# rogerbarton/optix-renderer

Hardware: AMD Instinct MI355X
Metric: Msamples/sec (whole node) + traversal HBM GB/s, cbox 1024x1024 256spp (higher is better)
Workload: dtype f32; 1 GPU; Cornell box (diffuse-only) 1024x1024, 16400 spp, path_mis; config=c2, width=1024, height=1024, spp=16400, mode=wavefront, traversal=ordered, pools=2, gpu_max_hw_queues=8, parallelism=single GPU

## Files before the change

### include/nori_hip.h

```cpp
#ifndef NORI_HIP_H
#define NORI_HIP_H

#include <stddef.h>
#include <stdint.h>

#ifdef __cplusplus
extern "C" {
#endif

#define NH_OK 0
#define NH_ERR_INVALID 1
#define NH_ERR_IO 2
#define NH_ERR_DEVICE 3
#define NH_ERR_UNSUPPORTED 4
#define NH_ERR_STATE 5


enum { NH_SHAPE_MESH = 0, NH_SHAPE_SPHERE = 1 };
enum { NH_BSDF_DIFFUSE = 0, NH_BSDF_MIRROR = 1, NH_BSDF_DIELECTRIC = 2, NH_BSDF_MICROFACET = 3, NH_BSDF_DISNEY = 4 };
enum { NH_EMITTER_AREA = 0, NH_EMITTER_POINT = 1, NH_EMITTER_ENVMAP = 2, NH_EMITTER_SPOT = 3,
       NH_EMITTER_DIRECTIONAL = 4 };
enum { NH_INTEGRATOR_PATH_MIS = 0, NH_INTEGRATOR_PATH_MATS = 1, NH_INTEGRATOR_DIRECT_EMS = 2,
       NH_INTEGRATOR_DIRECT_MATS = 3, NH_INTEGRATOR_DIRECT_MIS = 4, NH_INTEGRATOR_DIRECT = 5,
       NH_INTEGRATOR_NORMALS = 6,
// ... 102 lines not shown

typedef struct nh_envmap {
    int32_t width, height;
    const float *rgba;
    float radiance[3];
    float scale_u, scale_v;
    float offset_u, offset_v;
    int32_t spherical;
    int32_t constant;
    const float *cdf;
    float normalization;
    float rotation[9];
} nh_envmap;

enum { NH_DENOISER_NONE = 0, NH_DENOISER_SIMPLE = 1 };
typedef struct nh_denoiser {
    int32_t type;
    float sigma_d;
    float sigma_vr;
    int32_t range;
    int32_t amount;
} nh_denoiser;

enum { NH_SAMPLER_INDEPENDENT = 0, NH_SAMPLER_ADAPTIVE = 1 };

typedef struct nh_scene_desc {
    nh_camera camera;
    nh_filter filter;
    int32_t integrator;
    int32_t sample_count;
    uint32_t n_shapes;
    const nh_shape *shapes;
    uint32_t n_bsdfs;
    const nh_bsdf *bsdfs;
    uint32_t n_emitters;
    const nh_emitter *emitters;
    const float *emitter_cdf;
    int32_t envmap;
    uint32_t n_vertices;
    const float *V;
    const float *N;
    const float *UV;
    const float *T;
    const float *BT;
    uint32_t n_faces;
    const uint32_t *F;
    uint32_t n_area_cdf;
    const float *area_cdf;
    nh_envmap env;
    nh_denoiser denoiser;
    uint32_t n_textures;
    const nh_texture *textures;
    uint64_t n_texels;
    const float *texels;
    float normals_direction[3];
    const nh_emitter_ext *emitter_ext;
    uint32_t n_media;
    const nh_medium *media;
    const uint32_t *shape_medium;
    uint32_t ambient_medium;
    int32_t sampler;
    int32_t adaptive_initial_uniform;
} nh_scene_desc;


typedef struct nh_bvh_node {
    uint32_t word0;
    uint32_t word1;
    float bbox_min[3];
    float bbox_max[3];
} nh_bvh_node;

typedef struct nh_bvh_desc {
    uint32_t n_nodes;
    const nh_bvh_node *nodes;
    uint32_t n_indices;
    const uint32_t *indices;
    uint32_t n_shapes;
    const uint32_t *shape_offset;
    float bbox_min[3], bbox_max[3];
    uint32_t max_depth;
} nh_bvh_desc;


typedef struct nh_ray_soa {
    const float *ox, *oy, *oz;
    const float *dx, *dy, *dz;
    const float *mint, *maxt;
} nh_ray_soa;

typedef struct nh_hit_soa {
    uint8_t *hit;
    float *t, *u, *v;
    uint32_t *prim;
    uint32_t *shape;
} nh_hit_soa;


enum { NH_MODE_MEGAKERNEL = 0, NH_MODE_WAVEFRONT = 1 };
enum { NH_TRAVERSAL_REFERENCE = 0, NH_TRAVERSAL_ORDERED = 1, NH_TRAVERSAL_WIDE = 2 };

typedef struct nh_render_req {
    int32_t sample_begin;
    int32_t sample_end;
    uint64_t seed;
    int32_t n_blocks;
    const int32_t *blocks;
    int32_t mode;
    int32_t traversal;
    int32_t clear;
    int32_t collect_stats;
} nh_render_req;

#define NH_SMALL_TABLES_BYTES 4096

typedef struct nh_render_stats {
    double kernel_ms_path;
    double kernel_ms_splat;
    double kernel_ms_extend;
    double kernel_ms_shadow;
    double kernel_ms_shade;
    uint64_t launches_path, launches_splat, launches_extend, launches_shadow, launches_shade;
    uint64_t samples;
    uint64_t ray_queries;
    uint64_t nodes_visited;
    uint64_t boxes_tested;
    uint64_t prims_tested;
    uint64_t invalid_samples;
    uint64_t shadow_queries, shadow_nodes_visited, shadow_boxes_tested, shadow_prims_tested;
    uint64_t shade_state_bytes, extend_queue_bytes, shadow_queue_bytes, paths_shaded;
    double kernel_ms_tail;
    uint64_t launches_tail;
    uint64_t node_bytes;
    uint64_t tail_queries, tail_nodes_visited, tail_boxes_tested, tail_prims_tested;
    uint64_t tail_shadow_queries, tail_shadow_nodes_visited, tail_shadow_boxes_tested, tail_shadow_prims_tested;
    uint64_t lds_scene;
    uint64_t fused_bounce;
    uint64_t comm_inits;
    double kernel_ms_denoise;
    uint64_t launches_denoise;
    uint64_t tails_async;
    uint64_t pools_active;
    uint64_t trace_fused;
    uint64_t tail_cycles_body, tail_cycles_shadow, tail_cycles_closest, tail_cycles_head;
    uint64_t tail_bounces, tail_max_bounces;
    uint64_t tail_coop_cycles_body, tail_coop_cycles_shadow, tail_coop_cycles_closest, tail_coop_cycles_head;
    uint64_t tail_coop_bounces;
    uint64_t bounce_cycles_load, bounce_cycles_body, bounce_cycles_shadow, bounce_cycles_closest, bounce_cycles_head;
    uint64_t bounce_cycles_store, bounce_bounces;
    uint64_t bounce_traits;
    uint64_t primary_masks;
    uint64_t pair_kinds;
    uint64_t flat_trace;
} nh_render_stats;

typedef struct nh_scene nh_scene;
typedef struct nh_bvh nh_bvh;
typedef struct nh_ctx nh_ctx;

int nh_scene_load_xml(const char *path, nh_scene **out);
int nh_scene_load_xml_index(const char *path, int32_t index, nh_scene **out);
int nh_scene_get_desc(const nh_scene *scene, nh_scene_desc *out);
int nh_scene_set_resolution(nh_scene *scene, int32_t width, int32_t height);
int nh_scene_set_sample_count(nh_scene *scene, int32_t spp);
int nh_scene_set_sampler(nh_scene *scene, int32_t type, int32_t initial_uniform);
int nh_scene_set_bsdf(nh_scene *scene, uint32_t shape, const nh_bsdf *bsdf);
uint32_t nh_scene_add_texture(nh_scene *scene, const nh_texture *tex, const float *texels);
int nh_scene_set_normal_map(nh_scene *scene, uint32_t shape, uint32_t texture);
int nh_scene_set_lens_draw_order(nh_scene *scene, int32_t order);
int nh_texture_decode(const uint8_t *rgba8, uint64_t n, int32_t srgb, float *out);
int nh_scene_set_integrator(nh_scene *scene, int32_t integrator);
typedef struct nh_photon_params {
    int32_t photon_count;
    float photon_radius;
} nh_photon_params;
int nh_scene_get_photon_params(const nh_scene *scene, nh_photon_params *out);
int nh_scene_set_photon_params(nh_scene *scene, const nh_photon_params *params);
typedef struct nh_av_params {
    float length;
} nh_av_params;
int nh_scene_get_av_params(const nh_scene *scene, nh_av_params *out);
int nh_scene_set_av_params(nh_scene *scene, const nh_av_params *params);
int nh_photon_tables(float *cos_theta, float *sin_theta, float *cos_phi, float *sin_phi, float *exp_table);
void nh_scene_free(nh_scene *scene);
const char *nh_host_last_error(void);
int nh_debug_transform(const char *request, float *out, int32_t cap);

int nh_bvh_build(const nh_scene_desc *scene, int32_t n_threads, nh_bvh **out);
int nh_bvh_get_desc(const nh_bvh *bvh, nh_bvh_desc *out);
void nh_bvh_free(nh_bvh *bvh);

int nh_primary_masks(const nh_camera *camera, const float *records, int32_t n_records, const int32_t *blocks,
                     int32_t n_blocks, uint64_t *masks, int32_t *built);
int32_t nh_primary_mask_pad(int32_t width, int32_t height);

int nh_pair_layout(const float *records, int32_t n_records, const int32_t *leaves, int32_t n_leaves, int32_t by_kind,
                   int32_t *slots, int32_t *leaf_pairs);

int nh_flat_image(const float *records, int32_t n_records, const int32_t *leaves, int32_t n_leaves, const float *boxes,
                  int32_t allowed, float *image, int32_t image_cap_f4, int32_t *n_f4, int32_t *box_equal);

int nh_framebuffer_to_rgb(const float *rgbw, int32_t width, int32_t height, int32_t border, float *rgb);
int nh_write_pfm(const char *path, const float *rgb, int32_t width, int32_t height);
int nh_image_load_png(const char *path, uint8_t *rgba, size_t cap, int32_t *width, int32_t *height);
int nh_write_exr(const char *path, const float *rgb, int32_t width, int32_t height);
int nh_rgb_to_ldr(const float *rgb, int32_t width, int32_t height, uint8_t *rgb8);
int nh_write_png(const char *path, const float *rgb, int32_t width, int32_t height);

int nh_get_device_count(int *n);
int nh_create(int device, nh_ctx **out);
void nh_destroy(nh_ctx *ctx);
int nh_upload_scene(nh_ctx *ctx, const nh_scene_desc *scene);
int nh_upload_bvh(nh_ctx *ctx, const nh_bvh_desc *bvh);
int nh_trace_rays(nh_ctx *ctx, const nh_ray_soa *rays, int32_t n, int32_t any_hit, int32_t traversal, nh_hit_soa *out);
#define NH_ADAPTIVE_MAX_SAMPLES 133948
#define NH_ADAPTIVE_STAGING_BYTES ((size_t)4 << 30)
int nh_render(nh_ctx *ctx, const nh_render_req *req);
typedef struct nh_adaptive_stats {
    uint64_t total_samples;
    uint64_t passes;
    uint64_t max_passes;
    uint64_t n_blocks;
} nh_adaptive_stats;
int nh_get_adaptive_stats(nh_ctx *ctx, nh_adaptive_stats *out);
int nh_get_adaptive_variance(nh_ctx *ctx, float *out, size_t n_floats);
int nh_synchronize(nh_ctx *ctx);
int nh_get_framebuffer(nh_ctx *ctx, float *rgbw, size_t n_floats);
int nh_framebuffer_device_ptr(nh_ctx *ctx, void **dptr, size_t *n_floats);
int nh_get_stats(nh_ctx *ctx, nh_render_stats *out);
int nh_reset_stats(nh_ctx *ctx);
int nh_reduce_framebuffers(nh_ctx **ctxs, int32_t n, int32_t root);
int nh_denoise(nh_ctx *ctx, const nh_denoiser *params);
int nh_denoise_image(nh_ctx *ctx, float *rgbw, int32_t width, int32_t height, int32_t border,
                     const nh_denoiser *params);
enum { NH_BSDF_QUERY_EVAL = 0, NH_BSDF_QUERY_SAMPLE = 1 };
int nh_bsdf_query(nh_ctx *ctx, const nh_bsdf *bsdf, const float *albedo, int32_t mode, int32_t n, const float *wi,
                  const float *wo, const float *sample, float *wo_out, float *value, float *pdf, int32_t *measure);
enum { NH_EMITTER_QUERY_SAMPLE = 0, NH_EMITTER_QUERY_EVAL = 1, NH_EMITTER_QUERY_PDF = 2,
       NH_EMITTER_QUERY_SAMPLE_PHOTON = 3 };
#define NH_EMITTER_QUERY_SAMPLE_STRIDE 16
#define NH_EMITTER_QUERY_PHOTON_STRIDE 12
#define NH_EMITTER_QUERY_IN_STRIDE 9
int nh_emitter_query(nh_ctx *ctx, uint32_t emitter, int32_t mode, int32_t n, const float *ref, const float *sample,
                     float *out);
enum { NH_MEDIUM_QUERY_FREE_PATH = 0, NH_MEDIUM_QUERY_TRANSMITTANCE = 1, NH_MEDIUM_QUERY_PHASE_SAMPLE = 2,
       NH_MEDIUM_QUERY_PHASE_PDF = 3 };
int nh_medium_query(nh_ctx *ctx, uint32_t medium, int32_t mode, int32_t n, const float *in, float *out);


enum { NH_TEST_TTEST = 0, NH_TEST_CHI2TEST = 1 };
typedef struct nh_test_desc {
    int32_t type;
    float significance_level;
    int32_t sample_count;
    uint32_t n_angles;
    const float *angles;
    uint32_t n_references;
    const float *references;
    uint32_t n_scenes;
    uint32_t n_bsdfs;
    const nh_bsdf *bsdfs;
} nh_test_desc;
typedef struct nh_test nh_test;
int nh_test_load_xml(const char *path, nh_test **out);
int nh_test_get_desc(const nh_test *test, nh_test_desc *out);
void nh_test_free(nh_test *test);

int nh_students_t_test(double mean, double variance, double reference, int32_t n, double alpha, int32_t num_tests,
                       int32_t *accepted, double *p_value);

#define NH_RADIANCE_QUERY_MAX (1 << 24)
int nh_radiance_query(nh_ctx *ctx, uint64_t seed, int32_t n, const int32_t *pixel, const int32_t *sample,
                      const float *pixel_sample, float *rgb, float *jitter);
int nh_ttest_scene(nh_ctx *ctx, uint64_t seed, int64_t first, int32_t n, double *mean, double *variance,
                   float *luminance);
int nh_ttest_bsdf(nh_ctx *ctx, const nh_bsdf *bsdf, const float *albedo, float angle_deg, uint64_t first_draw,
                  int32_t n, double *mean, double *variance, float *luminance);
typedef struct nh_test_result {
    double mean, variance, reference, p_value;
    int32_t accepted;
    int32_t sample_count;
    float angle;
    int32_t pad;
} nh_test_result;
int nh_test_run(int device, const char *path, uint64_t seed, nh_test_result *results, int32_t cap,
                int32_t *n_results);


#define NH_PHOTON_STREAM ((uint64_t)1 << 32)
#define NH_PHOTON_DEFAULT_BATCH (1 << 18)
int nh_photon_map_build(nh_ctx *ctx, const nh_photon_params *params, uint64_t seed, int32_t batch_paths);
typedef struct nh_photon_stats {
    int32_t stored;
    int32_t emitted;
    float radius;
    float cell_size;
    uint64_t occupied_cells;
} nh_photon_stats;
int nh_get_photon_stats(nh_ctx *ctx, nh_photon_stats *out);
int nh_get_photons(nh_ctx *ctx, int32_t first, int32_t n, float *position, float *direction, float *power,
                   uint8_t *bytes, int32_t *path, int32_t *bounce);
enum { NH_PHOTON_QUERY_CODEC = 0, NH_PHOTON_QUERY_GATHER = 1 };
int nh_photon_query(nh_ctx *ctx, int32_t mode, int32_t n, const float *in, uint8_t *bytes, int32_t *count, float *out);


int nh_set_av_params(nh_ctx *ctx, const nh_av_params *params);

const char *nh_last_error(const nh_ctx *ctx);

#ifdef __cplusplus
}
#endif
#endif
```

### optix-renderer_amd/csrc/nh_api.hip

```cpp
#include <atomic>
#include <cmath>
#include <cstring>

#include "nh_ctx.h"

using nhd::DBsdf;

int query_bsdf_record(nh_ctx *c, std::vector<void *> &owner, const nh_bsdf *b, const float *albedo, DBsdf &o,
                      float alb[3]) {
    std::memset(&o, 0, sizeof(o));
    o.type = b->type;
    o.ar = b->albedo[0]; o.ag = b->albedo[1]; o.ab = b->albedo[2];
    o.alpha = b->alpha; o.int_ior = b->int_ior; o.ext_ior = b->ext_ior; o.ks = b->ks;
    o.kr = b->kd[0]; o.kg = b->kd[1]; o.kb = b->kd[2];
    o.tex = b->type == NH_BSDF_DISNEY && b->albedo_texture ? 1 : 0;
    for (int k = 0; k < 3; ++k) alb[k] = albedo ? albedo[k] : b->albedo[k];
    if (b->type == NH_BSDF_DISNEY) {
        nhd::DDisney *rec = nullptr;
        const std::vector<nhd::DDisney> recs{disney_record(*b)};
        const std::vector<float> a(alb, alb + 3);
        if (int rc = disney_upload(c, owner, recs, a, &rec)) return rc;
        disney_set_record(o, rec);
    }
    return NH_OK;
}

extern "C" {

const char *nh_last_error(const nh_ctx *ctx) { return ctx ? ctx->err.c_str() : "null context"; }

int nh_get_device_count(int *n) {
    if (!n) return NH_ERR_INVALID;
    int c = 0;
    if (hipGetDeviceCount(&c) != hipSuccess) c = 0;
    *n = c;
    return NH_OK;
}

int nh_create(int device, nh_ctx **out) {
    if (!out) return NH_ERR_INVALID;
    *out = nullptr;
    int n = 0;
    if (hipGetDeviceCount(&n) != hipSuccess || device < 0 || device >= n) return NH_ERR_DEVICE;
    auto *c = new nh_ctx();
    static std::atomic<uint64_t> next_id{1};
    c->id = next_id++;
    c->device = device;
    if (hipSetDevice(device) != hipSuccess || hipStreamCreateWithFlags(&c->stream, hipStreamNonBlocking) != hipSuccess ||
        hipMalloc(&c->counters, kStatShards * kStatStride * sizeof(unsigned long long)) != hipSuccess ||
        hipEventCreateWithFlags(&c->fb_ev, hipEventDisableTiming) != hipSuccess) {
        delete c;
        return NH_ERR_DEVICE;
    }
    (void)hipMemset(c->counters, 0, kStatShards * kStatStride * sizeof(unsigned long long));
    *out = c;
    return NH_OK;
}

void nh_destroy(nh_ctx *c) {
    if (!c) return;
    DeviceGuard guard;
    (void)hipSetDevice(c->device);
    (void)pipeline_drain(c);
    if (c->stream) (void)hipStreamSynchronize(c->stream);
    free_all(c->scene_bufs);
    free_all(c->bvh_bufs);
    (void)hipFree(c->fb);
    (void)hipFree(c->rec);
    c->px.release();
    (void)hipFree(c->pmask);
    (void)hipFree(c->block_rank);
    (void)hipFree(c->staging);
    free_all(c->av_bufs);
    (void)hipFree(c->counters);
    photon_release(c, true);
    (void)hipFree(c->d_scene);
    c->d_scene = nullptr;
    for (WfPool &p : c->pools) pool_free(p);
    adaptive_release(c);
    c->comms.reset();
    if (c->fb_ev) (void)hipEventDestroy(c->fb_ev);
    if (c->stream) (void)hipStreamDestroy(c->stream);
    delete c;
}

int nh_trace_rays(nh_ctx *c, const nh_ray_soa *r, int32_t n, int32_t any_hit, int32_t traversal, nh_hit_soa *out) {
    if (!c || !r || !out || n < 0) return NH_ERR_INVALID;
    if (!c->has_bvh) return fail(c, "nh_trace_rays: no BVH uploaded"), NH_ERR_STATE;
    if (n == 0) return NH_OK;
    HIP_TRY(c, hipSetDevice(c->device));
    if (int rc_ = pipeline_drain(c)) return rc_;
    std::vector<void *> tmp;
    const float *in[8];
    const float *src[8] = {r->ox, r->oy, r->oz, r->dx, r->dy, r->dz, r->mint, r->maxt};
    int rc;
    for (int i = 0; i < 8; ++i)
        if ((rc = upload(c, tmp, src[i], (size_t)n, &in[i]))) { free_all(tmp); return rc; }
    RayBatch rb{in[0], in[1], in[2], in[3], in[4], in[5], in[6], in[7]};
    HitBatch hb{};
    void *p;
    size_t nn = (size_t)n;
    HIP_TRY(c, hipMalloc(&p, nn)); tmp.push_back(p); hb.hit = (uint8_t *)p;
    HIP_TRY(c, hipMalloc(&p, nn * 4)); tmp.push_back(p); hb.t = (float *)p;
    HIP_TRY(c, hipMalloc(&p, nn * 4)); tmp.push_back(p); hb.u = (float *)p;
    HIP_TRY(c, hipMalloc(&p, nn * 4)); tmp.push_back(p); hb.v = (float *)p;
    HIP_TRY(c, hipMalloc(&p, nn * 4)); tmp.push_back(p); hb.k = (int *)p;
    if (traversal == NH_TRAVERSAL_WIDE && c->tv.wnodes) {
        HIP_TRY(c, hipMalloc(&p, nn * (size_t)c->depth_wide * sizeof(int2)));
        tmp.push_back(p);
        nh::launch_trace_wide(c->d_scene, c->tv, rb, hb, n, any_hit != 0, true, false, (int2 *)p, c->depth_wide,
                              c->counters, c->stream, c->wide_w);
    } else {
        nh::launch_trace(c->d_scene, c->tv, rb, hb, n, any_hit != 0, traversal != NH_TRAVERSAL_REFERENCE, false,
                         c->depth, c->counters, c->stream);
    }
    HIP_TRY(c, hipGetLastError());
    std::vector<int> k(nn);
    HIP_TRY(c, hipMemcpyAsync(out->hit, hb.hit, nn, hipMemcpyDeviceToHost, c->stream));
    if (!any_hit) {
        if (out->t) HIP_TRY(c, hipMemcpyAsync(out->t, hb.t, nn * 4, hipMemcpyDeviceToHost, c->stream));
        if (out->u) HIP_TRY(c, hipMemcpyAsync(out->u, hb.u, nn * 4, hipMemcpyDeviceToHost, c->stream));
        if (out->v) HIP_TRY(c, hipMemcpyAsync(out->v, hb.v, nn * 4, hipMemcpyDeviceToHost, c->stream));
        HIP_TRY(c, hipMemcpyAsync(k.data(), hb.k, nn * 4, hipMemcpyDeviceToHost, c->stream));
    }
    HIP_TRY(c, hipStreamSynchronize(c->stream));
    free_all(tmp);
    if (!any_hit)
        for (size_t i = 0; i < nn; ++i) {
            uint32_t prim = 0xffffffffu, shape = 0xffffffffu;
            if (k[i] >= 0) {
                prim = c->bvh_indices[(size_t)k[i]];
                shape = (uint32_t)(std::upper_bound(c->shape_offset.begin(), c->shape_offset.end(), prim) -
                                   c->shape_offset.begin()) - 1;
            }
            if (out->prim) out->prim[i] = prim;
            if (out->shape) out->shape[i] = shape;
        }
    return NH_OK;
}

int nh_bsdf_query(nh_ctx *c, const nh_bsdf *b, const float *albedo, int32_t mode, int32_t n, const float *wi,
                  const float *wo, const float *sample, float *wo_out, float *value, float *pdf, int32_t *measure) {
    if (!c) return NH_ERR_INVALID;
    if (!b || n < 0 || !wi || !value || !pdf) return fail(c, "nh_bsdf_query: null argument"), NH_ERR_INVALID;
    if (b->type < NH_BSDF_DIFFUSE || b->type > NH_BSDF_DISNEY) return fail(c, "unknown BSDF type"), NH_ERR_INVALID;
    if (mode != NH_BSDF_QUERY_EVAL && mode != NH_BSDF_QUERY_SAMPLE)
        return fail(c, "nh_bsdf_query: unknown mode"), NH_ERR_INVALID;
    if (mode == NH_BSDF_QUERY_EVAL ? !wo : (!sample || !wo_out || !measure))
        return fail(c, "nh_bsdf_query: the mode's arrays are missing"), NH_ERR_INVALID;
    if (n == 0) return NH_OK;
    HIP_TRY(c, hipSetDevice(c->device));
    std::vector<void *> bufs;
    struct Free {
        std::vector<void *> &v;
        ~Free() { free_all(v); }
    } guard{bufs};
    nh_disney::nh::BsdfQuery q;
    std::memset(&q, 0, sizeof(q));
    if (int rc = query_bsdf_record(c, bufs, b, albedo, q.bsdf, q.albedo)) return rc;
    q.mode = mode;
    q.n = n;
    const size_t sn = (size_t)n;
    if (int rc = upload(c, bufs, wi, 3 * sn, &q.wi)) return rc;
    if (mode == NH_BSDF_QUERY_EVAL) {
        if (int rc = upload(c, bufs, wo, 3 * sn, &q.wo)) return rc;
    } else {
        if (int rc = upload(c, bufs, sample, 2 * sn, &q.sample)) return rc;
    }
    void *out = nullptr;
    HIP_TRY(c, hipMalloc(&out, 8 * sn * sizeof(float)));
    bufs.push_back(out);
    float *f = static_cast<float *>(out);
    q.wo_out = f;
    q.value = f + 3 * sn;
    q.pdf = f + 6 * sn;
    q.measure = reinterpret_cast<int *>(f + 7 * sn);
    nh_disney::nh::launch_bsdf_query(q, c->stream);
    HIP_TRY(c, hipGetLastError());
    std::vector<float> host(8 * sn);
    HIP_TRY(c, hipMemcpyAsync(host.data(), out, host.size() * sizeof(float), hipMemcpyDeviceToHost, c->stream));
    HIP_TRY(c, hipStreamSynchronize(c->stream));
    if (wo_out) std::memcpy(wo_out, host.data(), 3 * sn * sizeof(float));
    std::memcpy(value, host.data() + 3 * sn, 3 * sn * sizeof(float));
    std::memcpy(pdf, host.data() + 6 * sn, sn * sizeof(float));
    if (measure) std::memcpy(measure, host.data() + 7 * sn, sn * sizeof(float));
    return NH_OK;
}

int nh_emitter_query(nh_ctx *c, uint32_t emitter, int32_t mode, int32_t n, const float *ref, const float *sample,
                     float *out) {
    if (!c) return NH_ERR_INVALID;
    const bool photon = mode == NH_EMITTER_QUERY_SAMPLE_PHOTON;
    if (n < 0 || (!ref && !photon) || !sample || !out) return fail(c, "nh_emitter_query: null argument"), NH_ERR_INVALID;
    if (mode < NH_EMITTER_QUERY_SAMPLE || mode > NH_EMITTER_QUERY_SAMPLE_PHOTON)
        return fail(c, "nh_emitter_query: unknown mode"), NH_ERR_INVALID;
    if (!c->has_scene) return fail(c, "nh_emitter_query: no scene uploaded"), NH_ERR_STATE;
    if (emitter >= c->h_emitters.size()) return fail(c, "nh_emitter_query: emitter index out of range"), NH_ERR_INVALID;
    const nhd::DEmitter &e = c->h_emitters[emitter];
    if (e.type == NH_EMITTER_AREA && (e.shape < 0 || (size_t)e.shape >= c->h_shapes.size()))
        return fail(c, "nh_emitter_query: area light without a valid shape"), NH_ERR_INVALID;
    if (photon && e.type != NH_EMITTER_AREA)
        return fail(c, "nh_emitter_query: samplePhoton of an emitter that is not an area light is not supported"),
               NH_ERR_UNSUPPORTED;
    const size_t sn = (size_t)n;
    if (mode == NH_EMITTER_QUERY_SAMPLE || photon)
        for (size_t i = 0; i < (photon ? 4 : 2) * sn; ++i)
            if (!(sample[i] >= 0.f && sample[i] < 1.f))
                return fail(c, "nh_emitter_query: sample outside [0, 1)"), NH_ERR_INVALID;
    if (n == 0) return NH_OK;
    HIP_TRY(c, hipSetDevice(c->device));
    if (int rc_ = pipeline_drain(c)) return rc_;
    std::vector<void *> bufs;
    struct Free {
        std::vector<void *> &v;
        ~Free() { free_all(v); }
    } guard{bufs};
    const nhd::DScene *d_s = nullptr;
    if (int rc = upload(c, bufs, &c->S, 1, &d_s)) return rc;
    nh_disney::nh::EmitterQuery q;
    q.emitter = (int)emitter;
    q.mode = mode;
    q.n = n;
    const size_t in_stride = photon ? 4 : (mode == NH_EMITTER_QUERY_SAMPLE ? 2 : NH_EMITTER_QUERY_IN_STRIDE);
// ... 272 lines not shown
```

### optix-renderer_amd/csrc/nh_ctx.h

```cpp
#pragma once
#include <hip/hip_runtime.h>
#include <rccl/rccl.h>

#include <algorithm>
#include <cstdint>
#include <deque>
#include <memory>
#include <string>
#include <vector>

#include "nh_internal.h"
#include "nori_hip.h"

constexpr int kRing = 4;
constexpr int kPools = 4;
constexpr int kTails = 3;
constexpr int kTailCap = 65536;
#ifndef NH_DEFAULT_POOLS
#define NH_DEFAULT_POOLS 2
#endif

struct WfJob {
    uint64_t seq;
    int s0, rounds;
// ... 1 lines not shown
    bool ordered, stats;
    bool staged;
    bool jit;
};

struct WfPool {
    hipStream_t stream = nullptr;
    WfState wf{};
    std::vector<void *> bufs;
    size_t cap = 0;
    float *rec = nullptr;
    size_t rec_cap = 0;
    float2 *jit = nullptr;
    size_t jit_cap = 0;
    float4 *staging = nullptr;
    size_t staging_cap = 0;
    uint32_t *spill = nullptr;
    int spill_words = 0;
    unsigned *h_counts = nullptr;
    hipEvent_t copy_ev[kRing] = {};
    std::vector<hipEvent_t> events;
    hipEvent_t ev_begin = nullptr, ev_path = nullptr, ev_splat0 = nullptr, ev_splat = nullptr;
    hipEvent_t ev_handoff = nullptr;
    enum State { IDLE, ENQUEUE, COUNTS, SPLAT, FINISH } state = IDLE;
    WfJob job{};
    WfLaunch L{};
    bool persistent = false, wide = false, trace2 = false, tail = false, draining = false;
    bool fused = false, sorted = false;
    bool rr = false;
    bool trait = false;
    bool shade_sorted = false;
    int64_t tail_at = 0, drain_at = 0;
    int it = 0;
    std::vector<uint64_t> in_e, in_s;
};

struct CommSet {
    std::vector<uint64_t> ids;
    std::vector<int> devices;
    std::vector<ncclComm_t> comms;
    ~CommSet() {
        int cur = 0;
        const bool have = hipGetDevice(&cur) == hipSuccess;
        for (size_t i = 0; i < comms.size(); ++i) {
            (void)hipSetDevice(devices[i]);
            (void)ncclCommDestroy(comms[i]);
        }
        if (have) (void)hipSetDevice(cur);
    }
};

struct DeviceGuard {
    int dev = 0;
    bool ok = false;
    DeviceGuard() { ok = hipGetDevice(&dev) == hipSuccess; }
    ~DeviceGuard() {
        if (ok) (void)hipSetDevice(dev);
    }
};

struct PixelList {
    int *pixel_list = nullptr, *pixel_map = nullptr;
    int *block_ids = nullptr, *block_slot = nullptr;
    int *color_slots = nullptr;
    int n_blocks = 0, n_color0 = 0, n_list = 0;
    std::vector<int32_t> list_key;
    bool have_list = false;
    void release() {
        for (int *p : {pixel_list, pixel_map, block_ids, block_slot, color_slots}) (void)hipFree(p);
        *this = PixelList{};
    }
};

struct AdaptiveState {
    int n_blocks = 0, nbx = 0, nby = 0;
    int next_sample = -1;
    int4 *blocks = nullptr;
    int *block_rank = nullptr, *active_list = nullptr, *next = nullptr;
    AdBlock *state = nullptr;
    unsigned *counts = nullptr, *h_count = nullptr;
    int2 *pos = nullptr;
    float4 *rad = nullptr, *staging = nullptr;
    float2 *jit = nullptr;
    size_t slot_cap = 0;
    unsigned long long *stats = nullptr;
    std::vector<int4> h_blocks;
};

struct PhotonState {
    bool built = false;
    std::vector<void *> bufs;
    const float *tables = nullptr;
    std::vector<float> h_tables;
    float *pos = nullptr;
    uint2 *bytes = nullptr;
    uint32_t *path = nullptr;
    int *bounce = nullptr;
    nh_photon_stats stats{};
};

struct nh_ctx {
    uint64_t id = 0;
    std::shared_ptr<CommSet> comms;
    int device = 0;
    hipStream_t stream = nullptr;
    std::string err;
    std::vector<nh_shape> shapes;
    std::vector<float> V;
    std::vector<uint32_t> F;
    int width = 0, height = 0, border = 0, n_emitters = 0, integrator = 0;
    nh_filter filter{};
    nhd::DScene S{};
    nhd::DScene *d_scene = nullptr;
    nhd::Traversal tv{};
    std::vector<void *> scene_bufs, bvh_bufs;
    bool has_scene = false, has_bvh = false;
    int depth = 0;
    int depth_wide = 0;
    int wide_w = 4;
    int n_node_f4 = 0, n_leaves = 0, n_prim_f4 = 0;
    std::vector<uint32_t> bvh_indices, shape_offset;
    std::vector<int> shape_bsdf_type;
    std::vector<int> shape_bsdf_real;
    int n_bsdf_types = 0;
    bool disney = false;
    bool specular = false;
    bool textured = false;
    bool normal_mapped = false;
    bool diffuse_area = false;
    bool bsdfless = false, has_media = false;
    int sampler = 0, adaptive_initial_uniform = 0;
    AdaptiveState ad;
    PhotonState photon;
    bool av_set = false;
    AvLaunch av{};
    std::vector<void *> av_bufs;
    size_t av_cap = 0;
    int2 *av_spill = nullptr;
    int av_spill_depth = 0;
    std::vector<nhd::DShape> h_shapes;
    std::vector<nhd::DBsdf> h_bsdfs;
    std::vector<nhd::DEmitter> h_emitters;
    std::vector<float> h_area_cdf;
    int n_emit_faces = 0;
    float4 *small_image = nullptr;
    int small_tab[5] = {0, 0, 0, 0, 0};
    bool pair_kinds = false;
    float4 *small_image_ref = nullptr;
    const float4 *flat_image = nullptr;
    nh_camera camera{};
    std::vector<float> h_prims;
    unsigned long long *pmask = nullptr;
    bool pmask_known = false;
    float *fb = nullptr;
    size_t fb_floats = 0;
    float *rec = nullptr;
    size_t rec_cap = 0;
    int *block_rank = nullptr;
    int nbx = 0, nby = 0;
    PixelList px;
    float4 *staging = nullptr;
    size_t staging_cap = 0;
    unsigned long long *counters = nullptr;
    nh_render_stats stats{};
    WfPool pools[kPools + kTails];
    std::deque<WfJob> jobs;
    uint64_t job_seq = 0, splat_seq = 0;
    hipEvent_t fb_ev = nullptr;
    bool fb_ev_set = false;
    uint64_t stats_comm_inits = 0;
};

inline void drop_primary_masks(nh_ctx *c) {
    (void)hipFree(c->pmask);
    c->pmask = nullptr;
    c->pmask_known = false;
}

#define NH_LAUNCH(c, fn) ((c)->disney ? nh_disney::nh::fn : nh::fn)

void pool_free(WfPool &p);
int pipeline_drain(nh_ctx *c);
int check_device(nh_ctx *c, const char *where);
int render_adaptive(nh_ctx *c, const nh_render_req *q);
void adaptive_release(nh_ctx *c);
void photon_release(nh_ctx *c, bool tables = false);
nhd::DDisney disney_record(const nh_bsdf &b);
void disney_set_record(nhd::DBsdf &o, const nhd::DDisney *rec);
int disney_upload(nh_ctx *c, std::vector<void *> &owner, const std::vector<nhd::DDisney> &recs,
                  const std::vector<float> &albedo, nhd::DDisney **out);

int query_bsdf_record(nh_ctx *c, std::vector<void *> &owner, const nh_bsdf *b, const float *albedo, nhd::DBsdf &o,
                      float alb[3]);

inline bool fail(nh_ctx *c, const std::string &m) {
    if (c) c->err = m;
    return false;
}

#define HIP_TRY(ctx, expr)                                                                               \
    do {                                                                                                 \
        hipError_t e_ = (expr);                                                                          \
        if (e_ != hipSuccess) {                                                                          \
            (ctx)->err = std::string(#expr) + ": " + hipGetErrorString(e_);                              \
            return NH_ERR_DEVICE;                                                                        \
        }                                                                                                \
    } while (0)

template <typename T>
int upload(nh_ctx *c, std::vector<void *> &owner, const T *src, size_t n, const T **dst) {
    void *p = nullptr;
    size_t bytes = (std::max<size_t>(n * sizeof(T), 16) + 15) / 16 * 16;
    HIP_TRY(c, hipMalloc(&p, bytes));
    owner.push_back(p);
    if (n) HIP_TRY(c, hipMemcpyAsync(p, src, n * sizeof(T), hipMemcpyHostToDevice, c->stream));
    *dst = reinterpret_cast<const T *>(p);
    return NH_OK;
}

inline void free_all(std::vector<void *> &v) {
    for (void *p : v) (void)hipFree(p);
    v.clear();
}
```

### optix-renderer_amd/csrc/nh_internal.h

```cpp
#pragma once
#include <hip/hip_runtime.h>
#include <stdint.h>

#include "nh_device.h"
#include "nh_traverse.h"
#include "nori_hip.h"

struct RayBatch {
    const float *ox, *oy, *oz, *dx, *dy, *dz, *mint, *maxt;
};
struct HitBatch {
    uint8_t *hit;
    float *t, *u, *v;
    int *k;
};
#ifndef NH_REC_STRIDE
#define NH_REC_STRIDE 3
#endif
constexpr int kRecFloats = NH_REC_STRIDE;

struct PathLaunch {
    int n_paths;
    int n_list;
    int s0;
    uint64_t seed;
    const int *pixel_list;
    float *rec;
    unsigned long long *counters;
};
struct AvLaunch {
    int n_paths, n_list, s0;
    uint64_t seed;
    const int *pixel_list;
    float *rec;
    float *ray[8];
    HitBatch hit;
    uint64_t *rng;
    float *q_ray[8];
    int *q_path;
    uint8_t *q_hit;
    unsigned *q_count;
};
__host__ __device__ __forceinline__ int stage_pitch(int cols) { return (cols + 7) & ~7; }
__host__ __device__ __forceinline__ int stage_off(int cols, int band, int xt, int yt) {
    if (!band) return yt * stage_pitch(cols) + xt;
    if (xt >= 32) return 1024 + yt * 4 + (xt - 32);
    if (yt >= 32) return 1024 + 144 + (yt - 32) * 32 + xt;
    return yt * 32 + xt;
}

struct SplatLaunch {
    float *fb;
    int width, height, border, reach, nbx, n_rounds, n_list;
    const int *pixel_map;
    const int *block_rank;
    const float *rec;
    const float2 *jit;
    uint64_t seed;
    int s0;
    float radius, lookup;
    float table[33];
    const int *blocks;
    const int *block_slot;
    int n_blocks;
    float4 *staging;
    int staged;
    int direct;
    int persist;
    int band;
    const int *color_slots;
    int n_color0;
    int debug;
};

struct DenoiseLaunch {
    const float4 *src;
    int src_stride;
    float4 *dst;
    int dst_stride;
    int width, height, range;
    float sigma_vr;
    const float *g;
    float *var;
    unsigned *minmax;
    int band_first;
    int lag;
    int chunk;
};

constexpr int kStatShards = 8, kStatStride = 48, kStatAny = 8, kStatTail = 16, kStatTailAny = 20;
constexpr int kStatTailClk = 24;
constexpr int kStatTailCoopClk = 32;
constexpr int kStatBounceClk = 40;
__device__ __forceinline__ unsigned long long *stat_shard(unsigned long long *c) {
    return c + (blockIdx.x & (kStatShards - 1)) * kStatStride;
}
__device__ __forceinline__ void flush_stats(const nhd::TravStats &st, uint32_t queries, unsigned long long *counters) {
    unsigned long long v[4] = {queries, st.nodes, st.boxes, st.prims};
#pragma unroll
    for (int i = 0; i < 4; ++i) {
        unsigned long long x = v[i];
#pragma unroll
        for (int off = 32; off > 0; off >>= 1) x += __shfl_xor(x, off, 64);
        if ((threadIdx.x & 63) == 0) atomicAdd(&counters[i], x);
    }
}

namespace nh {
void launch_trace(const nhd::DScene *S, const nhd::Traversal &tv, const RayBatch &rb, const HitBatch &hb, int n,
                  bool any, bool ordered, bool stats, int depth, unsigned long long *ctr, hipStream_t st);
void launch_trace_wide(const nhd::DScene *S, const nhd::Traversal &tv, const RayBatch &rb, const HitBatch &hb, int n,
                       bool any, bool ordered, bool stats, int2 *spill, int spill_depth, unsigned long long *ctr,
                       hipStream_t st, int wide = 4);
void launch_path(const nhd::DScene *S, const nhd::Traversal &tv, const PathLaunch &L, bool ordered, bool stats,
                 int depth, bool pm, hipStream_t st);
void launch_splat(const SplatLaunch &P, hipStream_t st);
void launch_av_primary(const nhd::DScene *S, const AvLaunch &L, hipStream_t st);
void launch_av_shade(const nhd::DScene *S, const nhd::Traversal &tv, const AvLaunch &L, hipStream_t st);
void launch_av_resolve(const AvLaunch &L, int bound, hipStream_t st);
bool splat_uses_staging(int border, int reach);
void launch_count_invalid(const float *rec, size_t n, unsigned long long *out, hipStream_t st);
void launch_denoise_variance(const DenoiseLaunch &P, hipStream_t st);
int denoise_band_rows();
int denoise_max_chunk();
int tree_top_nodes();
size_t denoise_tile_static_lds();
void launch_denoise_band(const DenoiseLaunch &P, int L, int n_bands, size_t tile_bytes, hipStream_t st);
void launch_denoise_copy(const float4 *src, int src_stride, float4 *dst, int dst_stride, int width, int height,
                         hipStream_t st);
}

constexpr int kQueueShards = 8, kCountStride = 32;

struct WfBuf {
    float4 *ray_o;
    float4 *ray_d;
    float4 *hit;
    uint64_t *rng;
    float4 *li;
    float4 *thr;
    float4 *pend;
    uint8_t *occl;
};
struct WfState {
    WfBuf buf[2];
    float4 *sh_o, *sh_d;
    int *sh_slot;
    unsigned *counts;
};
constexpr int kCountGroup = kQueueShards * kCountStride;
constexpr int kCountSlot = 4 * kCountGroup;

struct WfLaunch {
    WfState st;
    int n_paths, n_list, s0;
    uint64_t seed;
    const int *pixel_list;
    float *rec;
    float2 *jit;
    int in_q;
    int first;
    int cam_rays;
    unsigned *cnt_in;
    unsigned *cnt_out;
    int seg_cap;
    int small_nodes, small_leaves, small_prims;
    int small_frames;
    const float4 *small_image;
    int small_tab[5];
    uint32_t *trav_spill;
    int spill_depth;
    unsigned long long *counters;
    const unsigned long long *pmask;
    int pmask_nbx;
    const float4 *flat;
};
constexpr int kPersistentBlocks = 256 * 16;
constexpr size_t kSmallSceneBytes = 16384;
constexpr int kSmallFramesMaxPrims = 256;
constexpr size_t kSmallTablesBytes = NH_SMALL_TABLES_BYTES;
namespace nh {
void launch_wf_trace(const nhd::DScene *S, const nhd::Traversal &tv, const WfLaunch &L, bool ordered, bool stats,
                     bool shadow, bool persistent, int wide, int bound, int depth, hipStream_t st);
void launch_wf_trace2(const nhd::DScene *S, const nhd::Traversal &tv, const WfLaunch &L, bool ordered, bool stats,
                      int wide, int bound, hipStream_t st);
void launch_wf_camera_rays(const nhd::DScene *S, const WfLaunch &L, int bound, hipStream_t st);
void launch_wf_shade(const nhd::DScene *S, const nhd::Traversal &tv, const WfLaunch &L, bool sort, bool nmap, int bound,
                     hipStream_t st);
void launch_wf_bounce(const nhd::DScene *S, const nhd::Traversal &tv, const WfLaunch &L, bool ordered, bool stats,
                      bool sort, int bound, hipStream_t st);
void launch_wf_bounce_rr(const nhd::DScene *S, const nhd::Traversal &tv, const WfLaunch &L, bool ordered, bool stats, bool sort,
                         bool lean, bool nmap, bool trait, int bound, hipStream_t st);
void launch_wf_tail_rr(const nhd::DScene *S, const nhd::Traversal &tv, const WfLaunch &L, bool ordered, bool stats, int bound,
                       bool specular, bool lean, bool nmap, bool trait, hipStream_t st);
void launch_wf_bounce_trait(const nhd::DScene *S, const nhd::Traversal &tv, const WfLaunch &L, bool stats, int bound,
                            hipStream_t st);
void launch_wf_tail_trait(const nhd::DScene *S, const nhd::Traversal &tv, const WfLaunch &L, bool stats, int bound,
                          int coop, hipStream_t st);
void launch_wf_tail(const nhd::DScene *S, const nhd::Traversal &tv, const WfLaunch &L, bool ordered, bool stats,
                    int wide, int bound, int depth, hipStream_t st);
void launch_wf_pack_rr(const WfLaunch &L, const WfBuf &dst, unsigned *dst_counts, int bound, hipStream_t st);
void launch_small_image(const nhd::Traversal &tv, int n_prim_f4, const int2 *slots, int pairs_off, int frames_off,
                        float4 *image, hipStream_t st);
void launch_wf_counts(const unsigned *src, unsigned *host_dst, int n_copy, unsigned *zero, int n_zero, hipStream_t st);
}

namespace nh_disney {
namespace nh {
void launch_path(const nhd::DScene *S, const nhd::Traversal &tv, const PathLaunch &L, bool ordered, bool stats,
                 int depth, bool pm, hipStream_t st);
void launch_wf_shade(const nhd::DScene *S, const nhd::Traversal &tv, const WfLaunch &L, bool sort, bool nmap, int bound,
                     hipStream_t st);
void launch_wf_bounce(const nhd::DScene *S, const nhd::Traversal &tv, const WfLaunch &L, bool ordered, bool stats,
                      bool sort, int bound, hipStream_t st);
void launch_wf_bounce_rr(const nhd::DScene *S, const nhd::Traversal &tv, const WfLaunch &L, bool ordered, bool stats, bool sort,
                         bool lean, bool nmap, bool trait, int bound, hipStream_t st);
void launch_wf_tail_rr(const nhd::DScene *S, const nhd::Traversal &tv, const WfLaunch &L, bool ordered, bool stats, int bound,
                       bool specular, bool lean, bool nmap, bool trait, hipStream_t st);
void launch_wf_tail(const nhd::DScene *S, const nhd::Traversal &tv, const WfLaunch &L, bool ordered, bool stats,
                    int wide, int bound, int depth, hipStream_t st);
void launch_disney_fold(nhd::DDisney *recs, const float *albedo, int n, hipStream_t st);
struct BsdfQuery {
    nhd::DBsdf bsdf;
    float albedo[3];
    int mode, n;
    const float *wi, *wo, *sample;
    float *wo_out, *value, *pdf;
    int *measure;
};
void launch_bsdf_query(const BsdfQuery &q, hipStream_t st);
struct EmitterQuery {
    int emitter, mode, n;
    const float *ref, *in;
    float *out;
};
void launch_emitter_query(const nhd::DScene *S, const EmitterQuery &q, hipStream_t st);
void launch_vol_path(const nhd::DScene *S, const nhd::Traversal &tv, const PathLaunch &L, bool mis, bool stats, int depth,
                     hipStream_t st);
struct MediumQuery {
    int medium, mode, n;
    const float *in;
    float *out;
};
void launch_medium_query(const nhd::DScene *S, const MediumQuery &q, hipStream_t st);
}
}

struct PhotonTrace {
    uint64_t seed, k0;
    int n_paths;
    long long *counts;
    const long long *offsets;
    long long base;
    int cap;
    float *pos;
    uint2 *bytes;
    uint32_t *path;
    int *bounce;
    int *emitted;
};
struct PhotonFinalize {
    int n;
    const float *pos;
    const uint2 *bytes;
    const float *tab;
    nhd::DPhotonMap pm;
    uint64_t *keys;
    uint32_t *index;
    const uint32_t *sorted_index;
    unsigned long long *cells;
};
struct PhotonQuery {
    int mode, n;
    const float *in;
    const float *tab;
    uint8_t *bytes;
    int *count;
    float *out;
};
namespace nh_disney {
namespace nh {
void launch_photon_trace(const nhd::DScene *S, const nhd::Traversal &tv, const PhotonTrace &P, int depth, hipStream_t st);
size_t photon_scan_temp_bytes(int n);
hipError_t photon_scan(const long long *counts, long long *offsets, int n, void *tmp, size_t tmp_bytes, hipStream_t st);
void launch_photon_keys(const PhotonFinalize &F, hipStream_t st);
hipError_t photon_sort(const uint64_t *keys_in, uint64_t *keys_out, const uint32_t *index_in, uint32_t *index_out,
                       int n, hipStream_t st);
void launch_photon_scatter(const PhotonFinalize &F, hipStream_t st);
void launch_photon_path(const nhd::DScene *S, const nhd::Traversal &tv, const PathLaunch &L, bool stats, int depth,
                        hipStream_t st);
void launch_photon_query(const nhd::DScene *S, const PhotonQuery &q, hipStream_t st);
}
}

constexpr int kAdBlock = 4;
constexpr int kAdPaths = 16;
constexpr int kAdPassStride = 1002;
constexpr int kAdMaxRound = 1000;
constexpr int kAdMaxBorder = 2;
constexpr int kAdImagePx = 64;
struct AdBlock {
    uint64_t rng_state, rng_inc;
    float old_var[16];
    float old_norm;
    int active;
    int npass;
    int head, last;
    int pad;
};
struct AdaptiveLaunch {
    int n_blocks, nbx, nby;
    int width, height, border, initial_uniform;
    int s, k;
    uint64_t seed;
    const int4 *blocks;
    const int *block_rank;
    AdBlock *state;
    int *active_list;
    unsigned *counts;
    int n_active;
    int2 *pos;
    float4 *rad;
    float2 *jit;
    float4 *staging;
    int *next;
    int slot_base;
    unsigned long long *stats;
// ... 41 lines not shown
```

### optix-renderer_amd/csrc/nh_pipeline.hip

```cpp
#include <cmath>
#include <cstdlib>
#include <cstring>
#include <thread>
#include <type_traits>

#include "../host/gpu_layout.h"
#include "nh_ctx.h"


constexpr size_t kWfBytesPerPath = 2 * (16 * 6 + 8 + 1) + 36;

static int pool_alloc(nh_ctx *c, WfPool &p, size_t n, size_t rec_n, size_t staging_f4, bool jit = false) {
    if (!p.stream) {
        if (!p.h_counts && hipHostMalloc(reinterpret_cast<void **>(&p.h_counts),
                                         (kRing * 2 * kCountGroup + kCountSlot) * sizeof(unsigned)) != hipSuccess) {
            p.h_counts = nullptr;
            return fail(c, "hipHostMalloc failed"), NH_ERR_DEVICE;
        }
        for (hipEvent_t &e : p.copy_ev)
            if (!e) HIP_TRY(c, hipEventCreateWithFlags(&e, hipEventDisableTiming));
        for (hipEvent_t *e : {&p.ev_begin, &p.ev_path, &p.ev_splat0, &p.ev_splat})
            if (!*e) HIP_TRY(c, hipEventCreate(e));
        if (!p.ev_handoff) HIP_TRY(c, hipEventCreateWithFlags(&p.ev_handoff, hipEventDisableTiming));
        HIP_TRY(c, hipStreamCreateWithFlags(&p.stream, hipStreamNonBlocking));
// ... 41 lines not shown
        (void)hipFree(p.staging);
        p.staging = nullptr;
        p.staging_cap = 0;
        HIP_TRY(c, hipMalloc(&p.staging, staging_f4 * sizeof(float4)));
        p.staging_cap = staging_f4;
    }
    return NH_OK;
}

void pool_free(WfPool &p) {
    free_all(p.bufs);
    (void)hipFree(p.rec);
    (void)hipFree(p.jit);
    (void)hipFree(p.staging);
    (void)hipFree(p.spill);
    if (p.h_counts) (void)hipHostFree(p.h_counts);
    for (hipEvent_t e : p.events) (void)hipEventDestroy(e);
    for (hipEvent_t e : p.copy_ev)
        if (e) (void)hipEventDestroy(e);
    for (hipEvent_t e : {p.ev_begin, p.ev_path, p.ev_splat0, p.ev_splat, p.ev_handoff})
        if (e) (void)hipEventDestroy(e);
    if (p.stream) (void)hipStreamDestroy(p.stream);
    p = WfPool{};
}

static SplatLaunch make_splat(const nh_ctx *c, const float *rec, uint64_t seed, int s0, float4 *staging, int rounds,
                              bool staged) {
    SplatLaunch P{};
    P.staged = staged ? 1 : 0;
    P.fb = c->fb;
    P.width = c->width;
    P.height = c->height;
    P.border = c->border;
    P.reach = (int)std::floor(c->filter.radius + 0.5f);
    P.nbx = c->nbx;
    P.n_rounds = rounds;
    P.n_list = c->px.n_list;
    P.pixel_map = c->px.pixel_map;
    P.block_rank = c->block_rank;
    P.rec = rec;
    P.seed = seed;
    P.s0 = s0;
    P.radius = c->filter.radius;
    P.lookup = c->filter.lookup_factor;
    std::memcpy(P.table, c->filter.table, sizeof(P.table));
    P.blocks = c->px.block_ids;
    P.block_slot = c->px.block_slot;
    P.n_blocks = c->px.n_blocks;
    P.color_slots = c->px.color_slots;
    P.n_color0 = c->px.n_color0;
    P.staging = staging;
    return P;
}

static bool splat_staged(const nh_ctx *c) {
    return nh::splat_uses_staging(c->border, (int)std::floor(c->filter.radius + 0.5f));
}
static size_t block_px(const nh_ctx *c, bool staged) {
    if (!staged) return 0;
    return (size_t)(32 + 2 * c->border) * (size_t)stage_pitch(32 + 2 * c->border);
}

static int active_pools(const nh_ctx *c) {
    const char *np = std::getenv("NH_POOLS");
    const int def = c->specular ? NH_DEFAULT_POOLS + 1 : NH_DEFAULT_POOLS;
    return std::max(1, std::min(kPools, np ? std::atoi(np) : def));
}

static bool tail_async_enabled() {
    const char *e = std::getenv("NH_TAIL_ASYNC");
    return e && e[0] == '1';
}

static int pool_start(nh_ctx *c, WfPool &p, const WfJob &job) {
    WfJob j = job;
    j.staged = splat_staged(c);
    const char *jv = std::getenv("NH_SPLAT_JITTER");
    j.jit = jv && std::strcmp(jv, "stored") == 0;
    const int n_paths = j.rounds * c->px.n_list;
    const size_t staging_f4 = (size_t)j.rounds * c->px.n_blocks * block_px(c, j.staged);
    int rc = pool_alloc(c, p, (size_t)n_paths, (size_t)n_paths, staging_f4, j.jit);
    if (rc) return rc;
    for (int i = 0; i < active_pools(c); ++i) {
        WfPool &o = c->pools[i];
        if (&o == &p || o.state != WfPool::IDLE) continue;
        if ((rc = pool_alloc(c, o, (size_t)n_paths, (size_t)n_paths, staging_f4, j.jit))) return rc;
    }
    if (active_pools(c) > 1 && tail_async_enabled())
        for (int i = kPools; i < kPools + kTails; ++i) {
            WfPool &o = c->pools[i];
            if (o.state != WfPool::IDLE) continue;
            if ((rc = pool_alloc(c, o, (size_t)kTailCap, (size_t)n_paths, staging_f4, j.jit))) return rc;
        }
    p.job = j;
    WfLaunch &L = p.L;
    L = WfLaunch{};
    L.st = p.wf;
    L.n_paths = n_paths;
    L.n_list = c->px.n_list;
    L.s0 = j.s0;
    L.seed = j.seed;
    L.pixel_list = c->px.pixel_list;
    L.rec = p.rec;
    L.jit = j.jit ? p.jit : nullptr;
    L.counters = c->counters;
    const size_t scene_bytes = 16 * (size_t)(c->n_node_f4 + c->n_prim_f4) + 8 * (size_t)c->n_leaves;
    bool small = scene_bytes <= kSmallSceneBytes;
    if (const char *e = std::getenv("NH_LDS_SCENE")) small = small && e[0] != '0';
    if (small) {
        L.small_nodes = c->n_node_f4;
        L.small_leaves = c->n_leaves;
        L.small_prims = c->n_prim_f4;
        L.small_frames = c->n_prim_f4 / 3 <= kSmallFramesMaxPrims;
        if (const char *e = std::getenv("NH_LDS_FRAMES")) L.small_frames = L.small_frames && e[0] != '0';
        L.small_image = j.stats && c->small_image_ref ? c->small_image_ref : c->small_image;
        for (int i = 0; i < 5; ++i) L.small_tab[i] = c->small_tab[i];
    }
    const int per_chunk = 256;
    const int max_chunks = (n_paths + per_chunk - 1) / per_chunk;
    L.seg_cap = (max_chunks + kQueueShards - 1) / kQueueShards * per_chunk;
    p.persistent = c->depth > 20;
    if (const char *e = std::getenv("NH_PERSISTENT")) p.persistent = e[0] == '1';
    p.wide = p.persistent && j.ordered && c->tv.wnodes != nullptr;
    if (const char *e = std::getenv("NH_WIDE")) p.wide = p.wide && e[0] != '0';
    if (p.wide && !j.ordered) return fail(c, "wavefront pool: the wide traversal needs an ordered job"), NH_ERR_STATE;
    p.trace2 = p.wide && scene_bytes <= (size_t)256 << 20;
    if (const char *e = std::getenv("NH_TRACE2")) p.trace2 = p.wide && e[0] != '0';
    c->stats.trace_fused = p.trace2 ? 1 : 0;
    const int spill_words = p.wide ? 2 * c->depth_wide : (c->depth + 1) / 2 * 2;
    if (p.persistent && p.spill_words < spill_words) {
        HIP_TRY(c, hipStreamSynchronize(p.stream));
        (void)hipFree(p.spill);
        p.spill = nullptr;
        p.spill_words = 0;
        HIP_TRY(c, hipMalloc(&p.spill, (size_t)kPersistentBlocks * 128 * spill_words * sizeof(uint32_t)));
        p.spill_words = spill_words;
    }
    p.fused = small && !p.persistent && c->depth <= 16;
    if (const char *e = std::getenv("NH_FUSED")) p.fused = p.fused && e[0] != '0';
    p.sorted = p.fused && c->n_bsdf_types > 1;
    p.rr = p.fused;
    if (const char *e = std::getenv("NH_RR_AHEAD")) p.rr = p.fused && e[0] != '0';
    p.shade_sorted = false;
    if (const char *e = std::getenv("NH_SORT_SHADE")) p.shade_sorted = !p.fused && e[0] == '1';
    if (const char *e = std::getenv("NH_SORT")) p.sorted = p.fused && e[0] == '1';
    p.trait = p.rr && c->diffuse_area && c->small_tab[0] > 0 && j.ordered && !p.sorted;
    if (const char *e = std::getenv("NH_BOUNCE_TRAITS")) p.trait = p.trait && e[0] != '0';
    c->stats.bounce_traits = p.rr ? (p.trait ? 2 : 1) : 0;
    const char *pm = std::getenv("NH_PRIMARY_MASKS");
    const bool masks = p.rr && c->pmask && !j.stats && !(pm && pm[0] == '0');
    L.pmask = masks ? c->pmask : nullptr;
    L.pmask_nbx = c->nbx;
    c->stats.primary_masks = masks ? 1 : 0;
    c->stats.pair_kinds = p.fused && c->pair_kinds && !j.stats ? 1 : 0;
    const bool flat = p.rr && c->flat_image && c->pair_kinds && !j.stats && !c->disney;
    L.flat = flat ? c->flat_image : nullptr;
    c->stats.flat_trace = flat ? 1 : 0;
    c->stats.fused_bounce = p.fused ? 1 : 0;
    c->stats.node_bytes = p.wide ? 16 * nhd::kWideF4 * (c->wide_w / 4) : 64;
    c->stats.lds_scene = small && !p.persistent && c->depth <= 16 ? 1 : 0;
    L.trav_spill = p.spill;
    L.spill_depth = p.spill_words;
    p.tail_at = p.fused ? std::min<int64_t>(std::max<int64_t>(n_paths / 1024, 8192), 16384)
                        : std::min<int64_t>(std::max<int64_t>(n_paths / 64, 8192), 262144);
    if (const char *e = std::getenv("NH_TAIL")) p.tail_at = std::atoll(e);
    p.drain_at = std::max<int64_t>(n_paths / 8, p.tail_at);
    HIP_TRY(c, hipEventRecord(p.ev_begin, p.stream));
    unsigned *h_init = p.h_counts + kRing * 2 * kCountGroup;
    std::memset(h_init, 0, kCountSlot * sizeof(unsigned));
    h_init[0] = (unsigned)n_paths;
    HIP_TRY(c, hipMemcpyAsync(p.wf.counts, h_init, kCountSlot * sizeof(unsigned), hipMemcpyHostToDevice, p.stream));
    p.in_e.assign(1, (uint64_t)n_paths);
    p.in_s.assign(1, 0);
    p.it = 0;
    p.tail = false;
    p.draining = false;
    p.state = WfPool::ENQUEUE;
    return NH_OK;
}

static void chunk_swap(WfPool &a, WfPool &b) {
    std::swap(a.h_counts, b.h_counts);
    std::swap(a.copy_ev, b.copy_ev);
    std::swap(a.events, b.events);
    std::swap(a.ev_begin, b.ev_begin);
    std::swap(a.ev_path, b.ev_path);
    std::swap(a.ev_splat0, b.ev_splat0);
    std::swap(a.ev_splat, b.ev_splat);
    std::swap(a.job, b.job);
    std::swap(a.L, b.L);
    std::swap(a.persistent, b.persistent);
    std::swap(a.wide, b.wide);
    std::swap(a.trace2, b.trace2);
    std::swap(a.tail, b.tail);
    std::swap(a.draining, b.draining);
    std::swap(a.fused, b.fused);
    std::swap(a.sorted, b.sorted);
    std::swap(a.rr, b.rr);
    std::swap(a.trait, b.trait);
    std::swap(a.shade_sorted, b.shade_sorted);
    std::swap(a.tail_at, b.tail_at);
    std::swap(a.drain_at, b.drain_at);
    std::swap(a.it, b.it);
    std::swap(a.in_e, b.in_e);
    std::swap(a.in_s, b.in_s);
    std::swap(a.rec, b.rec);
    std::swap(a.rec_cap, b.rec_cap);
    std::swap(a.jit, b.jit);
    std::swap(a.jit_cap, b.jit_cap);
    std::swap(a.staging, b.staging);
    std::swap(a.staging_cap, b.staging_cap);
}

static WfPool *free_tail_slot(nh_ctx *c, const WfPool &p, int bound) {
    if (!p.rr || bound > kTailCap || active_pools(c) < 2) return nullptr;
    if (!tail_async_enabled()) return nullptr;
    for (int i = kPools; i < kPools + kTails; ++i)
        if (c->pools[i].state == WfPool::IDLE) return &c->pools[i];
    return nullptr;
}

static int pool_handoff(nh_ctx *c, WfPool &p, WfPool &T, int bound, hipEvent_t *ev) {
    int rc = pool_alloc(c, T, (size_t)kTailCap, 0, 0);
    if (rc) return rc;
    HIP_TRY(c, hipMemsetAsync(T.wf.counts, 0, kCountSlot * sizeof(unsigned), p.stream));
    nh::launch_wf_pack_rr(p.L, T.wf.buf[0], T.wf.counts, bound, p.stream);
    HIP_TRY(c, hipGetLastError());
    HIP_TRY(c, hipEventRecord(p.ev_handoff, p.stream));
    chunk_swap(p, T);
    WfLaunch &L = T.L;
    L.st = T.wf;
    L.in_q = 0;
    L.cnt_in = T.wf.counts;
    HIP_TRY(c, hipStreamWaitEvent(T.stream, p.ev_handoff, 0));
    HIP_TRY(c, hipEventRecord(ev[1], T.stream));
    HIP_TRY(c, hipEventRecord(ev[2], T.stream));
    NH_LAUNCH(c, launch_wf_tail_rr)(c->d_scene, c->tv, L, T.job.ordered, T.job.stats, bound, c->specular,
                          !c->specular && !c->textured, c->normal_mapped, T.trait, T.stream);
    HIP_TRY(c, hipGetLastError());
    HIP_TRY(c, hipEventRecord(ev[3], T.stream));
    T.tail = true;
    T.draining = true;
    T.state = WfPool::SPLAT;
    p.state = WfPool::IDLE;
    c->stats.tails_async++;
    return NH_OK;
}

static bool count_kernel() {
    static const bool on = [] {
        const char *e = std::getenv("NH_COUNT_KERNEL");
        return !(e && e[0] == '0');
    }();
    return on;
}

static int count_service(nh_ctx *c, WfPool &p, unsigned *out, unsigned *in_slot, int it) {
    unsigned *h = p.h_counts + (size_t)(it % kRing) * 2 * kCountGroup;
    if (count_kernel()) {
        nh::launch_wf_counts(out, h, 2 * kCountGroup, in_slot, kCountSlot, p.stream);
        HIP_TRY(c, hipGetLastError());
    } else {
        HIP_TRY(c, hipMemcpyAsync(h, out, 2 * kCountGroup * sizeof(unsigned), hipMemcpyDeviceToHost, p.stream));
    }
    HIP_TRY(c, hipEventRecord(p.copy_ev[it % kRing], p.stream));
    return NH_OK;
}

static int pool_enqueue(nh_ctx *c, WfPool &p) {
    WfLaunch &L = p.L;
    const int it = p.it, in = it & 1;
    unsigned *slot[2] = {p.wf.counts, p.wf.counts + kCountSlot};
    L.in_q = in;
    L.first = it == 0;
    L.cam_rays = it == 0 && p.persistent && c->S.dof ? 1 : 0;
    L.cnt_in = slot[in];
    L.cnt_out = slot[in ^ 1];
    while ((size_t)(it + 1) * 4 > p.events.size()) {
        hipEvent_t e;
        HIP_TRY(c, hipEventCreate(&e));
        p.events.push_back(e);
    }
    hipEvent_t *ev = &p.events[(size_t)it * 4];
    const int bound = (int)p.in_e[it == 0 ? 0 : it - 1];
    const bool ordered = p.job.ordered, stats = p.job.stats;
    if (it == 0 || !count_kernel()) HIP_TRY(c, hipMemsetAsync(slot[in ^ 1], 0, kCountSlot * sizeof(unsigned), p.stream));
    HIP_TRY(c, hipEventRecord(ev[0], p.stream));
    if (p.fused) {
        if (it > 0 && (int64_t)bound <= p.tail_at)
            if (WfPool *T = free_tail_slot(c, p, bound)) return pool_handoff(c, p, *T, bound, ev);
        HIP_TRY(c, hipEventRecord(ev[1], p.stream));
        HIP_TRY(c, hipEventRecord(ev[2], p.stream));
        if (it > 0 && (int64_t)bound <= p.tail_at) {
            if (p.rr)
                NH_LAUNCH(c, launch_wf_tail_rr)(c->d_scene, c->tv, L, ordered, stats, bound, c->specular,
                                                !c->specular && !c->textured, c->normal_mapped, p.trait, p.stream);
            else NH_LAUNCH(c, launch_wf_tail)(c->d_scene, c->tv, L, ordered, stats, false, bound, c->depth, p.stream);
            HIP_TRY(c, hipGetLastError());
            HIP_TRY(c, hipEventRecord(ev[3], p.stream));
            p.tail = true;
            p.draining = true;
            p.state = WfPool::SPLAT;
            return NH_OK;
        }
        if (p.rr) NH_LAUNCH(c, launch_wf_bounce_rr)(c->d_scene, c->tv, L, ordered, stats, p.sorted,
                                                    !c->specular && !c->textured, c->normal_mapped, p.trait, bound,
// ... 176 lines not shown
        if (q != hipSuccess && q != hipErrorNotReady) e = q;
    }
    if (e != hipSuccess) {
        c->err = std::string(where) + ": device error in the rendering kernels: " + hipGetErrorString(e);
        return NH_ERR_DEVICE;
    }
    return NH_OK;
}

static void pipeline_reset(nh_ctx *c) {
    for (WfPool &p : c->pools)
        if (p.stream) (void)hipStreamSynchronize(p.stream);
    for (WfPool &p : c->pools) p.state = WfPool::IDLE;
    c->jobs.clear();
    c->splat_seq = c->job_seq;
}

static int pipeline_run(nh_ctx *c, bool all) {
    const int n_pools = active_pools(c);
    c->stats.pools_active = (uint64_t)n_pools;
    for (;;) {
        bool progress = false;
        hipError_t ev_err = hipSuccess;
        for (WfPool &p : c->pools) {
            int rc = NH_OK;
            bool others_draining = true;
            for (const WfPool &o : c->pools) others_draining = others_draining && (o.state == WfPool::IDLE || o.draining);
            if (p.state == WfPool::IDLE && !c->jobs.empty() && &p - c->pools < n_pools && others_draining) {
                rc = pool_start(c, p, c->jobs.front());
                c->jobs.pop_front();
                progress = true;
            }
            if (!rc && p.state == WfPool::ENQUEUE) {
                rc = pool_enqueue(c, p);
                progress = true;
            }
            if (!rc && p.state == WfPool::COUNTS && event_done(p.copy_ev[(p.it - 1) % kRing], ev_err)) {
                rc = pool_read(c, p);
                progress = true;
            }
            if (!rc && p.state == WfPool::SPLAT && p.job.seq == c->splat_seq) {
                rc = pool_splat(c, p);
                progress = true;
            }
            if (!rc && p.state == WfPool::FINISH && event_done(p.ev_splat, ev_err)) {
                rc = pool_finish(c, p);
                progress = true;
            }
            if (!rc && ev_err != hipSuccess) {
                c->err = std::string("wavefront pipeline: ") + hipGetErrorString(ev_err);
                rc = NH_ERR_DEVICE;
            }
            if (rc) {
                pipeline_reset(c);
                return rc;
            }
        }
        if (c->jobs.empty()) {
            bool idle = true, draining = true;
            for (const WfPool &p : c->pools) {
                idle = idle && p.state == WfPool::IDLE;
                draining = draining && (p.state == WfPool::IDLE || p.draining);
            }
            if (idle || (!all && draining)) return NH_OK;
        }
        if (!progress) std::this_thread::yield();
    }
}

int pipeline_drain(nh_ctx *c) {
    int rc = pipeline_run(c, true);
    if (rc) return rc;
    for (WfPool &p : c->pools)
        if (p.stream) HIP_TRY(c, hipStreamSynchronize(p.stream));
    return NH_OK;
}

static int ensure_pixel_list(nh_ctx *c, const nh_render_req *q) {
    std::vector<int32_t> key;
    if (q->n_blocks > 0 && q->blocks) key.assign(q->blocks, q->blocks + q->n_blocks);
    if (c->px.have_list && key == c->px.list_key) return NH_OK;
    if (int rc = pipeline_drain(c)) return rc;
    std::vector<int32_t> blocks = key;
    if (blocks.empty())
        for (int i = 0; i < c->nbx * c->nby; ++i) blocks.push_back(i);
    std::vector<int> list, map((size_t)c->width * c->height, -1);
    for (int32_t bid : blocks) {
        if (bid < 0 || bid >= c->nbx * c->nby) return fail(c, "block id out of range"), NH_ERR_INVALID;
        int bx = bid % c->nbx, by = bid / c->nbx;
        for (int y = by * 32; y < std::min(c->height, by * 32 + 32); ++y)
            for (int x = bx * 32; x < std::min(c->width, bx * 32 + 32); ++x) {
                int pix = y * c->width + x;
                if (map[pix] >= 0) return fail(c, "duplicate block id"), NH_ERR_INVALID;
                map[pix] = (int)list.size();
                list.push_back(pix);
            }
    }
    std::vector<int> slot_map((size_t)c->nbx * c->nby, -1);
    for (size_t i = 0; i < blocks.size(); ++i) slot_map[blocks[i]] = (int)i;
    std::vector<int> color_slots;
    for (int col = 0; col < 2; ++col)
        for (size_t i = 0; i < blocks.size(); ++i)
            if (((blocks[i] % c->nbx + blocks[i] / c->nbx) & 1) == col) color_slots.push_back((int)i);
    PixelList n;
    struct Guard {
        PixelList &l;
        ~Guard() { l.release(); }
    } guard{n};
    for (int32_t bid : blocks) n.n_color0 += ((bid % c->nbx + bid / c->nbx) & 1) == 0;
    n.n_blocks = (int)blocks.size();
    n.n_list = (int)list.size();
    n.list_key = key;
    n.have_list = true;
    const auto table = [&](int *&dst, const std::vector<int> &src) -> int {
        HIP_TRY(c, hipMalloc(&dst, std::max<size_t>(src.size(), 1) * sizeof(int)));
        if (!src.empty())
            HIP_TRY(c, hipMemcpyAsync(dst, src.data(), src.size() * sizeof(int), hipMemcpyHostToDevice, c->stream));
        return NH_OK;
    };
    int rc;
    if ((rc = table(n.color_slots, color_slots)) || (rc = table(n.block_ids, blocks)) ||
        (rc = table(n.block_slot, slot_map)) || (rc = table(n.pixel_list, list)) || (rc = table(n.pixel_map, map)))
        return rc;
    HIP_TRY(c, hipStreamSynchronize(c->stream));
    std::swap(c->px, n);
    drop_primary_masks(c);
    return NH_OK;
}

static int ensure_primary_masks(nh_ctx *c) {
    if (c->pmask_known) return NH_OK;
    if (int rc = pipeline_drain(c)) return rc;
    drop_primary_masks(c);
    c->pmask_known = true;
    const size_t scene_bytes = 16 * (size_t)(c->n_node_f4 + c->n_prim_f4) + 8 * (size_t)c->n_leaves;
    if (c->h_prims.empty() || scene_bytes > kSmallSceneBytes) return NH_OK;
    std::vector<int32_t> blocks = c->px.list_key;
    if (blocks.empty())
        for (int i = 0; i < c->nbx * c->nby; ++i) blocks.push_back(i);
    std::vector<uint64_t> m;
    if (!nh::primary_masks(c->camera, reinterpret_cast<const nh::f4 *>(c->h_prims.data()), (int)(c->h_prims.size() / 12),
                           blocks.data(), (int)blocks.size(), m))
        return NH_OK;
    std::vector<unsigned long long> grid((size_t)c->nbx * c->nby, 0ull);
    for (size_t i = 0; i < blocks.size(); ++i) grid[(size_t)blocks[i]] = m[i];
    unsigned long long *d = nullptr;
    HIP_TRY(c, hipMalloc(&d, std::max<size_t>(grid.size(), 1) * sizeof(unsigned long long)));
    const hipError_t e = hipMemcpy(d, grid.data(), grid.size() * sizeof(unsigned long long), hipMemcpyHostToDevice);
    if (e != hipSuccess) {
        (void)hipFree(d);
        HIP_TRY(c, e);
    }
    c->pmask = d;
    return NH_OK;
}

constexpr size_t kAvBytesPerPath = 94;

static bool av_wide(const nh_ctx *c, const nh_render_req *q) {
    return q->traversal != NH_TRAVERSAL_REFERENCE && c->depth > 20 && c->tv.wnodes != nullptr;
}
static size_t av_bytes_per_path(const nh_ctx *c, const nh_render_req *q) {
    return kAvBytesPerPath + (av_wide(c, q) ? (size_t)c->depth_wide * sizeof(int2) : 0);
}

static int av_reserve(nh_ctx *c, size_t paths, bool wide) {
    const int spill_depth = wide ? c->depth_wide : 0;
    if (c->av_cap >= paths && c->av_spill_depth >= spill_depth) return NH_OK;
    free_all(c->av_bufs);
    c->av_cap = 0;
    c->av_spill_depth = 0;
    c->av_spill = nullptr;
    AvLaunch &L = c->av;
    L = AvLaunch{};
    const auto get = [&](auto **p, size_t n) -> int {
        void *d = nullptr;
        HIP_TRY(c, hipMalloc(&d, std::max<size_t>(n, 1) * sizeof(**p)));
        c->av_bufs.push_back(d);
        *p = static_cast<std::remove_reference_t<decltype(*p)>>(d);
        return NH_OK;
    };
    int rc = NH_OK;
    for (int i = 0; i < 8 && !rc; ++i)
        if (!(rc = get(&L.ray[i], paths))) rc = get(&L.q_ray[i], paths);
    if (rc || (rc = get(&L.hit.hit, paths)) || (rc = get(&L.hit.t, paths)) || (rc = get(&L.hit.u, paths)) ||
        (rc = get(&L.hit.v, paths)) || (rc = get(&L.hit.k, paths)) || (rc = get(&L.rng, paths)) ||
        (rc = get(&L.q_path, paths)) || (rc = get(&L.q_hit, paths)) || (rc = get(&L.q_count, 1)) ||
        (spill_depth && (rc = get(&c->av_spill, paths * (size_t)spill_depth)))) {
        free_all(c->av_bufs);
        return rc;
    }
    c->av_cap = paths;
    c->av_spill_depth = spill_depth;
    return NH_OK;
}

static int av_chunk(nh_ctx *c, const nh_render_req *q, const PathLaunch &P) {
    AvLaunch L = c->av;
    L.n_paths = P.n_paths;
    L.n_list = P.n_list;
    L.s0 = P.s0;
    L.seed = P.seed;
    L.pixel_list = P.pixel_list;
    L.rec = P.rec;
    const bool wide = av_wide(c, q), ordered = q->traversal != NH_TRAVERSAL_REFERENCE, stats = q->collect_stats != 0;
    const auto batch = [&](float *const r[8], const HitBatch &hb, int n, bool any) {
        const RayBatch rb{r[0], r[1], r[2], r[3], r[4], r[5], r[6], r[7]};
        unsigned long long *ctr = c->counters + (any ? kStatAny : 0);
        if (wide) nh::launch_trace_wide(c->d_scene, c->tv, rb, hb, n, any, true, stats, c->av_spill, c->av_spill_depth, ctr,
                                        c->stream, c->wide_w);
        else nh::launch_trace(c->d_scene, c->tv, rb, hb, n, any, ordered, stats, c->depth, ctr, c->stream);
    };
    HIP_TRY(c, hipMemsetAsync(L.q_count, 0, sizeof(unsigned), c->stream));
    nh::launch_av_primary(c->d_scene, L, c->stream);
    batch(L.ray, L.hit, L.n_paths, false);
    nh::launch_av_shade(c->d_scene, c->tv, L, c->stream);
    HIP_TRY(c, hipGetLastError());
    int n_queue = L.n_paths;
    if (stats) {
        unsigned n = 0;
        HIP_TRY(c, hipMemcpyAsync(&n, L.q_count, sizeof(n), hipMemcpyDeviceToHost, c->stream));
        HIP_TRY(c, hipStreamSynchronize(c->stream));
        n_queue = (int)n;
    }
    HitBatch occl{};
    occl.hit = L.q_hit;
    batch(L.q_ray, occl, n_queue, true);
    nh::launch_av_resolve(L, n_queue, c->stream);
    return NH_OK;
}

extern "C" {

int nh_render(nh_ctx *c, const nh_render_req *q) {
    if (!c || !q) return NH_ERR_INVALID;
    if (!c->has_scene || !c->has_bvh) return fail(c, "nh_render: scene and BVH must be uploaded"), NH_ERR_STATE;
    if (q->sample_end < q->sample_begin || q->sample_begin < 0) return fail(c, "invalid sample range"), NH_ERR_INVALID;
    if (c->S.dof && q->sample_end > nhd::kLensLo * nhd::kLensHi)
        return fail(c, "depth of field: sample rounds beyond 2^24"), NH_ERR_UNSUPPORTED;
    if ((c->integrator == NH_INTEGRATOR_PATH_MIS || c->integrator == NH_INTEGRATOR_DIRECT_MIS) && c->n_emitters == 0)
        return fail(c, "No Emitter in scene!"), NH_ERR_INVALID;
    if (q->mode != NH_MODE_MEGAKERNEL && q->mode != NH_MODE_WAVEFRONT) return fail(c, "unknown render mode"), NH_ERR_INVALID;
    const bool volumetric = c->integrator == NH_INTEGRATOR_PATH_VOL_MATS || c->integrator == NH_INTEGRATOR_PATH_VOL_MIS;
    if (!volumetric && (c->bsdfless || c->has_media))
        return fail(c, "the scene has a participating medium or a shape without a BSDF: only the path_vol_mats and "
                       "path_vol_mis integrators render it"), NH_ERR_UNSUPPORTED;
    if (c->integrator == NH_INTEGRATOR_PATH_VOL_MIS && c->n_emitters == 0)
        return fail(c, "No Emitter in scene!"), NH_ERR_INVALID;
    const bool photon = c->integrator == NH_INTEGRATOR_PHOTONMAPPER;
    if (photon && !c->photon.built)
        return fail(c, "nh_render: the photon mapper needs a photon map (nh_photon_map_build)"), NH_ERR_STATE;
    if (photon && c->sampler == NH_SAMPLER_ADAPTIVE)
        return fail(c, "photonmapper: the adaptive sampler is not supported"), NH_ERR_UNSUPPORTED;
    if (c->integrator == NH_INTEGRATOR_AV && !c->av_set)
        return fail(c, "nh_render: the av integrator needs its length (nh_set_av_params)"), NH_ERR_STATE;
    if (c->integrator == NH_INTEGRATOR_ENVMAPTESTER && c->S.envmap < 0)
        return fail(c, "This integrator requires an env map."), NH_ERR_INVALID;
    const bool av_split = q->mode == NH_MODE_WAVEFRONT && c->integrator == NH_INTEGRATOR_AV;
    const bool wavefront = q->mode == NH_MODE_WAVEFRONT && c->integrator <= NH_INTEGRATOR_PATH_MATS;
    if (q->traversal < NH_TRAVERSAL_REFERENCE || q->traversal > NH_TRAVERSAL_WIDE)
        return fail(c, "unknown traversal"), NH_ERR_INVALID;
    if (c->border > 4) return fail(c, "reconstruction filters wider than border 4 are not supported"), NH_ERR_UNSUPPORTED;
    HIP_TRY(c, hipSetDevice(c->device));
    int rc = NH_OK;
    if (!wavefront || q->collect_stats || q->clear || c->sampler == NH_SAMPLER_ADAPTIVE) rc = pipeline_drain(c);
    if (rc) return rc;
    if (c->sampler == NH_SAMPLER_ADAPTIVE) return render_adaptive(c, q);
    rc = ensure_pixel_list(c, q);
    if (rc) return rc;
    if (wavefront && (rc = ensure_primary_masks(c))) return rc;
    c->stats.node_bytes = 64;
    if (av_split && av_wide(c, q)) c->stats.node_bytes = 16 * nhd::kWideF4 * (c->wide_w / 4);
    c->stats.primary_masks = 0;
    c->stats.pair_kinds = 0;
    c->stats.flat_trace = 0;
    c->stats.trace_fused = 0;
    c->stats.lds_scene = 0;
    c->stats.fused_bounce = 0;
    if (q->clear) {
        HIP_TRY(c, hipMemsetAsync(c->fb, 0, c->fb_floats * sizeof(float), c->stream));
        HIP_TRY(c, hipEventRecord(c->fb_ev, c->stream));
        c->fb_ev_set = true;
    }
    const int rounds = q->sample_end - q->sample_begin;
    if (rounds == 0 || c->px.n_list == 0) return NH_OK;
    if (q->collect_stats)
        HIP_TRY(c, hipMemsetAsync(c->counters, 0, kStatShards * kStatStride * sizeof(unsigned long long), c->stream));
    const size_t per_round = (size_t)c->px.n_list;
    const char *jv = std::getenv("NH_SPLAT_JITTER");
    const size_t rec_bytes = kRecFloats * 4 + (wavefront && jv && std::strcmp(jv, "stored") == 0 ? 8 : 0);
    const size_t per_round_bytes = per_round * rec_bytes + (size_t)c->px.n_blocks * block_px(c, splat_staged(c)) * 16 +
                                   (wavefront ? per_round * kWfBytesPerPath : 0) +
                                   (av_split ? per_round * av_bytes_per_path(c, q) : 0);
    size_t budget = wavefront ? (size_t)24 << 30 : (size_t)1 << 30;
    if (const char *e = std::getenv(wavefront ? "NH_WF_BUDGET_MB" : "NH_RECORD_BUDGET_MB"))
        budget = (size_t)std::max(1L, std::atol(e)) << 20;
    if (wavefront) {
        size_t free_b = 0, total_b = 0;
        if (hipMemGetInfo(&free_b, &total_b) == hipSuccess) {
            size_t held = 0;
            for (const WfPool &p : c->pools)
                held += p.cap * kWfBytesPerPath + p.rec_cap * kRecFloats * 4 + p.jit_cap * 8 + p.staging_cap * sizeof(float4);
            const int shares = active_pools(c) + (active_pools(c) > 1 && tail_async_enabled() ? kTails : 0);
            const size_t avail = (size_t)((double)(free_b + held) * 0.85) / (size_t)shares;
            budget = std::min(budget, std::max(avail, per_round_bytes));
        }
    }
    int chunk = (int)std::max<size_t>(1, std::min<size_t>((size_t)rounds, budget / per_round_bytes));
    while ((size_t)chunk * per_round > (size_t)0x7fffffff) chunk = std::max(1, chunk / 2);
    if (wavefront) {
        if (per_round > ((size_t)1 << 26))
            return fail(c, "wavefront mode renders at most 2^26 pixels per context"), NH_ERR_UNSUPPORTED;
        chunk = std::min(chunk, (int)(((size_t)1 << 26) / per_round));
    }

    if (wavefront) {
        HIP_TRY(c, hipStreamSynchronize(c->stream));
        for (int s = q->sample_begin; s < q->sample_end; s += chunk)
            c->jobs.push_back(WfJob{c->job_seq++, s, std::min(chunk, q->sample_end - s), q->seed,
                                    q->traversal != NH_TRAVERSAL_REFERENCE, q->collect_stats != 0});
        rc = q->collect_stats ? pipeline_drain(c) : pipeline_run(c, false);
        if (rc) return rc;
        if (int e = check_device(c, "nh_render")) return e;
    } else {
        if (c->rec_cap < (size_t)chunk * per_round) {
            (void)hipFree(c->rec);
            c->rec = nullptr;
            c->rec_cap = 0;
            const size_t cap = (size_t)chunk * per_round;
            HIP_TRY(c, hipMalloc(&c->rec, cap * kRecFloats * sizeof(float)));
            c->rec_cap = cap;
        }
        if (av_split && (rc = av_reserve(c, (size_t)chunk * per_round, av_wide(c, q)))) return rc;
        const bool staged = splat_staged(c);
        if (c->staging_cap < (size_t)chunk * c->px.n_blocks * block_px(c, staged)) {
            (void)hipFree(c->staging);
            c->staging = nullptr;
            c->staging_cap = 0;
            const size_t cap = (size_t)chunk * c->px.n_blocks * block_px(c, staged);
            HIP_TRY(c, hipMalloc(&c->staging, cap * sizeof(float4)));
            c->staging_cap = cap;
        }
        struct Ev {
            hipEvent_t a, b, d;
        };
        std::vector<Ev> evs;
        for (int s = q->sample_begin; s < q->sample_end; s += chunk) {
            const int k = std::min(chunk, q->sample_end - s);
            PathLaunch L{};
            L.n_paths = k * c->px.n_list;
            L.n_list = c->px.n_list;
            L.s0 = s;
            L.seed = q->seed;
            L.pixel_list = c->px.pixel_list;
            L.rec = c->rec;
            L.counters = c->counters;
            Ev ev;
            HIP_TRY(c, hipEventCreate(&ev.a));
            HIP_TRY(c, hipEventCreate(&ev.b));
            HIP_TRY(c, hipEventCreate(&ev.d));
            HIP_TRY(c, hipEventRecord(ev.a, c->stream));
            if (av_split) {
                if ((rc = av_chunk(c, q, L))) return rc;
            } else if (photon)
                nh_disney::nh::launch_photon_path(c->d_scene, c->tv, L, q->collect_stats != 0, c->depth, c->stream);
            else if (volumetric)
                nh_disney::nh::launch_vol_path(c->d_scene, c->tv, L, c->integrator == NH_INTEGRATOR_PATH_VOL_MIS,
                                               q->collect_stats != 0, c->depth, c->stream);
            else
                NH_LAUNCH(c, launch_path)(c->d_scene, c->tv, L, q->traversal != NH_TRAVERSAL_REFERENCE, q->collect_stats != 0,
                            c->depth, c->integrator == NH_INTEGRATOR_PATH_MIS && !c->normal_mapped, c->stream);
            HIP_TRY(c, hipGetLastError());
            HIP_TRY(c, hipEventRecord(ev.b, c->stream));
            if (q->collect_stats) nh::launch_count_invalid(c->rec, (size_t)L.n_paths, c->counters, c->stream);
            nh::launch_splat(make_splat(c, c->rec, q->seed, s, c->staging, k, staged), c->stream);
            HIP_TRY(c, hipGetLastError());
            HIP_TRY(c, hipEventRecord(ev.d, c->stream));
            evs.push_back(ev);
        }
        HIP_TRY(c, hipStreamSynchronize(c->stream));
        for (auto &ev : evs) {
            float a = 0, b = 0;
            (void)hipEventElapsedTime(&a, ev.a, ev.b);
            (void)hipEventElapsedTime(&b, ev.b, ev.d);
            c->stats.kernel_ms_path += a;
            c->stats.kernel_ms_splat += b;
            c->stats.launches_path++;
            c->stats.launches_splat++;
            (void)hipEventDestroy(ev.a);
            (void)hipEventDestroy(ev.b);
            (void)hipEventDestroy(ev.d);
        }
        c->stats.samples += (uint64_t)rounds * (uint64_t)c->px.n_list;
    }
    if (q->collect_stats) {
        unsigned long long hs[kStatShards * kStatStride], h[kStatStride] = {};
        HIP_TRY(c, hipMemcpy(hs, c->counters, sizeof(hs), hipMemcpyDeviceToHost));
        for (int sh = 0; sh < kStatShards; ++sh)
            for (int j = 0; j < kStatStride; ++j) h[j] += hs[sh * kStatStride + j];
        h[kStatTailClk + 5] = 0;
        for (int sh = 0; sh < kStatShards; ++sh)
            h[kStatTailClk + 5] = std::max(h[kStatTailClk + 5], hs[sh * kStatStride + kStatTailClk + 5]);
        c->stats.tail_cycles_body += h[kStatTailClk];
        c->stats.tail_cycles_shadow += h[kStatTailClk + 1];
        c->stats.tail_cycles_closest += h[kStatTailClk + 2];
        c->stats.tail_cycles_head += h[kStatTailClk + 3];
        c->stats.tail_bounces += h[kStatTailClk + 4];
        c->stats.tail_max_bounces = std::max<uint64_t>(c->stats.tail_max_bounces, h[kStatTailClk + 5]);
        c->stats.tail_coop_cycles_body += h[kStatTailCoopClk];
        c->stats.tail_coop_cycles_shadow += h[kStatTailCoopClk + 1];
        c->stats.tail_coop_cycles_closest += h[kStatTailCoopClk + 2];
        c->stats.tail_coop_cycles_head += h[kStatTailCoopClk + 3];
        c->stats.tail_coop_bounces += h[kStatTailCoopClk + 4];
        c->stats.bounce_cycles_load += h[kStatBounceClk];
        c->stats.bounce_cycles_body += h[kStatBounceClk + 1];
        c->stats.bounce_cycles_shadow += h[kStatBounceClk + 2];
        c->stats.bounce_cycles_closest += h[kStatBounceClk + 3];
        c->stats.bounce_cycles_head += h[kStatBounceClk + 4];
        c->stats.bounce_cycles_store += h[kStatBounceClk + 5];
        c->stats.bounce_bounces += h[kStatBounceClk + 6];
        const unsigned long long *cl = h, *an = h + kStatAny, *tc = h + kStatTail, *ta = h + kStatTailAny;
        c->stats.ray_queries += cl[0] + an[0] + tc[0] + ta[0];
        c->stats.nodes_visited += cl[1] + an[1] + tc[1] + ta[1];
        c->stats.boxes_tested += cl[2] + an[2] + tc[2] + ta[2];
        c->stats.prims_tested += cl[3] + an[3] + tc[3] + ta[3];
        c->stats.invalid_samples += h[4];
// ... 18 lines not shown
```

### optix-renderer_amd/csrc/nh_upload.hip

```cpp
#include <cmath>
#include <cstdlib>
#include <cstring>

#include "../host/gpu_layout.h"
#include "nh_ctx.h"

using nhd::DBsdf;
using nhd::DEmitter;
using nhd::DShape;

static_assert(sizeof(nh::f4) == sizeof(float4) && alignof(float4) % alignof(nh::f4) == 0, "nh::f4 is float4's layout");
static_assert(sizeof(nh::i2) == sizeof(int2) && alignof(int2) % alignof(nh::i2) == 0, "nh::i2 is int2's layout");
static_assert(sizeof(nh::u64x2) == sizeof(ulonglong2) && alignof(ulonglong2) % alignof(nh::u64x2) == 0,
              "nh::u64x2 is ulonglong2's layout");
static_assert((int)nhd::BSDF_DIELECTRIC == (int)NH_BSDF_DIELECTRIC, "the isolated-sphere marking reads NH_BSDF_*");

nhd::DDisney disney_record(const nh_bsdf &b) {
    nhd::DDisney o;
    std::memset(&o, 0, sizeof(o));
    o.metallic = b.metallic; o.subsurface = b.subsurface; o.specular = b.specular; o.roughness = b.roughness;
    o.specular_tint = b.specular_tint; o.anisotropic = b.anisotropic; o.sheen = b.sheen; o.sheen_tint = b.sheen_tint;
    o.clearcoat = b.clearcoat; o.clearcoat_gloss = b.clearcoat_gloss;
    return o;
}
// ... 209 lines not shown
    if ((rc = upload(c, c->scene_bufs, d->BT, 3 * nv, &S.BT))) return rc;
    if ((rc = upload(c, c->scene_bufs, d->F, 3 * (size_t)d->n_faces, &S.F))) return rc;
    S.emit_faces = nullptr;
    if (!ef_tri.empty()) {
        const uint4 *tri = nullptr;
        if ((rc = upload(c, c->scene_bufs, ef_tri.data(), ef_tri.size(), &tri))) return rc;
        float4 *faces = nullptr;
        HIP_TRY(c, hipMalloc(&faces, 3 * ef_tri.size() * sizeof(float4)));
        c->scene_bufs.push_back(faces);
        const int n = (int)ef_tri.size();
        hipLaunchKernelGGL(emit_face_kernel, dim3((n + 255) / 256), dim3(256), 0, c->stream, S.V, tri, n, faces);
        HIP_TRY(c, hipGetLastError());
        S.emit_faces = faces;
    }
    if ((rc = upload(c, c->scene_bufs, d->area_cdf, (size_t)d->n_area_cdf, &S.area_cdf))) return rc;
    if (!dt.empty() && (rc = upload(c, c->scene_bufs, dt.data(), dt.size(), &S.texs))) return rc;
    if (d->n_texels) {
        const float *tx = nullptr;
        if ((rc = upload(c, c->scene_bufs, d->texels, 4 * (size_t)d->n_texels, &tx))) return rc;
        S.texels = reinterpret_cast<const float4 *>(tx);
    }
    S.envmap = d->envmap;
    if (d->envmap >= 0) {
        const nh_envmap &e = d->env;
        const size_t texels = (size_t)e.width * (size_t)e.height;
        const float *rgba = nullptr;
        if ((rc = upload(c, c->scene_bufs, e.rgba, 4 * texels, &rgba))) return rc;
        S.env_rgba = reinterpret_cast<const float4 *>(rgba);
        if ((rc = upload(c, c->scene_bufs, e.cdf, texels + 1, &S.env_cdf))) return rc;
        S.env_guide = nullptr;
        S.env_guide_bits = 0;
        bool monotone = true;
        for (size_t i = 0; i <= texels && monotone; ++i)
            monotone = !std::isnan(e.cdf[i]) && (i == 0 || !(e.cdf[i] < e.cdf[i - 1]));
        if (monotone && texels >= 64 && !(std::getenv("NH_ENV_GUIDE") && std::getenv("NH_ENV_GUIDE")[0] == '0')) {
            int bits = 0;
            while (bits < 20 && ((size_t)1 << (bits + 2)) < texels) ++bits;
            const size_t M = (size_t)1 << bits;
            std::vector<int> guide(M + 1);
            size_t i = 0;
            for (size_t j = 0; j <= M; ++j) {
                const float t = (float)((double)j / (double)M);
                while (i <= texels && e.cdf[i] < t) ++i;
                guide[j] = (int)i;
            }
            const int *g = nullptr;
            if ((rc = upload(c, c->scene_bufs, guide.data(), guide.size(), &g))) return rc;
            HIP_TRY(c, hipStreamSynchronize(c->stream));
            S.env_guide = g;
            S.env_guide_bits = bits;
        }
        S.env_w = e.width;
        S.env_h = e.height;
        S.env_spherical = e.spherical;
        std::memcpy(S.env_rot, e.rotation, sizeof(S.env_rot));
        S.env_constant = e.constant;
        S.env_norm = e.normalization;
        S.env_su = e.scale_u;
        S.env_sv = e.scale_v;
        S.env_ou = e.offset_u;
        S.env_ov = e.offset_v;
        S.env_r = e.radiance[0];
        S.env_g = e.radiance[1];
        S.env_b = e.radiance[2];
    }
    S.n_emitters = (int)d->n_emitters;
    S.nee_finite = nh::nee_finite(d) ? 1 : 0;
    if (d->integrator < NH_INTEGRATOR_PATH_MIS || d->integrator > NH_INTEGRATOR_ENVMAPTESTER)
        return fail(c, "unknown integrator"), NH_ERR_INVALID;
    S.integrator = d->integrator;
    S.av_length = 0.f;
    for (int i = 0; i < 3; ++i) S.ndir[i] = d->normals_direction[i];
    std::memcpy(S.s2c, d->camera.sample_to_camera, sizeof(S.s2c));
    std::memcpy(S.c2w, d->camera.camera_to_world, sizeof(S.c2w));
    {
        float ow[4];
        const float z = 0.0f;
        for (int i = 0; i < 4; ++i) {
            float acc = S.c2w[4 * i] * z;
            acc = acc + S.c2w[4 * i + 1] * z;
            acc = acc + S.c2w[4 * i + 2] * z;
            acc = acc + S.c2w[4 * i + 3] * 1.0f;
            ow[i] = acc;
        }
        for (int i = 0; i < 3; ++i) S.cam_o[i] = ow[i] / ow[3];
    }
    S.inv_w = d->camera.inv_output_size[0];
    S.inv_h = d->camera.inv_output_size[1];
    S.near_clip = d->camera.near_clip;
    S.far_clip = d->camera.far_clip;
    S.width = d->camera.width;
    S.height = d->camera.height;
    S.dof = d->camera.lens_radius > 1e-4f ? 1 : 0;
    S.lens_radius = d->camera.lens_radius;
    S.focal_distance = d->camera.focal_distance;
    S.lens_rtl = d->camera.lens_draw_order == NH_LENS_DRAWS_RTL ? 1 : 0;
    S.lens_pix = S.lens_lo = nullptr;
    S.lens_hi = nullptr;
    if (S.dof) {
        const nh::LensTables lt = nh::lens_tables(S.width, S.height);
        const nh::u64x2 *pix = nullptr, *lo = nullptr;
        if ((rc = upload(c, c->scene_bufs, lt.pix.data(), lt.pix.size(), &pix))) return rc;
        if ((rc = upload(c, c->scene_bufs, lt.lo.data(), lt.lo.size(), &lo))) return rc;
        if ((rc = upload(c, c->scene_bufs, lt.hi.data(), lt.hi.size(), &S.lens_hi))) return rc;
        S.lens_pix = reinterpret_cast<const ulonglong2 *>(pix);
        S.lens_lo = reinterpret_cast<const ulonglong2 *>(lo);
        HIP_TRY(c, hipStreamSynchronize(c->stream));
    }
    S.filter_radius = d->filter.radius;
    S.lookup = d->filter.lookup_factor;
    S.border = d->filter.border;
    std::memcpy(S.table, d->filter.table, sizeof(S.table));

    c->shapes.assign(d->shapes, d->shapes + d->n_shapes);
    c->shape_bsdf_type.clear();
    c->shape_bsdf_real.clear();
    unsigned types = 0;
    for (uint32_t i = 0; i < d->n_shapes; ++i) {
        const int t = d->shapes[i].bsdf < 0 ? NH_BSDF_DIFFUSE : d->bsdfs[d->shapes[i].bsdf].type;
        c->shape_bsdf_real.push_back(t);
        types |= 1u << t;
    }
    int disney_key = 0;
    for (int k : {NH_BSDF_MICROFACET, NH_BSDF_MIRROR, NH_BSDF_DIELECTRIC, NH_BSDF_DIFFUSE})
        if (!(types & (1u << k))) {
            disney_key = k;
            break;
        }
    for (int t : c->shape_bsdf_real) c->shape_bsdf_type.push_back(t == NH_BSDF_DISNEY ? disney_key : t);
    c->disney = (types & (1u << NH_BSDF_DISNEY)) != 0;
    c->disney = c->disney || !dx.empty();
    c->n_bsdf_types = __builtin_popcount(types);
    c->specular = (types & ((1u << NH_BSDF_MIRROR) | (1u << NH_BSDF_DIELECTRIC))) != 0;
    c->textured = false;
    for (uint32_t i = 0; i < d->n_bsdfs; ++i) c->textured = c->textured || d->bsdfs[i].albedo_texture != 0;
    c->normal_mapped = false;
    for (uint32_t i = 0; i < d->n_shapes; ++i) c->normal_mapped = c->normal_mapped || d->shapes[i].normal_map != 0;
    c->textured = c->textured || c->normal_mapped;
    c->diffuse_area = S.integrator == NH_INTEGRATOR_PATH_MIS && !c->textured && !S.dof && d->envmap < 0 &&
                      d->n_emitters > 0;
    for (uint32_t i = 0; i < d->n_bsdfs; ++i) c->diffuse_area = c->diffuse_area && d->bsdfs[i].type == NH_BSDF_DIFFUSE;
    for (uint32_t i = 0; i < d->n_emitters; ++i) {
        const nh_emitter &e = d->emitters[i];
        c->diffuse_area = c->diffuse_area && e.type == NH_EMITTER_AREA && e.shape >= 0 &&
                          (uint32_t)e.shape < d->n_shapes && ds[e.shape].ef_off >= 0;
    }
    for (uint32_t i = 0; i < d->n_shapes; ++i)
        c->diffuse_area = c->diffuse_area && d->shapes[i].emitter < (int32_t)d->n_emitters;
    c->h_shapes = ds;
    c->h_bsdfs = db;
    c->h_emitters = de;
    c->h_area_cdf.assign(d->area_cdf, d->area_cdf + d->n_area_cdf);
    c->n_emit_faces = (int)ef_tri.size();
    c->small_image = c->small_image_ref = nullptr;
    c->flat_image = nullptr;
    c->pair_kinds = false;
    c->V.assign(d->V, d->V + 3 * nv);
    c->F.assign(d->F, d->F + 3 * (size_t)d->n_faces);
    c->width = d->camera.width;
    c->height = d->camera.height;
    c->border = d->filter.border;
    c->filter = d->filter;
    c->n_emitters = (int)d->n_emitters;
    c->integrator = S.integrator;
    if (d->sampler != NH_SAMPLER_INDEPENDENT && d->sampler != NH_SAMPLER_ADAPTIVE)
        return fail(c, "unknown sampler"), NH_ERR_INVALID;
    c->sampler = d->sampler;
    c->adaptive_initial_uniform = std::max(1, (int)d->adaptive_initial_uniform);
    adaptive_release(c);
    photon_release(c);
    c->av_set = false;

    (void)hipFree(c->fb);
    c->fb = nullptr;
    c->fb_floats = 4 * (size_t)(c->width + 2 * c->border) * (size_t)(c->height + 2 * c->border);
    HIP_TRY(c, hipMalloc(&c->fb, c->fb_floats * sizeof(float)));
    HIP_TRY(c, hipMemsetAsync(c->fb, 0, c->fb_floats * sizeof(float), c->stream));
    auto rank = nh::spiral_rank(c->width, c->height, 32, c->nbx, c->nby);
    (void)hipFree(c->block_rank);
    HIP_TRY(c, hipMalloc(&c->block_rank, rank.size() * sizeof(int)));
    HIP_TRY(c, hipMemcpyAsync(c->block_rank, rank.data(), rank.size() * sizeof(int), hipMemcpyHostToDevice, c->stream));
    HIP_TRY(c, hipStreamSynchronize(c->stream));
    c->has_scene = true;
    return NH_OK;
}

static int build_small_image(nh_ctx *c, const nh::GpuBvh &g) {
    c->small_image = c->small_image_ref = nullptr;
    c->flat_image = nullptr;
    c->pair_kinds = false;
    for (int &v : c->small_tab) v = 0;
    const size_t scene_bytes = 16 * (size_t)(c->n_node_f4 + c->n_prim_f4) + 8 * (size_t)c->n_leaves;
    if (scene_bytes > kSmallSceneBytes) return NH_OK;
    const int n = c->n_prim_f4 / 3;
    const int leaves_f4 = (c->n_leaves + 1) / 2;
    const int pairs_off = c->n_node_f4 + c->n_prim_f4 + leaves_f4;
    const bool frames = n <= kSmallFramesMaxPrims;
    std::vector<float4> tab;
    if (c->diffuse_area) {
        std::vector<nhd::DShape> sh = c->h_shapes;
        std::vector<float> cdf;
        for (const nhd::DEmitter &e : c->h_emitters) {
            nhd::DShape &s = sh[e.shape];
            if ((size_t)s.pdf_off + s.n_faces + 1 > c->h_area_cdf.size()) return fail(c, "area CDF out of range"), NH_ERR_INVALID;
            const int off = (int)cdf.size();
            cdf.insert(cdf.end(), c->h_area_cdf.begin() + s.pdf_off, c->h_area_cdf.begin() + s.pdf_off + s.n_faces + 1);
            s.pdf_off = off;
        }
        cdf.resize((cdf.size() + 3) / 4 * 4, 0.f);
        const size_t bytes = sh.size() * sizeof(nhd::DShape) + c->h_bsdfs.size() * sizeof(nhd::DBsdf) +
                             c->h_emitters.size() * sizeof(nhd::DEmitter) + cdf.size() * sizeof(float) +
                             3 * (size_t)c->n_emit_faces * sizeof(float4);
        if (bytes <= kSmallTablesBytes) {
            static_assert(sizeof(nhd::DShape) % 16 == 0 && sizeof(nhd::DBsdf) % 16 == 0 && sizeof(nhd::DEmitter) % 16 == 0,
                          "table records are whole float4s");
            c->small_tab[0] = (int)(sh.size() * sizeof(nhd::DShape) / 16);
            c->small_tab[1] = (int)(c->h_bsdfs.size() * sizeof(nhd::DBsdf) / 16);
            c->small_tab[2] = (int)(c->h_emitters.size() * sizeof(nhd::DEmitter) / 16);
            c->small_tab[3] = (int)(cdf.size() / 4);
            c->small_tab[4] = 3 * c->n_emit_faces;
            tab.resize((size_t)c->small_tab[0] + c->small_tab[1] + c->small_tab[2] + c->small_tab[3]);
            char *w = reinterpret_cast<char *>(tab.data());
            std::memcpy(w, sh.data(), sh.size() * sizeof(nhd::DShape));
            w += sh.size() * sizeof(nhd::DShape);
            std::memcpy(w, c->h_bsdfs.data(), c->h_bsdfs.size() * sizeof(nhd::DBsdf));
            w += c->h_bsdfs.size() * sizeof(nhd::DBsdf);
            std::memcpy(w, c->h_emitters.data(), c->h_emitters.size() * sizeof(nhd::DEmitter));
            w += c->h_emitters.size() * sizeof(nhd::DEmitter);
            std::memcpy(w, cdf.data(), cdf.size() * sizeof(float));
        }
    }
    const int tab_f4 = (int)tab.size() + c->small_tab[4];
    const int pleaves_off = pairs_off + nhd::kPairF4 * n, tab_off = pleaves_off + leaves_f4;
    const int frames_off = tab_off + tab_f4;
    const size_t total = (size_t)frames_off + (frames ? 3 * (size_t)n : 0);
    const auto d2d = [&](float4 *dst, const void *src, size_t bytes) {
        return bytes ? hipMemcpyAsync(dst, src, bytes, hipMemcpyDeviceToDevice, c->stream) : hipSuccess;
    };
    const char *pk = std::getenv("NH_PAIR_KINDS");
    c->pair_kinds = n > 0 && !(pk && pk[0] == '0');
    for (int pass = 0; pass < (c->pair_kinds ? 2 : 1); ++pass) {
        const bool by_kind = c->pair_kinds && pass == 0;
        const nh::PairLayout pl = nh::pair_layout(g.leaves.data(), c->n_leaves, g.prims.data(), n, by_kind);
        float4 *img = nullptr;
        HIP_TRY(c, hipMalloc(&img, std::max<size_t>(total, 1) * sizeof(float4)));
        c->bvh_bufs.push_back(img);
        HIP_TRY(c, hipMemsetAsync(img, 0, std::max<size_t>(total, 1) * sizeof(float4), c->stream));
        HIP_TRY(c, d2d(img, c->tv.nodes, 16 * (size_t)c->n_node_f4));
        HIP_TRY(c, d2d(img + c->n_node_f4, c->tv.prims, 16 * (size_t)c->n_prim_f4));
        HIP_TRY(c, d2d(img + c->n_node_f4 + c->n_prim_f4, c->tv.leaves, 8 * (size_t)c->n_leaves));
        if (n > 0) {
            const nh::i2 *slots = nullptr;
            if (int rc = upload(c, c->bvh_bufs, pl.slots.data(), pl.slots.size(), &slots)) return rc;
            nh::launch_small_image(c->tv, c->n_prim_f4, reinterpret_cast<const int2 *>(slots), pairs_off,
                                   frames ? frames_off : -1, img, c->stream);
            HIP_TRY(c, hipGetLastError());
        }
        if (c->n_leaves > 0)
            HIP_TRY(c, hipMemcpyAsync(img + pleaves_off, pl.leaves.data(), 8 * (size_t)c->n_leaves, hipMemcpyHostToDevice,
                                      c->stream));
        if (!tab.empty()) {
            float4 *t = img + tab_off;
            HIP_TRY(c, hipMemcpyAsync(t, tab.data(), tab.size() * sizeof(float4), hipMemcpyHostToDevice, c->stream));
            HIP_TRY(c, d2d(t + tab.size(), c->S.emit_faces, 16 * (size_t)c->small_tab[4]));
        }
        HIP_TRY(c, hipStreamSynchronize(c->stream));
        (pass == 0 ? c->small_image : c->small_image_ref) = img;
    }
    const bool one_leaf = g.root_kind == 2 && c->n_leaves == 1;
    bool two_leaves = g.root_kind == 1 && c->n_node_f4 == 4 && c->n_leaves == 2;
    if (two_leaves) {
        int refs[2];
        std::memcpy(refs, &g.nodes[3].x, sizeof(refs));
        two_leaves = refs[0] == ~0 && refs[1] == ~1;
    }
    if (c->pair_kinds && (one_leaf || two_leaves)) {
        float boxes[18];
        for (int i = 0; i < 3; ++i) {
            boxes[i] = g.root_min[i];
            boxes[3 + i] = g.root_max[i];
        }
        if (two_leaves) {
            const nh::f4 n0 = g.nodes[0], n1 = g.nodes[1], n2 = g.nodes[2];
            const float lr[12] = {n0.x, n0.y, n0.z, n0.w, n1.x, n1.y, n1.z, n1.w, n2.x, n2.y, n2.z, n2.w};
            std::memcpy(boxes + 6, lr, sizeof(lr));
        } else {
            std::memcpy(boxes + 6, boxes, 6 * sizeof(float));
            std::memcpy(boxes + 12, boxes, 6 * sizeof(float));
        }
        const nh::PairLayout pl = nh::pair_layout(g.leaves.data(), c->n_leaves, g.prims.data(), n, true);
        const nh::FlatImage fi = nh::flat_image(boxes, g.leaves.data(), c->n_leaves, g.prims.data(), n, pl, nh::flat_trace_knob());
        if (fi.flat) {
            const nh::f4 *dev = nullptr;
            if (int rc = upload(c, c->bvh_bufs, fi.data.data(), fi.data.size(), &dev)) return rc;
            HIP_TRY(c, hipStreamSynchronize(c->stream));
            c->flat_image = reinterpret_cast<const float4 *>(dev);
        }
    }
    return NH_OK;
}

int nh_set_av_params(nh_ctx *c, const nh_av_params *params) {
    if (!c) return NH_ERR_INVALID;
    if (!params || std::isnan(params->length)) return fail(c, "nh_set_av_params: invalid av parameters"), NH_ERR_INVALID;
    if (!c->has_scene) return fail(c, "nh_set_av_params: no scene uploaded"), NH_ERR_STATE;
    HIP_TRY(c, hipSetDevice(c->device));
// ... 65 lines not shown
```

### optix-renderer_amd/csrc/nh_wavefront.hip

```cpp
#include "nh_dispatch.h"
#include "nh_internal.h"
#include "nh_shade.h"

#include <algorithm>
#include <cstdlib>

using namespace nhd;

#ifdef NH_DISNEY
namespace nh_disney {
#endif

namespace {

enum : int { F_DISCRETE = 1, F_NEE = 2, F_ZERO_COL = 4, F_ZNAN = 8, F_FIRST = 64 };
constexpr int kPidBits = 26;

__device__ __forceinline__ int wave_append(unsigned *counter, bool pred) {
    const unsigned long long mask = __ballot(pred);
    const int lane = threadIdx.x & 63;
    const int leader = __ffsll((long long)mask) - 1;
    unsigned base = 0;
    if (mask != 0ull && lane == leader) base = atomicAdd(counter, (unsigned)__popcll(mask));
    base = __shfl(base, leader < 0 ? 0 : leader, 64);
// ... 855 lines not shown
    const QView qv = queue_view(L.cnt_in);
    const int base = blockIdx.x * 256;
    if (base >= qv.n) return;
    if (threadIdx.x < kMatClasses) s_n[threadIdx.x] = 0u;
    const Traversal tv = stage_small_scene<true>(tv_g, L, lds_scene);
    const int shard = blockIdx.x & (kQueueShards - 1);
    const int q = base + (int)threadIdx.x;
    const WfBuf &B = L.st.buf[L.in_q];
    uint32_t *my_stk = stk + threadIdx.x;
    TravStats st_e{0, 0, 0}, st_s{0, 0, 0};
    unsigned long long q_e = 0, q_s = 0;
    bool cont = false;
    PState o;
    float4 hit_out = make_float4(0.f, 0.f, 0.f, 0.f);
    int cls = kMatClasses - 1;
    if (q < qv.n) {
        const int s = queue_slot(qv.pre, L.seg_cap, q);
        float4 hv;
        if (L.first) {
            float4 ro, rd;
            load_ray(S, L, B, q, s, ro, rd);
            Hit h;
            const bool live = rd.w >= ro.w;
            q_e += live ? 1 : 0;
            const bool found = live && trace<16, ORDERED, false, STATS, true>(tv, S, xyz(ro), xyz(rd), ro.w, rd.w, h,
                                                                        my_stk, 256, st_e);
            hv = make_float4(h.t, h.u, h.v, __int_as_float(found ? h.k : -1));
        } else {
            hv = B.hit[s];
        }
        bool nee = false;
        float4 so, sd;
        cont = shade_path(S, tv, L, MemState{B, s}, s, hv, o, nee, so, sd);
        if (cont) {
            if (nee) {
                Hit hs;
                ++q_s;
                if (!trace<16, ORDERED, true, STATS, true>(tv, S, xyz(so), xyz(sd), so.w, sd.w, hs, my_stk, 256, st_s)) {
                    o.li.x = o.li.x + o.pe.x;
                    o.li.y = o.li.y + o.pe.y;
                    o.li.z = o.li.z + o.pe.z;
                    o.thr.w = o.pe.w;
                } else if (o.flags & F_ZNAN) {
                    o.li.x = o.li.x + NAN;
                    o.li.y = o.li.y + NAN;
                    o.li.z = o.li.z + NAN;
                }
                o.flags &= ~(F_NEE | F_ZNAN);
            }
            Hit h;
            const bool live = o.rd.w >= o.ro.w;
            q_e += live ? 1 : 0;
#ifdef NH_EXPERIMENT_TRACE_TWICE
            {
                Hit h2;
                if (live && trace<16, ORDERED, false, STATS, true>(tv, S, xyz(o.ro), xyz(o.rd), o.ro.w, o.rd.w, h2, my_stk, 256, st_e))
                    o.rng ^= (uint64_t)(h2.k == -7);
            }
#endif
            const bool found = live && trace_next<16, ORDERED, STATS, true>(tv, S, __float_as_int(hv.w), xyz(o.ro),
                                                                      xyz(o.rd), o.ro.w, o.rd.w, h, my_stk, 256, st_e);
            hit_out = make_float4(h.t, h.u, h.v, __int_as_float(found ? h.k : -1));
            if (found) cls = prim_material(tv.prims[3 * h.k + 2]);
        }
    }
    int rank = 0;
    if (SORT) {
#pragma unroll
        for (int c = 0; c < kMatClasses; ++c) {
            const int r = wave_append(&s_n[c], cont && cls == c);
            if (cls == c) rank = r;
        }
    } else {
        cls = 0;
        rank = wave_append(&s_n[0], cont);
    }
    __syncthreads();
    if (threadIdx.x == 0) {
        unsigned tot = 0;
        for (int c = 0; c < kMatClasses; ++c) {
            s_off[c] = tot;
            tot += s_n[c];
        }
        s_base = tot ? atomicAdd(&L.cnt_out[shard * kCountStride], tot) : 0u;
    }
    __syncthreads();
    if (cont) {
        const WfBuf &Bo = L.st.buf[1 - L.in_q];
        const int slot = shard * L.seg_cap + (int)(s_base + s_off[cls]) + rank;
        store_state(Bo, slot, o);
        Bo.hit[slot] = hit_out;
    }
    if (STATS) {
        flush_trav_stats(stat_shard(L.counters), q_e, st_e);
        flush_trav_stats(stat_shard(L.counters) + kStatAny, q_s, st_s);
    }
}

__device__ __forceinline__ void store_post_head(const WfBuf &B, int s, const PathV &v, const Hit &h) {
    B.ray_o[s] = make_float4(v.org.x, v.org.y, v.org.z, 0.f);
    B.ray_d[s] = make_float4(v.d.x, v.d.y, v.d.z, __int_as_float((int)(((unsigned)(v.flags & 0x30) << kPidBits) | (unsigned)v.pid)));
    B.li[s] = make_float4(v.li.x, v.li.y, v.li.z, v.w_mats);
    B.thr[s] = make_float4(v.t.x, v.t.y, v.t.z, v.w_ems);
    B.rng[s] = v.rng.state;
    B.hit[s] = make_float4(h.t, h.u, h.v, __int_as_float(h.k));
}

struct RawState {
    float4 ro, rd, li4, th4, hv;
    uint64_t rng;
};
__device__ __forceinline__ RawState load_raw_state(const WfBuf &B, int s) {
    RawState r;
    r.ro = B.ray_o[s];
    r.rd = B.ray_d[s];
    r.li4 = B.li[s];
    r.th4 = B.thr[s];
    r.hv = B.hit[s];
    r.rng = B.rng[s];
    return r;
}

template <bool NMAP = true, class ST = DScene>
__device__ __forceinline__ void unpack_post_head(const DScene &S, const ST &T, const Traversal &tv, const WfLaunch &L,
                                                 const RawState &r, PathV &v, Hit &h, Its &its) {
    const float4 ro = r.ro, rd = r.rd, li4 = r.li4, th4 = r.th4, hv = r.hv;
    v.rng.state = r.rng;
    const int bits = __float_as_int(rd.w);
    v.flags = (int)((unsigned)bits >> kPidBits);
    v.pid = bits & ((1 << kPidBits) - 1);
    v.rng.inc = ((uint64_t)(L.s0 + v.pid / L.n_list) << 1u) | 1u;
    v.org = xyz(ro);
    v.d = xyz(rd);
    v.li = xyz(li4);
    v.w_mats = li4.w;
    v.t = xyz(th4);
    v.w_ems = th4.w;
    h.t = hv.x;
    h.u = hv.y;
    h.v = hv.z;
    h.k = __float_as_int(hv.w);
    hit_info<NMAP>(S, T.shapes, tv, h, v.org, v.d, its);
}

template <bool NMAP = true, class ST = DScene>
__device__ __forceinline__ void load_post_head(const DScene &S, const ST &T, const Traversal &tv, const WfLaunch &L,
                                               const WfBuf &B, int s, PathV &v, Hit &h, Its &its) {
    unpack_post_head<NMAP>(S, T, tv, L, load_raw_state(B, s), v, h, its);
}

template <bool ORDERED, bool STATS, bool NMAP = true, bool TRAIT = false, bool FLAT = false, class ST = DScene>
__device__ __forceinline__ bool first_vertex(const DScene &S, const ST &T, const Traversal &tv, const WfLaunch &L, int s,
                                             PathV &v, Hit &h, Its &its, uint32_t *stk, int stride, TravStats &st_e,
                                             unsigned long long &q_e, const float4 *__restrict__ flat = nullptr) {
    float4 ro, rd;
    float jx, jy;
#ifndef NH_AB_NO_PMASK
    constexpr bool MASKED = !STATS;
#else
    constexpr bool MASKED = false;
#endif
    unsigned long long cand = ~0ull;
    if constexpr (MASKED) {
        int blk;
        camera_sample<!TRAIT>(S, L, s, v.rng, ro, rd, jx, jy, &blk);
        if (L.pmask) cand = L.pmask[blk];
    } else {
        camera_sample<!TRAIT>(S, L, s, v.rng, ro, rd, jx, jy);
    }
    if (L.jit) L.jit[s] = make_float2(jx, jy);
    v.org = xyz(ro);
    v.d = xyz(rd);
    v.li = f3(0.f, 0.f, 0.f);
    v.t = f3(1.f, 1.f, 1.f);
    v.w_mats = 1.f;
    v.w_ems = 0.f;
    v.flags = F_FIRST;
    v.pid = s;
    const bool live = rd.w >= ro.w;
    q_e += live ? 1 : 0;
    bool found;
    if constexpr (FLAT)
        found = live && trace_flat<ORDERED, false, TRAIT, MASKED>(flat, S, v.org, v.d, ro.w, rd.w, h, cand);
    else
        found = live && trace<16, ORDERED, false, STATS, true, 1, TRAIT, MASKED>(tv, S, v.org, v.d, ro.w, rd.w, h, stk,
                                                                                stride, st_e, cand);
    if (!shade_head<NMAP, TRAIT>(S, T, tv, v, h, found, 0.f, its)) {
        write_radiance(L, v);
        return false;
    }
    return true;
}

struct TailClocks {
    unsigned long long c[4] = {0, 0, 0, 0};
    unsigned long long bounces = 0, max_bounces = 0;
    unsigned long long cc[4] = {0, 0, 0, 0}, coop_bounces = 0;
};

template <bool ORDERED, bool STATS, bool CLK = false, int G = 1, bool FULL = true, bool NMAP = FULL, bool TRAIT = false,
          bool LEAN = false, bool FLAT = false, class ST = DScene>
__device__ __forceinline__ bool rr_step(const DScene &S, const ST &T, const Traversal &tv, const WfLaunch &L, PathV &v, Its &its,
                                        Hit &h, uint32_t *stk, int stride, TravStats &st_e, TravStats &st_s,
                                        unsigned long long &q_e, unsigned long long &q_s, TailClocks *clk = nullptr,
                                        const float4 *__restrict__ flat = nullptr) {
    static_assert(!FLAT || (G == 1 && !STATS), "the flat traversal carries one ray per lane and counts nothing");
    const bool lead = G == 1 || (threadIdx.x & (G - 1)) == 0;
    PState o;
    bool nee = false;
    float4 so, sd;
    unsigned long long t0 = 0, t1 = 0;
    unsigned long long *cs = CLK ? (G > 1 ? clk->cc : clk->c) : nullptr;
    if constexpr (CLK) t0 = clock64();
    [[maybe_unused]] const uint64_t inc = v.rng.inc;
    shade_body<FULL, TRAIT>(S, T, tv, v, its, o, nee, so, sd);
    if constexpr (CLK) {
        t1 = clock64();
        if (lead) cs[0] += t1 - t0;
        t0 = t1;
    }
    if (nee) {
        Hit hs;
        if (lead) ++q_s;
        bool occluded;
        if constexpr (FLAT) occluded = trace_flat<ORDERED, true, TRAIT>(flat, S, xyz(so), xyz(sd), so.w, sd.w, hs);
        else occluded = trace<16, ORDERED, true, STATS, true, G, TRAIT>(tv, S, xyz(so), xyz(sd), so.w, sd.w, hs, stk, stride, st_s);
        if (!occluded) {
            o.li.x = o.li.x + o.pe.x;
            o.li.y = o.li.y + o.pe.y;
            o.li.z = o.li.z + o.pe.z;
            o.thr.w = o.pe.w;
        } else if (o.flags & F_ZNAN) {
            o.li.x = o.li.x + NAN;
            o.li.y = o.li.y + NAN;
            o.li.z = o.li.z + NAN;
        }
        o.flags &= ~(F_NEE | F_ZNAN);
    }
    if constexpr (CLK) {
        t1 = clock64();
        if (lead) cs[1] += t1 - t0;
        t0 = t1;
    }
    const bool live = o.rd.w >= o.ro.w;
    if (lead) q_e += live ? 1 : 0;
    bool found;
    if constexpr (FLAT)
        found = live && trace_next_flat<ORDERED, FULL, TRAIT>(flat, tv, S, h.k, xyz(o.ro), xyz(o.rd), o.ro.w, o.rd.w, h);
    else
        found = live && trace_next<16, ORDERED, STATS, true, G, FULL, TRAIT>(tv, S, h.k, xyz(o.ro), xyz(o.rd), o.ro.w,
                                                                            o.rd.w, h, stk, stride, st_e);
    if constexpr (CLK) {
        t1 = clock64();
        if (lead) cs[2] += t1 - t0;
        t0 = t1;
    }
    if constexpr (TRAIT) {
        v.org = xyz(o.ro);
        v.d = xyz(o.rd);
        v.li = xyz(o.li);
        v.w_mats = o.li.w;
        v.t = xyz(o.thr);
        v.w_ems = o.thr.w;
        v.rng.state = o.rng;
        v.rng.inc = inc;
        v.flags = o.flags;
        v.pid = o.pid;
    } else {
        v = path_of(L, o);
    }
    const bool alive = shade_head<NMAP, TRAIT, LEAN>(S, T, tv, v, h, found, o.pdfmat, its);
    if constexpr (CLK) {
        if (lead) cs[3] += clock64() - t0;
        if (lead) ++(G > 1 ? clk->coop_bounces : clk->bounces);
    }
    if (!alive) {
        if (lead) write_radiance(L, v);
        return false;
    }
    return true;
}

#ifndef NH_BOUNCE_TB
#define NH_BOUNCE_TB 256
#endif

template <bool ORDERED, bool STATS, bool FULL, bool NMAP = FULL, bool TRAIT = false, int BOUNCE = -1, bool FLAT = false,
          class ST = DScene>
__device__ __forceinline__ bool bounce_path(const DScene &S, const ST &T, const Traversal &tv, const WfLaunch &L, const QView &qv,
                                            int q, uint32_t *my_stk, PathV &v, Hit &h, TravStats &st_e,
                                            TravStats &st_s, unsigned long long &q_e, unsigned long long &q_s,
                                            TailClocks &clk, unsigned long long &c_load, const RawState *pre = nullptr,
                                            const float4 *__restrict__ flat = nullptr) {
    Its its;
    bool alive = true;
    unsigned long long t_ph = 0;
    if constexpr (STATS) t_ph = clock64();
    const bool first = BOUNCE < 0 ? L.first != 0 : BOUNCE == 0;
    if (first) {
        const int s = queue_slot(qv.pre, L.seg_cap, q);
        alive = first_vertex<ORDERED, STATS, NMAP, TRAIT, FLAT>(S, T, tv, L, s, v, h, its, my_stk, NH_BOUNCE_TB, st_e, q_e,
                                                                flat);
    } else if (BOUNCE == 1) {
        unpack_post_head<NMAP>(S, T, tv, L, *pre, v, h, its);
    } else {
        load_post_head<NMAP>(S, T, tv, L, L.st.buf[L.in_q], queue_slot(qv.pre, L.seg_cap, q), v, h, its);
    }
    if constexpr (STATS) c_load += clock64() - t_ph;
    return alive && rr_step<ORDERED, STATS, STATS, 1, FULL, NMAP, TRAIT, true, FLAT>(S, T, tv, L, v, its, h, my_stk, NH_BOUNCE_TB,
                                                                               st_e, st_s, q_e, q_s, &clk, flat);
}

template <bool ORDERED, bool STATS, bool SORT, bool FULL = true, bool NMAP = FULL, bool TRAIT = false, int BOUNCE = -1,
          bool FLAT = false>
__global__ __launch_bounds__(NH_BOUNCE_TB, NH_DZ_WAVES(true, NH_BOUNCE_WAVES)) void wf_bounce_rr(const DScene *__restrict__ Sp, Traversal tv_g,
                                                                     WfLaunch L, const float4 *__restrict__ flat) {
    static_assert(!(FLAT && STATS), "the counting kernels walk the tree");
    __shared__ uint32_t stk[FLAT ? 1 : 16 * NH_BOUNCE_TB];
    __shared__ unsigned s_n[kMatClasses], s_off[kMatClasses], s_base;
    extern __shared__ float4 lds_scene[];
    const QView qv = queue_view(L.cnt_in);
    const int base = blockIdx.x * NH_BOUNCE_TB;
    if (base >= qv.n) return;
    if (threadIdx.x < kMatClasses) s_n[threadIdx.x] = 0u;
    const DScene &S = *Sp;
    const int q = base + (int)threadIdx.x;
    [[maybe_unused]] RawState pre;
    if constexpr (BOUNCE == 1)
        if (q < qv.n) pre = load_raw_state(L.st.buf[L.in_q], queue_slot(qv.pre, L.seg_cap, q));
    const Traversal tv = stage_small_scene<true>(tv_g, L, lds_scene);
    const int shard = blockIdx.x & (kQueueShards - 1);
    uint32_t *my_stk = FLAT ? stk : stk + threadIdx.x;
    TravStats st_e{0, 0, 0}, st_s{0, 0, 0};
    unsigned long long q_e = 0, q_s = 0;
    bool cont = false;
    PathV v;
    Hit h;
    int cls = kMatClasses - 1;
    TailClocks clk;
    unsigned long long c_load = 0, c_store = 0, t_ph = 0;
    if (q < qv.n) {
        const auto &T = scene_tables<TRAIT && NH_TRAIT_TABLES>(S, L, lds_scene);
        cont = bounce_path<ORDERED, STATS, FULL, NMAP, TRAIT, BOUNCE, FLAT>(S, T, tv, L, qv, q, my_stk, v, h, st_e, st_s, q_e,
                                                                            q_s, clk, c_load, BOUNCE == 1 ? &pre : nullptr, flat);
        if (cont) cls = prim_material(tv.prims[3 * h.k + 2]);
        if constexpr (STATS) t_ph = clock64();
    }
    int rank = 0;
    if (SORT) {
#pragma unroll
        for (int c = 0; c < kMatClasses; ++c) {
            const int r = wave_append(&s_n[c], cont && cls == c);
            if (cls == c) rank = r;
        }
    } else {
        cls = 0;
        rank = wave_append(&s_n[0], cont);
    }
    __syncthreads();
    if (threadIdx.x == 0) {
        unsigned tot = 0;
        for (int c = 0; c < kMatClasses; ++c) {
            s_off[c] = tot;
            tot += s_n[c];
        }
        s_base = tot ? atomicAdd(&L.cnt_out[shard * kCountStride], tot) : 0u;
    }
    __syncthreads();
    if (cont) store_post_head(L.st.buf[1 - L.in_q], shard * L.seg_cap + (int)(s_base + s_off[cls]) + rank, v, h);
    if (STATS) {
        if (q < qv.n) c_store = clock64() - t_ph;
        flush_trav_stats(stat_shard(L.counters), q_e, st_e);
        flush_trav_stats(stat_shard(L.counters) + kStatAny, q_s, st_s);
        unsigned long long *dst = stat_shard(L.counters) + kStatBounceClk;
        for (int j = 0; j < 7; ++j) {
            unsigned long long x = j == 0 ? c_load : j < 5 ? clk.c[j - 1] : j == 5 ? c_store : clk.bounces;
            for (int off = 32; off > 0; off >>= 1) x += __shfl_xor(x, off, 64);
            if ((threadIdx.x & 63) == 0) atomicAdd(&dst[j], x);
        }
    }
}

constexpr int kTailCoopWords = 48;
template <bool ORDERED, bool STATS, int TB, int W, bool FULL = true, bool NMAP = FULL, bool TRAIT = false>
__global__ __launch_bounds__(TB) __attribute__((amdgpu_waves_per_eu(W))) void wf_tail_rr(
    const DScene *__restrict__ Sp, Traversal tv_g, WfLaunch L, int coop) {
    __shared__ uint32_t stk[16 * TB];
    __shared__ uint32_t xfer[TB == 64 ? 4 * kTailCoopWords : 1];
    extern __shared__ float4 lds_scene[];
    const DScene &S = *Sp;
    const Traversal tv = stage_small_scene<true>(tv_g, L, lds_scene);
    const QView qv = queue_view(L.cnt_in);
    const WfBuf &B = L.st.buf[L.in_q];
    TravStats st_e{0, 0, 0}, st_s{0, 0, 0};
    unsigned long long q_e = 0, q_s = 0;
    TailClocks clk;
    const int q = blockIdx.x * TB + threadIdx.x;
    bool alive = q < qv.n;
    PathV v;
    Hit h;
    Its its;
    unsigned long long nb = 0;
    const auto &T = scene_tables<TRAIT && NH_TRAIT_TABLES>(S, L, lds_scene);
    if (alive) load_post_head<NMAP>(S, T, tv, L, B, queue_slot(qv.pre, L.seg_cap, q), v, h, its);
    const bool can_coop = TB == 64 && coop == 16;
    for (;;) {
        const unsigned long long m = __ballot(alive);
        if (m == 0ull || (can_coop && __popcll(m) <= 4)) break;
        if (alive) {
            alive = rr_step<ORDERED, STATS, STATS, 1, FULL, NMAP, TRAIT>(S, T, tv, L, v, its, h, stk + threadIdx.x, TB, st_e,
                                                                   st_s, q_e, q_s, &clk);
            ++nb;
        }
    }
    if (STATS && !can_coop) clk.max_bounces = max(clk.max_bounces, nb);
    if constexpr (TB == 64) {
        const unsigned long long m = __ballot(alive);
        if (can_coop && m) {
            const int lane = threadIdx.x & 63;
            if (alive) {
                uint32_t *w = xfer + __popcll(m & ((1ull << lane) - 1ull)) * kTailCoopWords;
                static_assert(sizeof(PathV) + sizeof(Hit) + sizeof(Its) + 8 <= kTailCoopWords * 4, "xfer slot");
                __builtin_memcpy(w, &v, sizeof(PathV));
                __builtin_memcpy(w + sizeof(PathV) / 4, &h, sizeof(Hit));
                __builtin_memcpy(w + (sizeof(PathV) + sizeof(Hit)) / 4, &its, sizeof(Its));
                __builtin_memcpy(w + (sizeof(PathV) + sizeof(Hit) + sizeof(Its)) / 4, &nb, 8);
            }
            __syncthreads();
            const int g = lane >> 4;
            bool carry = g < __popcll(m);
            if (carry) {
                const uint32_t *w = xfer + g * kTailCoopWords;
                __builtin_memcpy(&v, w, sizeof(PathV));
                __builtin_memcpy(&h, w + sizeof(PathV) / 4, sizeof(Hit));
                __builtin_memcpy(&its, w + (sizeof(PathV) + sizeof(Hit)) / 4, sizeof(Its));
                __builtin_memcpy(&nb, w + (sizeof(PathV) + sizeof(Hit) + sizeof(Its)) / 4, 8);
            }
            while (__ballot(carry)) {
                if (carry) {
                    carry = rr_step<ORDERED, STATS, STATS, 16, FULL, NMAP, TRAIT>(S, T, tv, L, v, its, h, stk + threadIdx.x,
                                                                            TB, st_e, st_s, q_e, q_s, &clk);
                    ++nb;
                }
            }
            if (STATS && (lane & 15) == 0 && g < __popcll(m)) clk.max_bounces = max(clk.max_bounces, nb);
        } else if (STATS && can_coop) {
            clk.max_bounces = max(clk.max_bounces, nb);
        }
    }
    if (STATS) {
        flush_trav_stats(stat_shard(L.counters) + kStatTail, q_e, st_e);
        flush_trav_stats(stat_shard(L.counters) + kStatTailAny, q_s, st_s);
        unsigned long long *dst = stat_shard(L.counters) + kStatTailClk;
        for (int j = 0; j < 5; ++j) {
            unsigned long long x = j < 4 ? clk.c[j] : clk.bounces;
            unsigned long long y = j < 4 ? clk.cc[j] : clk.coop_bounces;
            for (int off = 32; off > 0; off >>= 1) {
                x += __shfl_xor(x, off, 64);
                y += __shfl_xor(y, off, 64);
            }
            if ((threadIdx.x & 63) == 0) {
                atomicAdd(&dst[j], x);
                atomicAdd(&dst[kStatTailCoopClk - kStatTailClk + j], y);
// ... 347 lines not shown
```

### optix-renderer_amd/host/gpu_layout.h

```cpp
#pragma once
#include <cstdint>
#include <string>
#include <vector>

#include "nori_hip.h"

namespace nh {

struct f4 {
    float x, y, z, w;
};
struct i2 {
    int x, y;
};
struct u64x2 {
    uint64_t x, y;
};

struct GpuBvh {
    std::vector<f4> nodes;
    std::vector<i2> leaves;
    std::vector<f4> prims;
    std::vector<f4> wide;
    std::vector<uint32_t> shape_offset;
    int root_kind = 0;
    float root_min[3] = {0.f, 0.f, 0.f}, root_max[3] = {0.f, 0.f, 0.f};
    uint32_t tree_depth = 0;
    int depth_wide = 1;
    int n_top = 0;
    int iso_spheres = 0;
};

int build_gpu_bvh(const nh_bvh_desc &b, const std::vector<nh_shape> &shapes, const std::vector<float> &V,
                  const std::vector<uint32_t> &F, const std::vector<int> &shape_mat_key,
                  const std::vector<int> &shape_bsdf_real, int wide_w, int top_k, GpuBvh &out, std::string &err);

std::vector<f4> collapse_wide(const std::vector<f4> &nodes, const std::vector<i2> &leaves, int &depth_out, int W = 4);
int number_top_first(std::vector<f4> &wide, const float root_min[3], const float root_max[3], int K, int W = 4);

std::vector<int> spiral_rank(int w, int h, int bs, int &nbx, int &nby);
std::vector<uint32_t> serial_ray_index(int w, int h, int bs);

struct LensTables {
    std::vector<u64x2> pix, lo;
    std::vector<uint64_t> hi;
};
LensTables lens_tables(int w, int h);

bool nee_finite(const nh_scene_desc *d);

bool primary_masks(const nh_camera &cam, const f4 *prims, int n_records, const int32_t *blocks, int n_blocks,
                   std::vector<uint64_t> &masks);
int primary_mask_pad(int width, int height);

struct PairLayout {
    std::vector<i2> slots, leaves;
};
PairLayout pair_layout(const i2 *leaves, int n_leaves, const f4 *prims, int n_records, bool by_kind);

struct FlatImage {
    bool flat = false;
    int box_equal = 0;
    std::vector<f4> data;
};
FlatImage flat_image(const float boxes[18], const i2 *leaves, int n_leaves, const f4 *prims, int n_records,
                     const PairLayout &pl, bool allowed);
bool flat_trace_knob();

}
```

### optix-renderer_amd/host/primary_masks.cpp

```cpp
#include <algorithm>
#include <cmath>
#include <cstring>

#include "gpu_layout.h"
#include "nh_host.h"

#include "../csrc/nh_layout.h"

namespace nh {

namespace {

struct V3 {
    double x, y, z;
};

bool invert4(const float *m, double inv[16]) {
    double a[4][8];
    for (int r = 0; r < 4; ++r)
        for (int c = 0; c < 4; ++c) {
            a[r][c] = m[4 * r + c];
            a[r][4 + c] = r == c ? 1.0 : 0.0;
        }
    for (int c = 0; c < 4; ++c) {
        int piv = c;
        for (int r = c + 1; r < 4; ++r)
            if (std::fabs(a[r][c]) > std::fabs(a[piv][c])) piv = r;
        if (!(std::fabs(a[piv][c]) > 0.0) || !std::isfinite(a[piv][c])) return false;
        for (int k = 0; k < 8; ++k) std::swap(a[c][k], a[piv][k]);
        const double s = 1.0 / a[c][c];
        for (int k = 0; k < 8; ++k) a[c][k] *= s;
        for (int r = 0; r < 4; ++r) {
            if (r == c) continue;
            const double f = a[r][c];
            for (int k = 0; k < 8; ++k) a[r][k] -= f * a[c][k];
        }
    }
    for (int r = 0; r < 4; ++r)
        for (int c = 0; c < 4; ++c) inv[4 * r + c] = a[r][4 + c];
    return true;
}

struct Projector {
    double w2c[16];
    double m[16];
    double width, height;

    bool raster(const V3 &p, double &rx, double &ry) const {
        double c[4];
        for (int r = 0; r < 4; ++r) c[r] = w2c[4 * r] * p.x + w2c[4 * r + 1] * p.y + w2c[4 * r + 2] * p.z + w2c[4 * r + 3];
        if (!(std::fabs(c[3]) > 0.0)) return false;
        const V3 q{c[0] / c[3], c[1] / c[3], c[2] / c[3]};
        const double dist = std::sqrt(q.x * q.x + q.y * q.y + q.z * q.z);
        if (!std::isfinite(dist) || !(q.z > 1e-3 * dist) || !(dist > 0.0)) return false;
        const double a0[3] = {m[0], m[4], m[8]}, a1[3] = {m[1], m[5], m[9]}, a2[3] = {-q.x, -q.y, -q.z};
        const double b[3] = {-m[3], -m[7], -m[11]};
        const auto det3 = [](const double *u, const double *v, const double *w) {
            return u[0] * (v[1] * w[2] - v[2] * w[1]) - v[0] * (u[1] * w[2] - u[2] * w[1]) +
                   w[0] * (u[1] * v[2] - u[2] * v[1]);
        };
        const double det = det3(a0, a1, a2);
        if (!(std::fabs(det) > 0.0)) return false;
        const double sx = det3(b, a1, a2) / det, sy = det3(a0, b, a2) / det, lambda = det3(a0, a1, b) / det;
        const double hw = m[12] * sx + m[13] * sy + m[15];
        if (!std::isfinite(sx) || !std::isfinite(sy) || !(lambda / hw > 0.0)) return false;
        rx = sx * width;
        ry = sy * height;
        return true;
    }
};

}

int primary_mask_pad(int width, int height) { return std::max(2, (std::max(width, height) + 255) / 256); }

bool primary_masks(const nh_camera &cam, const f4 *prims, int n_records, const int32_t *blocks, int n_blocks,
                   std::vector<uint64_t> &masks) {
    masks.clear();
    if (n_records < 0 || n_records > 64 || cam.lens_radius > 1e-4f || cam.width <= 0 || cam.height <= 0) return false;
    Projector pr;
    if (!invert4(cam.camera_to_world, pr.w2c)) return false;
    for (int i = 0; i < 16; ++i) pr.m[i] = cam.sample_to_camera[i];
    pr.width = cam.width;
    pr.height = cam.height;
    const float *cw = cam.camera_to_world;
    const V3 org{(double)cw[3] / cw[15], (double)cw[7] / cw[15], (double)cw[11] / cw[15]};

    struct Box {
        bool everywhere;
        double x0, y0, x1, y1;
    };
    std::vector<Box> box((size_t)n_records);
    for (int k = 0; k < n_records; ++k) {
        const f4 a = prims[3 * k], b = prims[3 * k + 1], c = prims[3 * k + 2];
        int bits;
        std::memcpy(&bits, &c.w, sizeof(bits));
        V3 pts[8];
        int n_pts;
        if (bits & nhd::kPrimSphere) {
            const double r = std::fabs((double)a.w);
            const double dx = a.x - org.x, dy = a.y - org.y, dz = a.z - org.z;
            const double far_d = std::sqrt(dx * dx + dy * dy + dz * dz) + r;
            const double g = r + 1e-3 * r + 64.0 * std::ldexp(1.0, -24) * far_d * far_d / std::max(r, 1e-300);
            n_pts = 8;
            for (int i = 0; i < 8; ++i)
                pts[i] = V3{a.x + (i & 1 ? g : -g), a.y + (i & 2 ? g : -g), a.z + (i & 4 ? g : -g)};
        } else {
            n_pts = 3;
            pts[0] = V3{a.x, a.y, a.z};
            pts[1] = V3{b.x, b.y, b.z};
            pts[2] = V3{c.x, c.y, c.z};
        }
        Box bx{false, INFINITY, INFINITY, -INFINITY, -INFINITY};
        for (int i = 0; i < n_pts && !bx.everywhere; ++i) {
            double rx, ry;
            if (!pr.raster(pts[i], rx, ry)) {
                bx.everywhere = true;
                break;
            }
            bx.x0 = std::min(bx.x0, rx);
            bx.x1 = std::max(bx.x1, rx);
            bx.y0 = std::min(bx.y0, ry);
            bx.y1 = std::max(bx.y1, ry);
        }
        box[(size_t)k] = bx;
    }

    const double pad = primary_mask_pad(cam.width, cam.height);
    const int nbx = (cam.width + 31) / 32, nby = (cam.height + 31) / 32;
    masks.assign((size_t)std::max(n_blocks, 0), 0);
    for (int i = 0; i < n_blocks; ++i) {
        const int bid = blocks[i];
        if (bid < 0 || bid >= nbx * nby) {
            masks[(size_t)i] = ~(uint64_t)0;
            continue;
        }
        const int bx = bid % nbx, by = bid / nbx;
        const double x0 = 32.0 * bx - pad, x1 = std::min(32.0 * bx + 32.0, (double)cam.width) + pad;
        const double y0 = 32.0 * by - pad, y1 = std::min(32.0 * by + 32.0, (double)cam.height) + pad;
        uint64_t mk = 0;
        for (int k = 0; k < n_records; ++k) {
            const Box &b = box[(size_t)k];
            const bool miss = !b.everywhere && (b.x1 < x0 || b.x0 > x1 || b.y1 < y0 || b.y0 > y1);
            if (!miss) mk |= (uint64_t)1 << k;
        }
        masks[(size_t)i] = mk;
    }
    return true;
}

}

extern "C" {

int nh_primary_masks(const nh_camera *camera, const float *records, int32_t n_records, const int32_t *blocks,
                     int32_t n_blocks, uint64_t *masks, int32_t *built) {
    if (!camera || !built || n_records < 0 || n_blocks < 0 || (n_records > 0 && !records) ||
        (n_blocks > 0 && (!blocks || !masks))) {
        nh::set_host_error("nh_primary_masks: invalid argument");
        return NH_ERR_INVALID;
    }
    static_assert(sizeof(nh::f4) == 4 * sizeof(float), "records are read as float4 triples");
    std::vector<uint64_t> m;
    *built = nh::primary_masks(*camera, reinterpret_cast<const nh::f4 *>(records), n_records, blocks, n_blocks, m) ? 1 : 0;
    if (*built && n_blocks > 0) std::memcpy(masks, m.data(), (size_t)n_blocks * sizeof(uint64_t));
    return NH_OK;
}

int32_t nh_primary_mask_pad(int32_t width, int32_t height) { return nh::primary_mask_pad(width, height); }

}
```

### optix-renderer_amd/nori_hip.py

```python
from __future__ import annotations

import ctypes as C
import os

import numpy as np

_HERE = os.path.dirname(os.path.abspath(__file__))
LIB_PATH = os.environ.get("NH_LIB_PATH") or os.path.join(_HERE, "lib", "libnori_hip.so")

from nh_env import raise_hw_queues

if not os.path.exists(LIB_PATH):
    raise ImportError(f"nori_hip: HIP library not built ({LIB_PATH}); run `make` or __graft_entry__.build()")
_lib = C.CDLL(LIB_PATH)

NH_OK = 0
SHAPE_MESH, SHAPE_SPHERE = 0, 1
BSDF_DIFFUSE, BSDF_MIRROR, BSDF_DIELECTRIC, BSDF_MICROFACET = 0, 1, 2, 3
BSDF_DISNEY = 4
BSDF_QUERY_EVAL, BSDF_QUERY_SAMPLE = 0, 1
EMITTER_AREA, EMITTER_POINT, EMITTER_ENVMAP = 0, 1, 2
EMITTER_SPOT, EMITTER_DIRECTIONAL = 3, 4
EMITTER_QUERY_SAMPLE, EMITTER_QUERY_EVAL, EMITTER_QUERY_PDF = 0, 1, 2
EMITTER_QUERY_SAMPLE_STRIDE, EMITTER_QUERY_IN_STRIDE = 16, 9
# ... 12 lines not shown
ADAPTIVE_MAX_SAMPLES = 133948
LENS_DRAWS_LTR, LENS_DRAWS_RTL = 0, 1

_f = C.c_float
_i32 = C.c_int32
_u32 = C.c_uint32
_fp = C.POINTER(C.c_float)
_u32p = C.POINTER(C.c_uint32)


class nh_shape(C.Structure):
    _fields_ = [("type", _i32), ("bsdf", _i32), ("emitter", _i32), ("v_offset", _u32), ("n_vertices", _u32),
                ("f_offset", _u32), ("n_faces", _u32), ("has_normals", _i32), ("has_uvs", _i32),
                ("center", _f * 3), ("radius", _f), ("bbox_min", _f * 3), ("bbox_max", _f * 3),
                ("pdf_offset", _u32), ("pdf_normalization", _f), ("normal_map", _u32)]


DISNEY_PARAMS = ("metallic", "subsurface", "specular", "roughness", "specular_tint", "anisotropic", "sheen",
                 "sheen_tint", "clearcoat", "clearcoat_gloss")
DISNEY_DEFAULTS = dict(zip(DISNEY_PARAMS, (0.0, 0.0, 0.5, 0.5, 0.0, 0.0, 0.0, 0.5, 0.0, 1.0)))


class nh_bsdf(C.Structure):
    _fields_ = [("type", _i32), ("albedo", _f * 3), ("alpha", _f), ("int_ior", _f), ("ext_ior", _f),
                ("kd", _f * 3), ("ks", _f), ("albedo_texture", _u32)] + [(n, _f) for n in DISNEY_PARAMS]


TEXTURE_CONSTANT, TEXTURE_CHECKERBOARD, TEXTURE_PNG = 0, 1, 2


class nh_texture(C.Structure):
    _fields_ = [("type", _i32), ("value1", _f * 3), ("value2", _f * 3), ("delta", _f * 2), ("scale", _f * 2),
                ("width", _i32), ("height", _i32), ("texel_offset", C.c_uint64), ("scale_u", _f), ("scale_v", _f),
                ("offset_u", _f), ("offset_v", _f), ("spherical", _i32), ("rotation", _f * 9), ("linear", _i32),
                ("intensity", _f), ("pad", _i32)]


class nh_emitter(C.Structure):
    _fields_ = [("type", _i32), ("shape", _i32), ("radiance", _f * 3), ("light_prob", _f),
                ("position", _f * 3), ("pad", _f)]


class nh_emitter_ext(C.Structure):
    _fields_ = [("direction", _f * 3), ("cos_total_width", _f), ("frame_s", _f * 3), ("cos_falloff_start", _f),
                ("frame_t", _f * 3), ("cos_theta_max", _f), ("frame_n", _f * 3), ("pad", _f)]


class nh_medium(C.Structure):
    _fields_ = [("type", _i32), ("mu_a", _f * 3), ("mu_s", _f * 3), ("mu_t", _f * 3), ("density", _f),
                ("phase", _i32), ("g", _f)]


class nh_camera(C.Structure):
    _fields_ = [("width", _i32), ("height", _i32), ("sample_to_camera", _f * 16), ("camera_to_world", _f * 16),
                ("inv_output_size", _f * 2), ("near_clip", _f), ("far_clip", _f), ("lens_radius", _f),
                ("focal_distance", _f), ("lens_draw_order", _i32)]


class nh_filter(C.Structure):
    _fields_ = [("radius", _f), ("border", _i32), ("lookup_factor", _f), ("table", _f * 33)]


class nh_envmap(C.Structure):
    _fields_ = [("width", _i32), ("height", _i32), ("rgba", _fp), ("radiance", _f * 3), ("scale_u", _f),
                ("scale_v", _f), ("offset_u", _f), ("offset_v", _f), ("spherical", _i32), ("constant", _i32),
                ("cdf", _fp), ("normalization", _f), ("rotation", _f * 9)]


class nh_denoiser(C.Structure):
    _fields_ = [("type", _i32), ("sigma_d", _f), ("sigma_vr", _f), ("range", _i32), ("amount", _i32)]


def simple_denoiser(sigma_d: float = 0.0, sigma_vr: float = 0.6, range: int = 1, amount: int = 1) -> nh_denoiser:
    eps = np.float32(1e-4)

    def clampf(v, lo, hi):
        v = np.float32(v)
        return float(lo if v < lo else (hi if v > hi else v))
    d = nh_denoiser()
    d.type = DENOISER_SIMPLE
    d.sigma_d = clampf(sigma_d, eps, np.float32(10))
    d.sigma_vr = clampf(sigma_vr, eps, np.float32(10))
    d.range = int(min(max(range, 0), 50))
    d.amount = int(min(max(amount, 1), 10))
    return d


class nh_scene_desc(C.Structure):
    _fields_ = [("camera", nh_camera), ("filter", nh_filter), ("integrator", _i32), ("sample_count", _i32),
                ("n_shapes", _u32), ("shapes", C.POINTER(nh_shape)), ("n_bsdfs", _u32),
                ("bsdfs", C.POINTER(nh_bsdf)), ("n_emitters", _u32), ("emitters", C.POINTER(nh_emitter)),
                ("emitter_cdf", _fp), ("envmap", _i32), ("n_vertices", _u32), ("V", _fp), ("N", _fp),
                ("UV", _fp), ("T", _fp), ("BT", _fp), ("n_faces", _u32), ("F", _u32p), ("n_area_cdf", _u32),
                ("area_cdf", _fp), ("env", nh_envmap), ("denoiser", nh_denoiser), ("n_textures", _u32),
                ("textures", C.POINTER(nh_texture)), ("n_texels", C.c_uint64), ("texels", _fp),
                ("normals_direction", _f * 3), ("emitter_ext", C.POINTER(nh_emitter_ext)),
                ("n_media", _u32), ("media", C.POINTER(nh_medium)), ("shape_medium", _u32p),
                ("ambient_medium", _u32), ("sampler", _i32), ("adaptive_initial_uniform", _i32)]


class nh_bvh_node(C.Structure):
    _fields_ = [("word0", _u32), ("word1", _u32), ("bbox_min", _f * 3), ("bbox_max", _f * 3)]


class nh_bvh_desc(C.Structure):
    _fields_ = [("n_nodes", _u32), ("nodes", C.POINTER(nh_bvh_node)), ("n_indices", _u32), ("indices", _u32p),
                ("n_shapes", _u32), ("shape_offset", _u32p), ("bbox_min", _f * 3), ("bbox_max", _f * 3),
                ("max_depth", _u32)]


class nh_ray_soa(C.Structure):
    _fields_ = [(n, _fp) for n in ("ox", "oy", "oz", "dx", "dy", "dz", "mint", "maxt")]


class nh_hit_soa(C.Structure):
    _fields_ = [("hit", C.POINTER(C.c_uint8)), ("t", _fp), ("u", _fp), ("v", _fp), ("prim", _u32p),
                ("shape", _u32p)]


class nh_render_req(C.Structure):
    _fields_ = [("sample_begin", _i32), ("sample_end", _i32), ("seed", C.c_uint64), ("n_blocks", _i32),
                ("blocks", C.POINTER(_i32)), ("mode", _i32), ("traversal", _i32), ("clear", _i32),
                ("collect_stats", _i32)]


class nh_adaptive_stats(C.Structure):
    _fields_ = [("total_samples", C.c_uint64), ("passes", C.c_uint64), ("max_passes", C.c_uint64),
                ("n_blocks", C.c_uint64)]


class nh_render_stats(C.Structure):
    _fields_ = [("kernel_ms_path", C.c_double), ("kernel_ms_splat", C.c_double), ("kernel_ms_extend", C.c_double),
                ("kernel_ms_shadow", C.c_double), ("kernel_ms_shade", C.c_double), ("launches_path", C.c_uint64),
                ("launches_splat", C.c_uint64), ("launches_extend", C.c_uint64), ("launches_shadow", C.c_uint64),
                ("launches_shade", C.c_uint64), ("samples", C.c_uint64), ("ray_queries", C.c_uint64),
                ("nodes_visited", C.c_uint64), ("boxes_tested", C.c_uint64), ("prims_tested", C.c_uint64),
                ("invalid_samples", C.c_uint64), ("shadow_queries", C.c_uint64),
                ("shadow_nodes_visited", C.c_uint64), ("shadow_boxes_tested", C.c_uint64),
                ("shadow_prims_tested", C.c_uint64), ("shade_state_bytes", C.c_uint64),
                ("extend_queue_bytes", C.c_uint64), ("shadow_queue_bytes", C.c_uint64),
                ("paths_shaded", C.c_uint64), ("kernel_ms_tail", C.c_double), ("launches_tail", C.c_uint64),
                ("node_bytes", C.c_uint64)] + [
        (n, C.c_uint64) for n in ("tail_queries", "tail_nodes_visited", "tail_boxes_tested", "tail_prims_tested",
                                  "tail_shadow_queries", "tail_shadow_nodes_visited", "tail_shadow_boxes_tested",
                                  "tail_shadow_prims_tested", "lds_scene", "fused_bounce", "comm_inits")] + [
        ("kernel_ms_denoise", C.c_double), ("launches_denoise", C.c_uint64), ("tails_async", C.c_uint64),
        ("pools_active", C.c_uint64), ("trace_fused", C.c_uint64)] + [
        (n, C.c_uint64) for n in ("tail_cycles_body", "tail_cycles_shadow", "tail_cycles_closest", "tail_cycles_head",
                                  "tail_bounces", "tail_max_bounces", "tail_coop_cycles_body",
                                  "tail_coop_cycles_shadow", "tail_coop_cycles_closest", "tail_coop_cycles_head",
                                  "tail_coop_bounces", "bounce_cycles_load", "bounce_cycles_body",
                                  "bounce_cycles_shadow", "bounce_cycles_closest", "bounce_cycles_head",
                                  "bounce_cycles_store", "bounce_bounces", "bounce_traits", "primary_masks",
                                  "pair_kinds", "flat_trace")]


def _sig(name, res, *args):
    fn = getattr(_lib, name)
    fn.restype = res
    fn.argtypes = list(args)
    return fn


_vp = C.c_void_p
_sig("nh_scene_load_xml", _i32, C.c_char_p, C.POINTER(_vp))
_sig("nh_scene_load_xml_index", _i32, C.c_char_p, _i32, C.POINTER(_vp))
_sig("nh_scene_get_desc", _i32, _vp, C.POINTER(nh_scene_desc))
_sig("nh_scene_set_resolution", _i32, _vp, _i32, _i32)
_sig("nh_scene_set_sample_count", _i32, _vp, _i32)
_sig("nh_scene_set_sampler", _i32, _vp, _i32, _i32)
_sig("nh_scene_set_bsdf", _i32, _vp, _u32, C.POINTER(nh_bsdf))
_sig("nh_scene_set_integrator", _i32, _vp, _i32)
_sig("nh_scene_add_texture", _u32, _vp, C.POINTER(nh_texture), _fp)
_sig("nh_scene_set_normal_map", _i32, _vp, _u32, _u32)
_sig("nh_scene_set_lens_draw_order", _i32, _vp, _i32)
_sig("nh_texture_decode", _i32, C.POINTER(C.c_uint8), C.c_uint64, _i32, _fp)
_sig("nh_scene_free", None, _vp)
_sig("nh_host_last_error", C.c_char_p)
_sig("nh_debug_transform", _i32, C.c_char_p, _fp, _i32)
_sig("nh_bvh_build", _i32, C.POINTER(nh_scene_desc), _i32, C.POINTER(_vp))
_sig("nh_bvh_get_desc", _i32, _vp, C.POINTER(nh_bvh_desc))
_sig("nh_bvh_free", None, _vp)
_sig("nh_primary_masks", _i32, C.POINTER(nh_camera), _fp, _i32, C.POINTER(_i32), _i32, C.POINTER(C.c_uint64),
     C.POINTER(_i32))
_sig("nh_primary_mask_pad", _i32, _i32, _i32)
_sig("nh_pair_layout", _i32, _fp, _i32, C.POINTER(_i32), _i32, _i32, C.POINTER(_i32), C.POINTER(_i32))
_sig("nh_flat_image", _i32, _fp, _i32, C.POINTER(_i32), _i32, _fp, _i32, _fp, _i32, C.POINTER(_i32), C.POINTER(_i32))
_sig("nh_framebuffer_to_rgb", _i32, _fp, _i32, _i32, _i32, _fp)
_sig("nh_write_pfm", _i32, C.c_char_p, _fp, _i32, _i32)
_sig("nh_image_load_png", _i32, C.c_char_p, C.POINTER(C.c_uint8), C.c_size_t, C.POINTER(_i32), C.POINTER(_i32))
_sig("nh_write_exr", _i32, C.c_char_p, _fp, _i32, _i32)
_sig("nh_write_png", _i32, C.c_char_p, _fp, _i32, _i32)
_sig("nh_rgb_to_ldr", _i32, _fp, _i32, _i32, C.POINTER(C.c_uint8))
_sig("nh_get_device_count", _i32, C.POINTER(C.c_int))
_sig("nh_create", _i32, C.c_int, C.POINTER(_vp))
_sig("nh_destroy", None, _vp)
_sig("nh_upload_scene", _i32, _vp, C.POINTER(nh_scene_desc))
_sig("nh_upload_bvh", _i32, _vp, C.POINTER(nh_bvh_desc))
_sig("nh_trace_rays", _i32, _vp, C.POINTER(nh_ray_soa), _i32, _i32, _i32, C.POINTER(nh_hit_soa))
_sig("nh_render", _i32, _vp, C.POINTER(nh_render_req))
_sig("nh_synchronize", _i32, _vp)
_sig("nh_get_framebuffer", _i32, _vp, _fp, C.c_size_t)
_sig("nh_framebuffer_device_ptr", _i32, _vp, C.POINTER(_vp), C.POINTER(C.c_size_t))
_sig("nh_get_stats", _i32, _vp, C.POINTER(nh_render_stats))
_sig("nh_reset_stats", _i32, _vp)
_sig("nh_get_adaptive_stats", _i32, _vp, C.POINTER(nh_adaptive_stats))
_sig("nh_get_adaptive_variance", _i32, _vp, _fp, C.c_size_t)
_sig("nh_reduce_framebuffers", _i32, C.POINTER(_vp), _i32, _i32)
_sig("nh_denoise", _i32, _vp, C.POINTER(nh_denoiser))
_sig("nh_denoise_image", _i32, _vp, _fp, _i32, _i32, _i32, C.POINTER(nh_denoiser))
_sig("nh_bsdf_query", _i32, _vp, C.POINTER(nh_bsdf), _fp, _i32, _i32, _fp, _fp, _fp, _fp, _fp, _fp, C.POINTER(_i32))
_sig("nh_emitter_query", _i32, _vp, _u32, _i32, _i32, _fp, _fp, _fp)
_sig("nh_medium_query", _i32, _vp, _u32, _i32, _i32, _fp, _fp)
_sig("nh_last_error", C.c_char_p, _vp)


class nh_test_desc(C.Structure):
    _fields_ = [("type", _i32), ("significance_level", _f), ("sample_count", _i32), ("n_angles", _u32),
                ("angles", _fp), ("n_references", _u32), ("references", _fp), ("n_scenes", _u32), ("n_bsdfs", _u32),
                ("bsdfs", C.POINTER(nh_bsdf))]


class nh_test_result(C.Structure):
    _fields_ = [("mean", C.c_double), ("variance", C.c_double), ("reference", C.c_double), ("p_value", C.c_double),
                ("accepted", _i32), ("sample_count", _i32), ("angle", _f), ("pad", _i32)]


TEST_TTEST, TEST_CHI2TEST = 0, 1
RADIANCE_QUERY_MAX = 1 << 24
_dp = C.POINTER(C.c_double)
_i32p = C.POINTER(_i32)
_sig("nh_test_load_xml", _i32, C.c_char_p, C.POINTER(_vp))
_sig("nh_test_get_desc", _i32, _vp, C.POINTER(nh_test_desc))
_sig("nh_test_free", None, _vp)
_sig("nh_students_t_test", _i32, C.c_double, C.c_double, C.c_double, _i32, C.c_double, _i32, _i32p, _dp)
_sig("nh_radiance_query", _i32, _vp, C.c_uint64, _i32, _i32p, _i32p, _fp, _fp, _fp)
_sig("nh_ttest_scene", _i32, _vp, C.c_uint64, C.c_int64, _i32, _dp, _dp, _fp)
_sig("nh_ttest_bsdf", _i32, _vp, C.POINTER(nh_bsdf), _fp, _f, C.c_uint64, _i32, _dp, _dp, _fp)
_sig("nh_test_run", _i32, C.c_int, C.c_char_p, C.c_uint64, C.POINTER(nh_test_result), _i32, _i32p)


INTEGRATOR_PHOTONMAPPER = 9
EMITTER_QUERY_SAMPLE_PHOTON, EMITTER_QUERY_PHOTON_STRIDE = 3, 12
PHOTON_QUERY_CODEC, PHOTON_QUERY_GATHER = 0, 1
PHOTON_STREAM = 1 << 32
PHOTON_DEFAULT_BATCH = 1 << 18


class nh_photon_params(C.Structure):
    _fields_ = [("photon_count", _i32), ("photon_radius", _f)]


class nh_photon_stats(C.Structure):
    _fields_ = [("stored", _i32), ("emitted", _i32), ("radius", _f), ("cell_size", _f),
                ("occupied_cells", C.c_uint64)]


_u8p = C.POINTER(C.c_uint8)
_sig("nh_scene_get_photon_params", _i32, _vp, C.POINTER(nh_photon_params))
_sig("nh_scene_set_photon_params", _i32, _vp, C.POINTER(nh_photon_params))
_sig("nh_photon_tables", _i32, _fp, _fp, _fp, _fp, _fp)
_sig("nh_photon_map_build", _i32, _vp, C.POINTER(nh_photon_params), C.c_uint64, _i32)
_sig("nh_get_photon_stats", _i32, _vp, C.POINTER(nh_photon_stats))
_sig("nh_get_photons", _i32, _vp, _i32, _i32, _fp, _fp, _fp, _u8p, _i32p, _i32p)
_sig("nh_photon_query", _i32, _vp, _i32, _i32, _fp, _u8p, _i32p, _fp)


INTEGRATOR_AV, INTEGRATOR_ENVMAPTESTER = 10, 11


class nh_av_params(C.Structure):
    _fields_ = [("length", _f)]


_sig("nh_scene_get_av_params", _i32, _vp, C.POINTER(nh_av_params))
_sig("nh_scene_set_av_params", _i32, _vp, C.POINTER(nh_av_params))
_sig("nh_set_av_params", _i32, _vp, C.POINTER(nh_av_params))


def photon_tables() -> dict:
    t = {k: np.zeros(256, np.float32) for k in ("cos_theta", "sin_theta", "cos_phi", "sin_phi", "exp")}
    _host_check(_lib.nh_photon_tables(*[_fptr(t[k]) for k in ("cos_theta", "sin_theta", "cos_phi", "sin_phi", "exp")]),
                "photon_tables")
    return t


lib = _lib
_hip_used = False


def configure_runtime(min_hw_queues: int = 8) -> int:
    if _hip_used:
        raise RuntimeError("configure_runtime: the HIP runtime is already initialised in this process")
    return raise_hw_queues(min_hw_queues)


class NoriError(RuntimeError):
    pass


def _fptr(a):
    return a.ctypes.data_as(_fp)


def _host_check(rc, what):
    if rc != NH_OK:
        raise NoriError(f"{what}: {_lib.nh_host_last_error().decode()}")


class Scene:

    def __init__(self, path: str, index: int = 0):
        h = _vp()
        _host_check(_lib.nh_scene_load_xml_index(path.encode(), index, C.byref(h)), f"load {path}")
        self._h = h
        self.path = path

    def __del__(self):
        if getattr(self, "_h", None):
            _lib.nh_scene_free(self._h)
            self._h = None

    @property
    def desc(self) -> nh_scene_desc:
        d = nh_scene_desc()
        _host_check(_lib.nh_scene_get_desc(self._h, C.byref(d)), "get_desc")
        return d

    def set_resolution(self, w: int, h: int):
        _host_check(_lib.nh_scene_set_resolution(self._h, w, h), "set_resolution")

    def set_sample_count(self, spp: int):
        _host_check(_lib.nh_scene_set_sample_count(self._h, spp), "set_sample_count")

    def set_sampler(self, type: int, initial_uniform: int = 2):
        _host_check(_lib.nh_scene_set_sampler(self._h, type, initial_uniform), "set_sampler")

    def set_integrator(self, integ: int):
# ... 317 lines not shown
        p, n = _vp(), C.c_size_t()
        self._check(_lib.nh_framebuffer_device_ptr(self._h, C.byref(p), C.byref(n)), "framebuffer_device_ptr")
        return p.value, n.value

    def stats(self) -> dict:
        s = nh_render_stats()
        self._check(_lib.nh_get_stats(self._h, C.byref(s)), "get_stats")
        return {f: getattr(s, f) for f, _ in s._fields_}

    def adaptive_stats(self) -> dict:
        s = nh_adaptive_stats()
        self._check(_lib.nh_get_adaptive_stats(self._h, C.byref(s)), "get_adaptive_stats")
        return {f: int(getattr(s, f)) for f, _ in s._fields_}

    def adaptive_variance(self) -> np.ndarray:
        out = np.zeros((self.scene.height, self.scene.width), np.float32)
        self._check(_lib.nh_get_adaptive_variance(self._h, _fptr(out), out.size), "get_adaptive_variance")
        return out

    def reset_stats(self):
        self._check(_lib.nh_reset_stats(self._h), "reset_stats")

    def denoise(self, params: nh_denoiser = None):
        if params is None:
            params = self.scene.desc.denoiser
        self._check(_lib.nh_denoise(self._h, C.byref(params)), "denoise")

    def denoise_image(self, rgbw: np.ndarray, border: int, params: nh_denoiser) -> np.ndarray:
        out = np.array(rgbw, dtype=np.float32, order="C", copy=True)
        h, w = out.shape[0] - 2 * border, out.shape[1] - 2 * border
        self._check(_lib.nh_denoise_image(self._h, _fptr(out), w, h, border, C.byref(params)), "denoise_image")
        return out

    def bsdf_query(self, bsdf: nh_bsdf, wi: np.ndarray, wo: np.ndarray = None, sample: np.ndarray = None,
                   albedo=None) -> dict:
        if (wo is None) == (sample is None):
            raise ValueError("bsdf_query: give either wo (eval) or sample (sample)")
        wi = np.ascontiguousarray(wi, dtype=np.float32).reshape(-1, 3)
        n = len(wi)
        out = {"value": np.zeros((n, 3), np.float32), "pdf": np.zeros(n, np.float32)}
        alb = None if albedo is None else np.ascontiguousarray(albedo, dtype=np.float32).reshape(3)
        if wo is not None:
            wo = np.ascontiguousarray(wo, dtype=np.float32).reshape(n, 3)
            rc = _lib.nh_bsdf_query(self._h, C.byref(bsdf), None if alb is None else _fptr(alb), BSDF_QUERY_EVAL, n,
                                    _fptr(wi), _fptr(wo), None, None, _fptr(out["value"]), _fptr(out["pdf"]), None)
        else:
            sample = np.ascontiguousarray(sample, dtype=np.float32).reshape(n, 2)
            out["wo"] = np.zeros((n, 3), np.float32)
            out["measure"] = np.zeros(n, np.int32)
            rc = _lib.nh_bsdf_query(self._h, C.byref(bsdf), None if alb is None else _fptr(alb), BSDF_QUERY_SAMPLE, n,
                                    _fptr(wi), None, _fptr(sample), _fptr(out["wo"]), _fptr(out["value"]),
                                    _fptr(out["pdf"]), out["measure"].ctypes.data_as(C.POINTER(_i32)))
        self._check(rc, "bsdf_query")
        return out

    def emitter_query(self, emitter: int, ref: np.ndarray, sample: np.ndarray = None, wi: np.ndarray = None,
                      p: np.ndarray = None, n: np.ndarray = None, mode: int = None) -> dict:
        if (sample is None) == (wi is None):
            raise ValueError("emitter_query: give either sample (sample) or wi (eval and pdf)")
        ref = np.ascontiguousarray(ref, dtype=np.float32).reshape(-1, 3)
        m = len(ref)

        def call(md, inp, out):
            self._check(_lib.nh_emitter_query(self._h, emitter, md, m, _fptr(ref), _fptr(inp), _fptr(out)),
                        "emitter_query")
            return out
        if sample is not None:
            sample = np.ascontiguousarray(sample, dtype=np.float32).reshape(m, 2)
            o = call(EMITTER_QUERY_SAMPLE, sample, np.zeros((m, EMITTER_QUERY_SAMPLE_STRIDE), np.float32))
            return {"value": o[:, 0:3].copy(), "wi": o[:, 3:6].copy(), "pdf": o[:, 6].copy(), "o": o[:, 7:10].copy(),
                    "d": o[:, 10:13].copy(), "mint": o[:, 13].copy(), "maxt": o[:, 14].copy()}
        inp = np.zeros((m, EMITTER_QUERY_IN_STRIDE), np.float32)
        inp[:, 0:3] = np.asarray(wi, np.float32).reshape(m, 3)
        if p is not None:
            inp[:, 3:6] = np.asarray(p, np.float32).reshape(m, 3)
        if n is not None:
            inp[:, 6:9] = np.asarray(n, np.float32).reshape(m, 3)
        out = {}
        if mode in (None, EMITTER_QUERY_EVAL):
            out["value"] = call(EMITTER_QUERY_EVAL, inp, np.zeros((m, 3), np.float32))
        if mode in (None, EMITTER_QUERY_PDF):
            out["pdf"] = call(EMITTER_QUERY_PDF, inp, np.zeros(m, np.float32))
        return out

    def medium_query(self, medium: int, mode: int, inp: np.ndarray) -> np.ndarray:
        n_in, n_out = {MEDIUM_QUERY_FREE_PATH: (2, 2), MEDIUM_QUERY_TRANSMITTANCE: (6, 3),
                       MEDIUM_QUERY_PHASE_SAMPLE: (2, 4), MEDIUM_QUERY_PHASE_PDF: (3, 1)}[mode]
        inp = np.ascontiguousarray(inp, dtype=np.float32).reshape(-1, n_in)
        out = np.zeros((len(inp), n_out), np.float32)
        self._check(_lib.nh_medium_query(self._h, medium, mode, len(inp), _fptr(inp), _fptr(out)), "medium_query")
        return out[:, 0] if n_out == 1 else out

    def radiance_query(self, pixel, sample, seed: int = 0, pixel_sample=None) -> dict:
        pixel = np.ascontiguousarray(pixel, dtype=np.int32).ravel()
        sample = np.ascontiguousarray(np.broadcast_to(np.asarray(sample, dtype=np.int32), pixel.shape))
        n = len(pixel)
        ps = None if pixel_sample is None else np.ascontiguousarray(pixel_sample, dtype=np.float32).reshape(n, 2)
        out = {"rgb": np.zeros((n, 3), np.float32), "jitter": np.zeros((n, 2), np.float32)}
        self._check(_lib.nh_radiance_query(self._h, seed, n, pixel.ctypes.data_as(_i32p), sample.ctypes.data_as(_i32p),
                                           None if ps is None else _fptr(ps), _fptr(out["rgb"]), _fptr(out["jitter"])),
                    "radiance_query")
        return out

    def ttest_scene(self, n: int, seed: int = 0, first: int = 0, luminance: bool = False):
        m, v = C.c_double(0.0), C.c_double(0.0)
        lum = np.zeros(max(n, 0), np.float32) if luminance else None
        self._check(_lib.nh_ttest_scene(self._h, seed, first, n, C.byref(m), C.byref(v),
                                        None if lum is None else _fptr(lum)), "ttest_scene")
        return (m.value, v.value, lum) if luminance else (m.value, v.value)

    def ttest_bsdf(self, bsdf: nh_bsdf, angle_deg: float, n: int, first_draw: int = 0, albedo=None,
                   luminance: bool = False):
        m, v = C.c_double(0.0), C.c_double(0.0)
        lum = np.zeros(max(n, 0), np.float32) if luminance else None
        alb = None if albedo is None else np.ascontiguousarray(albedo, dtype=np.float32).reshape(3)
        self._check(_lib.nh_ttest_bsdf(self._h, C.byref(bsdf), None if alb is None else _fptr(alb), angle_deg, first_draw,
                                       n, C.byref(m), C.byref(v), None if lum is None else _fptr(lum)), "ttest_bsdf")
        return (m.value, v.value, lum) if luminance else (m.value, v.value)

    def trace(self, o: np.ndarray, d: np.ndarray, mint: np.ndarray, maxt: np.ndarray, any_hit=False,
              traversal: int = TRAVERSAL_REFERENCE) -> dict:
        n = len(o)
        cols = [np.ascontiguousarray(x, dtype=np.float32) for x in (o[:, 0], o[:, 1], o[:, 2], d[:, 0], d[:, 1],
                                                                     d[:, 2], mint, maxt)]
        r = nh_ray_soa(*[_fptr(c) for c in cols])
        res = {"hit": np.zeros(n, np.uint8), "t": np.zeros(n, np.float32), "u": np.zeros(n, np.float32),
               "v": np.zeros(n, np.float32), "prim": np.zeros(n, np.uint32), "shape": np.zeros(n, np.uint32)}
        h = nh_hit_soa(res["hit"].ctypes.data_as(C.POINTER(C.c_uint8)), _fptr(res["t"]), _fptr(res["u"]),
                       _fptr(res["v"]), res["prim"].ctypes.data_as(_u32p), res["shape"].ctypes.data_as(_u32p))
        self._check(_lib.nh_trace_rays(self._h, C.byref(r), n, int(any_hit), traversal, C.byref(h)), "trace_rays")
        return res


def tile_shard(width: int, height: int, world: int, rank: int) -> list:
    nbx, nby = (width + 31) // 32, (height + 31) // 32
    return [b for b in range(nbx * nby) if b % world == rank]


def primary_mask_pad(width: int, height: int) -> int:
    return int(_lib.nh_primary_mask_pad(width, height))


def primary_masks(camera: nh_camera, records: np.ndarray, blocks):
    rec = np.ascontiguousarray(records, dtype=np.float32).reshape(-1, 12)
    blk = np.ascontiguousarray(blocks, dtype=np.int32).ravel()
    out = np.zeros(len(blk), np.uint64)
    built = _i32(0)
    _host_check(_lib.nh_primary_masks(C.byref(camera), _fptr(rec), len(rec), blk.ctypes.data_as(C.POINTER(_i32)),
                                      len(blk), out.ctypes.data_as(C.POINTER(C.c_uint64)), C.byref(built)),
                "primary_masks")
    return out if built.value else None


def pair_layout(records: np.ndarray, leaves, by_kind: bool = True):
    rec = np.ascontiguousarray(records, dtype=np.float32).reshape(-1, 12)
    lv = np.ascontiguousarray(leaves, dtype=np.int32).reshape(-1, 2)
    slots, lp = np.zeros((len(rec), 2), np.int32), np.zeros((len(lv), 3), np.int32)
    ip = C.POINTER(_i32)
    _host_check(_lib.nh_pair_layout(_fptr(rec), len(rec), lv.ctypes.data_as(ip), len(lv), 1 if by_kind else 0,
                                    slots.ctypes.data_as(ip), lp.ctypes.data_as(ip)), "pair_layout")
    return slots, lp


def flat_image(records: np.ndarray, leaves, boxes, allowed: bool = True):
    rec = np.ascontiguousarray(records, dtype=np.float32).reshape(-1, 12)
    lv = np.ascontiguousarray(leaves, dtype=np.int32).reshape(-1, 2)
    bx = np.ascontiguousarray(boxes, dtype=np.float32).ravel()
    assert bx.size == 18
    cap = 6 + 6 * 16
    img, n, eq = np.zeros((cap, 4), np.float32), _i32(0), _i32(0)
    _host_check(_lib.nh_flat_image(_fptr(rec), len(rec), lv.ctypes.data_as(C.POINTER(_i32)), len(lv), _fptr(bx),
                                   1 if allowed else 0, _fptr(img), cap, C.byref(n), C.byref(eq)), "flat_image")
    return (img[:n.value].copy() if n.value else None), int(eq.value)


def reduce_framebuffers(ctxs, root: int = 0):
    arr = (_vp * len(ctxs))(*[c._h for c in ctxs])
    rc = _lib.nh_reduce_framebuffers(arr, len(ctxs), root)
    if rc != NH_OK:
        raise NoriError(f"nh_reduce_framebuffers failed ({rc})")


def to_rgb(rgbw: np.ndarray, border: int) -> np.ndarray:
    h, w = rgbw.shape[0] - 2 * border, rgbw.shape[1] - 2 * border
    src = np.ascontiguousarray(rgbw, dtype=np.float32)
    out = np.zeros((h, w, 3), np.float32)
    rc = _lib.nh_framebuffer_to_rgb(_fptr(src), w, h, border, _fptr(out))
    if rc != NH_OK:
        raise NoriError("framebuffer_to_rgb failed")
    return out


def write_exr(path: str, rgb: np.ndarray):
    rgb = np.ascontiguousarray(rgb, dtype=np.float32)
    _host_check(_lib.nh_write_exr(path.encode(), _fptr(rgb), rgb.shape[1], rgb.shape[0]), "write_exr")


def write_png(path: str, rgb: np.ndarray):
    rgb = np.ascontiguousarray(rgb, dtype=np.float32)
    _host_check(_lib.nh_write_png(path.encode(), _fptr(rgb), rgb.shape[1], rgb.shape[0]), "write_png")


def rgb_to_ldr(rgb: np.ndarray) -> np.ndarray:
    rgb = np.ascontiguousarray(rgb, dtype=np.float32)
    out = np.empty(rgb.shape[:2] + (3,), np.uint8)
    _host_check(_lib.nh_rgb_to_ldr(_fptr(rgb), rgb.shape[1], rgb.shape[0],
                                   out.ctypes.data_as(C.POINTER(C.c_uint8))), "rgb_to_ldr")
    return out


def write_pfm(path: str, rgb: np.ndarray):
    rgb = np.ascontiguousarray(rgb, dtype=np.float32)
    _host_check(_lib.nh_write_pfm(path.encode(), _fptr(rgb), rgb.shape[1], rgb.shape[0]), "write_pfm")


def load_png(path: str) -> np.ndarray:
    w, h = _i32(), _i32()
    _host_check(_lib.nh_image_load_png(path.encode(), None, 0, C.byref(w), C.byref(h)), "load_png")
    out = np.zeros((h.value, w.value, 4), np.uint8)
    _host_check(_lib.nh_image_load_png(path.encode(), out.ctypes.data_as(C.POINTER(C.c_uint8)), out.nbytes,
                                       C.byref(w), C.byref(h)), "load_png")
    return out
```

Baseline: 8764 Msamples/s.

## Cull shadow-ray candidate records per screen block using host-built emitter masks

Adds a host-side geometric analysis that works out, for each 32x32 screen block, which scene records could occlude a shadow ray from a primary hit toward the area emitters. The result is uploaded as a per-block 64-bit mask. In the first bounce, lanes OR together the masks of their wave's blocks and pass that as a candidate set to the shadow trace, so records that cannot occlude are skipped. This adds host precomputation, a shared-memory block index, and a wave-level ballot loop, and its correctness depends on conservative floating-point bounds in the analysis.

New measurement: 8859 Msamples/s, median of 6. 1.1% higher.

```diff
diff --git a/include/nori_hip.h b/include/nori_hip.h
--- a/include/nori_hip.h
+++ b/include/nori_hip.h
@@ -278,6 +278,7 @@
     uint64_t primary_masks;
     uint64_t pair_kinds;
     uint64_t flat_trace;
+    uint64_t shadow_masks;
 } nh_render_stats;
 
 typedef struct nh_scene nh_scene;
@@ -319,6 +320,11 @@
 int nh_primary_masks(const nh_camera *camera, const float *records, int32_t n_records, const int32_t *blocks,
                      int32_t n_blocks, uint64_t *masks, int32_t *built);
 int32_t nh_primary_mask_pad(int32_t width, int32_t height);
+
+int nh_shadow_emitter_faces(const nh_scene_desc *scene, float *faces, int32_t cap_faces, int32_t *n_faces);
+int nh_shadow_masks(const nh_camera *camera, const float *records, int32_t n_records, const float *emit_faces,
+                    int32_t n_emit_faces, const int32_t *blocks, int32_t n_blocks, uint64_t *emitter_mask,
+                    uint64_t *masks, int32_t *built);
 
 int nh_pair_layout(const float *records, int32_t n_records, const int32_t *leaves, int32_t n_leaves, int32_t by_kind,
                    int32_t *slots, int32_t *leaf_pairs);
diff --git a/optix-renderer_amd/csrc/nh_api.hip b/optix-renderer_amd/csrc/nh_api.hip
--- a/optix-renderer_amd/csrc/nh_api.hip
+++ b/optix-renderer_amd/csrc/nh_api.hip
@@ -69,6 +69,7 @@
     (void)hipFree(c->rec);
     c->px.release();
     (void)hipFree(c->pmask);
+    (void)hipFree(c->smask);
     (void)hipFree(c->block_rank);
     (void)hipFree(c->staging);
     free_all(c->av_bufs);
diff --git a/optix-renderer_amd/csrc/nh_ctx.h b/optix-renderer_amd/csrc/nh_ctx.h
--- a/optix-renderer_amd/csrc/nh_ctx.h
+++ b/optix-renderer_amd/csrc/nh_ctx.h
@@ -177,6 +177,8 @@
     std::vector<float> h_prims;
     unsigned long long *pmask = nullptr;
     bool pmask_known = false;
+    std::vector<float> h_emit_tris;
+    unsigned long long *smask = nullptr;
     float *fb = nullptr;
     size_t fb_floats = 0;
     float *rec = nullptr;
@@ -198,7 +200,9 @@
 
 inline void drop_primary_masks(nh_ctx *c) {
     (void)hipFree(c->pmask);
+    (void)hipFree(c->smask);
     c->pmask = nullptr;
+    c->smask = nullptr;
     c->pmask_known = false;
 }
 
diff --git a/optix-renderer_amd/csrc/nh_internal.h b/optix-renderer_amd/csrc/nh_internal.h
--- a/optix-renderer_amd/csrc/nh_internal.h
+++ b/optix-renderer_amd/csrc/nh_internal.h
@@ -173,6 +173,7 @@
     unsigned long long *counters;
     const unsigned long long *pmask;
     int pmask_nbx;
+    const unsigned long long *smask;
     const float4 *flat;
 };
 constexpr int kPersistentBlocks = 256 * 16;
diff --git a/optix-renderer_amd/csrc/nh_pipeline.hip b/optix-renderer_amd/csrc/nh_pipeline.hip
--- a/optix-renderer_amd/csrc/nh_pipeline.hip
+++ b/optix-renderer_amd/csrc/nh_pipeline.hip
@@ -217,6 +217,10 @@
     L.pmask = masks ? c->pmask : nullptr;
     L.pmask_nbx = c->nbx;
     c->stats.primary_masks = masks ? 1 : 0;
+    const char *sm = std::getenv("NH_SHADOW_MASKS");
+    const bool shadow = p.rr && c->smask && !j.stats && !(sm && (sm[0] == '0' || sm[0] == '1'));
+    L.smask = shadow ? c->smask : nullptr;
+    c->stats.shadow_masks = shadow ? 2 : 0;
     c->stats.pair_kinds = p.fused && c->pair_kinds && !j.stats ? 1 : 0;
     const bool flat = p.rr && c->flat_image && c->pair_kinds && !j.stats && !c->disney;
     L.flat = flat ? c->flat_image : nullptr;
@@ -699,6 +703,20 @@
         HIP_TRY(c, e);
     }
     c->pmask = d;
+    const int n_faces = (int)(c->h_emit_tris.size() / 9);
+    const nh::f4 *recs = reinterpret_cast<const nh::f4 *>(c->h_prims.data());
+    const int n_recs = (int)(c->h_prims.size() / 12);
+    if (n_faces == 0 ||
+        !nh::shadow_block_masks(c->camera, recs, n_recs, c->h_emit_tris.data(), n_faces, blocks.data(), (int)blocks.size(), m))
+        return NH_OK;
+    for (size_t i = 0; i < blocks.size(); ++i) grid[(size_t)blocks[i]] = m[i];
+    HIP_TRY(c, hipMalloc(&d, std::max<size_t>(grid.size(), 1) * sizeof(unsigned long long)));
+    const hipError_t e2 = hipMemcpy(d, grid.data(), grid.size() * sizeof(unsigned long long), hipMemcpyHostToDevice);
+    if (e2 != hipSuccess) {
+        (void)hipFree(d);
+        HIP_TRY(c, e2);
+    }
+    c->smask = d;
     return NH_OK;
 }
 
@@ -819,6 +837,7 @@
     c->stats.node_bytes = 64;
     if (av_split && av_wide(c, q)) c->stats.node_bytes = 16 * nhd::kWideF4 * (c->wide_w / 4);
     c->stats.primary_masks = 0;
+    c->stats.shadow_masks = 0;
     c->stats.pair_kinds = 0;
     c->stats.flat_trace = 0;
     c->stats.trace_fused = 0;
diff --git a/optix-renderer_amd/csrc/nh_upload.hip b/optix-renderer_amd/csrc/nh_upload.hip
--- a/optix-renderer_amd/csrc/nh_upload.hip
+++ b/optix-renderer_amd/csrc/nh_upload.hip
@@ -385,6 +385,8 @@
     c->h_emitters = de;
     c->h_area_cdf.assign(d->area_cdf, d->area_cdf + d->n_area_cdf);
     c->n_emit_faces = (int)ef_tri.size();
+    c->h_emit_tris = nh::shadow_emitter_faces(*d);
+    if (c->h_emit_tris.size() != 9 * ef_tri.size()) c->h_emit_tris.clear();
     c->small_image = c->small_image_ref = nullptr;
     c->flat_image = nullptr;
     c->pair_kinds = false;
diff --git a/optix-renderer_amd/csrc/nh_wavefront.hip b/optix-renderer_amd/csrc/nh_wavefront.hip
--- a/optix-renderer_amd/csrc/nh_wavefront.hip
+++ b/optix-renderer_amd/csrc/nh_wavefront.hip
@@ -1031,7 +1031,8 @@
 template <bool ORDERED, bool STATS, bool NMAP = true, bool TRAIT = false, bool FLAT = false, class ST = DScene>
 __device__ __forceinline__ bool first_vertex(const DScene &S, const ST &T, const Traversal &tv, const WfLaunch &L, int s,
                                              PathV &v, Hit &h, Its &its, uint32_t *stk, int stride, TravStats &st_e,
-                                             unsigned long long &q_e, const float4 *__restrict__ flat = nullptr) {
+                                             unsigned long long &q_e, const float4 *__restrict__ flat = nullptr,
+                                             int *sblk = nullptr) {
     float4 ro, rd;
     float jx, jy;
 #ifndef NH_AB_NO_PMASK
@@ -1040,10 +1041,11 @@
     constexpr bool MASKED = false;
 #endif
     unsigned long long cand = ~0ull;
-    if constexpr (MASKED) {
+    if constexpr (!STATS) {
         int blk;
         camera_sample<!TRAIT>(S, L, s, v.rng, ro, rd, jx, jy, &blk);
-        if (L.pmask) cand = L.pmask[blk];
+        if (MASKED && L.pmask) cand = L.pmask[blk];
+        if (sblk) *sblk = blk;
     } else {
         camera_sample<!TRAIT>(S, L, s, v.rng, ro, rd, jx, jy);
     }
@@ -1078,12 +1080,13 @@
 };
 
 template <bool ORDERED, bool STATS, bool CLK = false, int G = 1, bool FULL = true, bool NMAP = FULL, bool TRAIT = false,
-          bool LEAN = false, bool FLAT = false, class ST = DScene>
+          bool LEAN = false, bool FLAT = false, bool SMASK = false, class ST = DScene>
 __device__ __forceinline__ bool rr_step(const DScene &S, const ST &T, const Traversal &tv, const WfLaunch &L, PathV &v, Its &its,
                                         Hit &h, uint32_t *stk, int stride, TravStats &st_e, TravStats &st_s,
                                         unsigned long long &q_e, unsigned long long &q_s, TailClocks *clk = nullptr,
-                                        const float4 *__restrict__ flat = nullptr) {
+                                        const float4 *__restrict__ flat = nullptr, const int *s_blk = nullptr) {
     static_assert(!FLAT || (G == 1 && !STATS), "the flat traversal carries one ray per lane and counts nothing");
+    static_assert(!SMASK || (G == 1 && !STATS), "the counting and cooperative queries test every record");
     const bool lead = G == 1 || (threadIdx.x & (G - 1)) == 0;
     PState o;
     bool nee = false;
@@ -1102,8 +1105,24 @@
         Hit hs;
         if (lead) ++q_s;
         bool occluded;
-        if constexpr (FLAT) occluded = trace_flat<ORDERED, true, TRAIT>(flat, S, xyz(so), xyz(sd), so.w, sd.w, hs);
-        else occluded = trace<16, ORDERED, true, STATS, true, G, TRAIT>(tv, S, xyz(so), xyz(sd), so.w, sd.w, hs, stk, stride, st_s);
+        [[maybe_unused]] unsigned long long scand = ~0ull;
+        if constexpr (SMASK) {
+            if (s_blk && L.smask) {
+                const int sblk = s_blk[threadIdx.x];
+                unsigned long long acc = 0;
+                for (unsigned long long rem = __ballot(1); rem;) {
+                    const int b = __builtin_amdgcn_readlane(sblk, __ffsll((long long)rem) - 1);
+                    acc |= L.smask[b];
+                    rem &= ~__ballot(sblk == b);
+                }
+                scand = acc;
+            }
+        }
+        if constexpr (FLAT)
+            occluded = trace_flat<ORDERED, true, TRAIT, SMASK>(flat, S, xyz(so), xyz(sd), so.w, sd.w, hs, scand);
+        else
+            occluded = trace<16, ORDERED, true, STATS, true, G, TRAIT, SMASK>(tv, S, xyz(so), xyz(sd), so.w, sd.w, hs, stk,
+                                                                             stride, st_s, scand);
         if (!occluded) {
             o.li.x = o.li.x + o.pe.x;
             o.li.y = o.li.y + o.pe.y;
@@ -1176,18 +1195,23 @@
     unsigned long long t_ph = 0;
     if constexpr (STATS) t_ph = clock64();
     const bool first = BOUNCE < 0 ? L.first != 0 : BOUNCE == 0;
+    __shared__ int s_blk[NH_BOUNCE_TB];
+    bool sblk = false;
     if (first) {
         const int s = queue_slot(qv.pre, L.seg_cap, q);
         alive = first_vertex<ORDERED, STATS, NMAP, TRAIT, FLAT>(S, T, tv, L, s, v, h, its, my_stk, NH_BOUNCE_TB, st_e, q_e,
-                                                                flat);
+                                                                flat, &s_blk[threadIdx.x]);
+        sblk = true;
     } else if (BOUNCE == 1) {
         unpack_post_head<NMAP>(S, T, tv, L, *pre, v, h, its);
     } else {
         load_post_head<NMAP>(S, T, tv, L, L.st.buf[L.in_q], queue_slot(qv.pre, L.seg_cap, q), v, h, its);
     }
     if constexpr (STATS) c_load += clock64() - t_ph;
-    return alive && rr_step<ORDERED, STATS, STATS, 1, FULL, NMAP, TRAIT, true, FLAT>(S, T, tv, L, v, its, h, my_stk, NH_BOUNCE_TB,
-                                                                               st_e, st_s, q_e, q_s, &clk, flat);
+    constexpr bool SMASK = !STATS && BOUNCE != 1;
+    return alive && rr_step<ORDERED, STATS, STATS, 1, FULL, NMAP, TRAIT, true, FLAT, SMASK>(S, T, tv, L, v, its, h, my_stk,
+                                                                                       NH_BOUNCE_TB, st_e, st_s, q_e, q_s,
+                                                                                       &clk, flat, sblk ? s_blk : nullptr);
 }
 
 template <bool ORDERED, bool STATS, bool SORT, bool FULL = true, bool NMAP = FULL, bool TRAIT = false, int BOUNCE = -1,
diff --git a/optix-renderer_amd/host/gpu_layout.h b/optix-renderer_amd/host/gpu_layout.h
--- a/optix-renderer_amd/host/gpu_layout.h
+++ b/optix-renderer_amd/host/gpu_layout.h
@@ -52,6 +52,12 @@
 bool primary_masks(const nh_camera &cam, const f4 *prims, int n_records, const int32_t *blocks, int n_blocks,
                    std::vector<uint64_t> &masks);
 int primary_mask_pad(int width, int height);
+bool primary_mask_in_front(const nh_camera &cam, const f4 *prims, int n_records, std::vector<char> &in_front);
+
+uint64_t shadow_emitter_mask(const f4 *prims, int n_records, const float *emit_faces, int n_faces);
+std::vector<float> shadow_emitter_faces(const nh_scene_desc &d);
+bool shadow_block_masks(const nh_camera &cam, const f4 *prims, int n_records, const float *emit_faces, int n_faces,
+                        const int32_t *blocks, int n_blocks, std::vector<uint64_t> &masks);
 
 struct PairLayout {
     std::vector<i2> slots, leaves;
diff --git a/optix-renderer_amd/host/primary_masks.cpp b/optix-renderer_amd/host/primary_masks.cpp
--- a/optix-renderer_amd/host/primary_masks.cpp
+++ b/optix-renderer_amd/host/primary_masks.cpp
@@ -74,9 +74,14 @@
 
 int primary_mask_pad(int width, int height) { return std::max(2, (std::max(width, height) + 255) / 256); }
 
-bool primary_masks(const nh_camera &cam, const f4 *prims, int n_records, const int32_t *blocks, int n_blocks,
-                   std::vector<uint64_t> &masks) {
-    masks.clear();
+namespace {
+
+struct Box {
+    bool everywhere;
+    double x0, y0, x1, y1;
+};
+
+bool record_boxes(const nh_camera &cam, const f4 *prims, int n_records, std::vector<Box> &box) {
     if (n_records < 0 || n_records > 64 || cam.lens_radius > 1e-4f || cam.width <= 0 || cam.height <= 0) return false;
     Projector pr;
     if (!invert4(cam.camera_to_world, pr.w2c)) return false;
@@ -86,11 +91,7 @@
     const float *cw = cam.camera_to_world;
     const V3 org{(double)cw[3] / cw[15], (double)cw[7] / cw[15], (double)cw[11] / cw[15]};
 
-    struct Box {
-        bool everywhere;
-        double x0, y0, x1, y1;
-    };
-    std::vector<Box> box((size_t)n_records);
+    box.assign((size_t)n_records, Box{});
     for (int k = 0; k < n_records; ++k) {
         const f4 a = prims[3 * k], b = prims[3 * k + 1], c = prims[3 * k + 2];
         int bits;
@@ -125,6 +126,24 @@
         }
         box[(size_t)k] = bx;
     }
+    return true;
+}
+
+}
+
+bool primary_mask_in_front(const nh_camera &cam, const f4 *prims, int n_records, std::vector<char> &in_front) {
+    std::vector<Box> box;
+    in_front.clear();
+    if (!record_boxes(cam, prims, n_records, box)) return false;
+    for (const Box &b : box) in_front.push_back(b.everywhere ? 0 : 1);
+    return true;
+}
+
+bool primary_masks(const nh_camera &cam, const f4 *prims, int n_records, const int32_t *blocks, int n_blocks,
+                   std::vector<uint64_t> &masks) {
+    masks.clear();
+    std::vector<Box> box;
+    if (!record_boxes(cam, prims, n_records, box)) return false;
 
     const double pad = primary_mask_pad(cam.width, cam.height);
     const int nbx = (cam.width + 31) / 32, nby = (cam.height + 31) / 32;
diff --git a/optix-renderer_amd/host/shadow_masks.cpp b/optix-renderer_amd/host/shadow_masks.cpp
--- /dev/null
+++ b/optix-renderer_amd/host/shadow_masks.cpp
@@ -0,0 +1,368 @@
+#include <algorithm>
+#include <cmath>
+#include <cstring>
+
+#include "gpu_layout.h"
+#include "nh_host.h"
+
+#include "../csrc/nh_layout.h"
+
+namespace nh {
+
+namespace {
+
+struct V3 {
+    double x, y, z;
+};
+V3 operator-(V3 a, V3 b) { return V3{a.x - b.x, a.y - b.y, a.z - b.z}; }
+V3 operator+(V3 a, V3 b) { return V3{a.x + b.x, a.y + b.y, a.z + b.z}; }
+V3 operator*(double s, V3 a) { return V3{s * a.x, s * a.y, s * a.z}; }
+double dot(V3 a, V3 b) { return a.x * b.x + a.y * b.y + a.z * b.z; }
+V3 cross(V3 a, V3 b) { return V3{a.y * b.z - a.z * b.y, a.z * b.x - a.x * b.z, a.x * b.y - a.y * b.x}; }
+double norm(V3 a) { return std::sqrt(dot(a, a)); }
+
+const double kU = std::ldexp(1.0, -24);
+
+struct AABB {
+    V3 lo{INFINITY, INFINITY, INFINITY}, hi{-INFINITY, -INFINITY, -INFINITY};
+    void add(V3 p) {
+        lo = V3{std::min(lo.x, p.x), std::min(lo.y, p.y), std::min(lo.z, p.z)};
+        hi = V3{std::max(hi.x, p.x), std::max(hi.y, p.y), std::max(hi.z, p.z)};
+    }
+    bool empty() const { return !(lo.x <= hi.x); }
+    bool meets(const AABB &o, double g) const {
+        return lo.x - g <= o.hi.x && o.lo.x <= hi.x + g && lo.y - g <= o.hi.y && o.lo.y <= hi.y + g &&
+               lo.z - g <= o.hi.z && o.lo.z <= hi.z + g;
+    }
+};
+
+struct Face {
+    V3 p[3], n;
+};
+
+struct Record {
+    bool sphere;
+    V3 p[3];
+    double r;
+    V3 n;
+    double sin_t;
+    double len;
+    double rho;
+    double grown;
+    AABB box;
+};
+
+double sphere_grown(double r, double far_d) {
+    const double g = r + 1e-3 * r + 64.0 * kU * far_d * far_d / std::max(r, 1e-300);
+    return 1.5 * g;
+}
+
+struct Analysis {
+    bool ok = false;
+    std::vector<Face> faces;
+    std::vector<Record> rec;
+    AABB scene, emit;
+    double eps_o = 0, eta = 0, d_e = 0, m = 0;
+    uint64_t emitter_word = ~(uint64_t)0;
+};
+
+Analysis analyse(const f4 *prims, int n_records, const float *emit_faces, int n_faces) {
+    Analysis A;
+    if (n_records <= 0 || n_records > 64 || n_faces <= 0 || !emit_faces) return A;
+    double min_sin = 1.0, max_abs = 0.0;
+    for (int f = 0; f < n_faces; ++f) {
+        Face F;
+        for (int j = 0; j < 3; ++j) {
+            F.p[j] = V3{emit_faces[9 * f + 3 * j], emit_faces[9 * f + 3 * j + 1], emit_faces[9 * f + 3 * j + 2]};
+            A.emit.add(F.p[j]);
+            max_abs = std::max({max_abs, std::fabs(F.p[j].x), std::fabs(F.p[j].y), std::fabs(F.p[j].z)});
+        }
+        const V3 e1 = F.p[1] - F.p[0], e2 = F.p[2] - F.p[0], c = cross(e1, e2);
+        const double a2 = norm(c), l = norm(e1) * norm(e2);
+        if (!(a2 > 0.0) || !std::isfinite(a2) || !(l > 0.0)) return A;
+        min_sin = std::min(min_sin, a2 / l);
+        F.n = (1.0 / a2) * c;
+        A.faces.push_back(F);
+    }
+    if (!(min_sin >= 1.0 / 16)) return A;
+    A.rec.resize((size_t)n_records);
+    for (int k = 0; k < n_records; ++k) {
+        const f4 a = prims[3 * k], b = prims[3 * k + 1], c = prims[3 * k + 2];
+        int bits;
+        std::memcpy(&bits, &c.w, sizeof(bits));
+        Record &R = A.rec[(size_t)k];
+        R.sphere = (bits & nhd::kPrimSphere) != 0;
+        R.p[0] = V3{a.x, a.y, a.z};
+        R.rho = INFINITY;
+        if (R.sphere) {
+            R.r = std::fabs((double)a.w);
+            R.box.add(V3{a.x - R.r, a.y - R.r, a.z - R.r});
+            R.box.add(V3{a.x + R.r, a.y + R.r, a.z + R.r});
+        } else {
+            R.p[1] = V3{b.x, b.y, b.z};
+            R.p[2] = V3{c.x, c.y, c.z};
+            for (int j = 0; j < 3; ++j) R.box.add(R.p[j]);
+        }
+        A.scene.add(R.box.lo);
+        A.scene.add(R.box.hi);
+    }
+    if (!std::isfinite(A.scene.lo.x + A.scene.lo.y + A.scene.lo.z + A.scene.hi.x + A.scene.hi.y + A.scene.hi.z)) return A;
+    const V3 ext = A.scene.hi - A.scene.lo;
+    A.m = 1e-4 * std::max({ext.x, ext.y, ext.z});
+    for (const Face &F : A.faces)
+        for (int j = 0; j < 3; ++j)
+            for (int i = 0; i < 8; ++i) {
+                const V3 q{i & 1 ? A.scene.hi.x : A.scene.lo.x, i & 2 ? A.scene.hi.y : A.scene.lo.y,
+                           i & 4 ? A.scene.hi.z : A.scene.lo.z};
+                A.d_e = std::max(A.d_e, norm(q - F.p[j]));
+            }
+    A.eps_o = 8.0 * kU * max_abs;
+    A.eta = 32.0 * kU / min_sin;
+    for (Record &R : A.rec) {
+        if (R.sphere) {
+            double far_d = 0;
+            for (const Face &F : A.faces)
+                for (int j = 0; j < 3; ++j) far_d = std::max(far_d, norm(F.p[j] - R.p[0]) + R.r);
+            R.grown = sphere_grown(R.r, far_d);
+            R.rho = R.grown - R.r;
+            continue;
+        }
+        const V3 e1 = R.p[1] - R.p[0], e2 = R.p[2] - R.p[0], c = cross(e1, e2);
+        const double a2 = norm(c), l1 = norm(e1), l2 = norm(e2);
+        R.n = V3{0, 0, 0};
+        R.sin_t = 0;
+        R.len = std::max(l1, l2);
+        if (!(a2 > 0.0) || !(l1 * l2 > 0.0)) continue;
+        R.n = (1.0 / a2) * c;
+        R.sin_t = a2 / (l1 * l2);
+        double s = INFINITY, reach = 0;
+        int side = 0;
+        bool one_side = true;
+        for (const Face &F : A.faces)
+            for (int j = 0; j < 3; ++j) {
+                const double h = dot(R.n, F.p[j] - R.p[0]);
+                const int sg = h > 0 ? 1 : h < 0 ? -1 : 0;
+                if (sg == 0 || (side && sg != side)) one_side = false;
+                side = sg;
+                s = std::min(s, std::fabs(h));
+                for (int i = 0; i < 3; ++i) reach = std::max(reach, norm(F.p[j] - R.p[i]));
+            }
+        s -= A.eps_o;
+        if (!one_side || !(s > 0.0) || !(32.0 * kU * reach <= s * R.sin_t)) continue;
+        R.rho = 64.0 * kU * (reach + R.len + A.d_e) * A.d_e / (s * R.sin_t);
+    }
+    A.ok = true;
+    uint64_t word = n_records < 64 ? ~(uint64_t)0 << n_records : 0;
+    for (int k = 0; k < n_records; ++k) {
+        const Record &R = A.rec[(size_t)k];
+        bool behind = std::isfinite(R.rho);
+        const double delta = A.eps_o + 1.01 * A.d_e * A.eta + (R.sphere ? 0.0 : R.rho);
+        for (size_t f = 0; f < A.faces.size() && behind; ++f) {
+            const Face &F = A.faces[f];
+            if (R.sphere) {
+                for (int i = 0; i < 8 && behind; ++i) {
+                    const V3 q{R.p[0].x + (i & 1 ? R.grown : -R.grown), R.p[0].y + (i & 2 ? R.grown : -R.grown),
+                               R.p[0].z + (i & 4 ? R.grown : -R.grown)};
+                    behind = dot(F.n, q - F.p[0]) <= -delta;
+                }
+            } else {
+                for (int j = 0; j < 3 && behind; ++j) behind = dot(F.n, R.p[j] - F.p[0]) <= -delta;
+            }
+        }
+        if (!behind) word |= (uint64_t)1 << k;
+    }
+    A.emitter_word = word;
+    return A;
+}
+
+void clip(const std::vector<V3> &in, V3 org, V3 n, std::vector<V3> &out) {
+    out.clear();
+    const size_t k = in.size();
+    for (size_t i = 0; i < k; ++i) {
+        const V3 a = in[i], b = in[(i + 1) % k];
+        const double da = dot(n, a - org), db = dot(n, b - org);
+        if (da >= 0) out.push_back(a);
+        if ((da >= 0) != (db >= 0)) out.push_back(a + (da / (da - db)) * (b - a));
+    }
+}
+
+}
+
+std::vector<float> shadow_emitter_faces(const nh_scene_desc &d) {
+    std::vector<float> out;
+    if (d.n_emitters == 0) return out;
+    for (uint32_t i = 0; i < d.n_emitters; ++i) {
+        const nh_emitter &e = d.emitters[i];
+        if (e.type != NH_EMITTER_AREA || e.shape < 0 || (uint32_t)e.shape >= d.n_shapes) return out;
+        const nh_shape &s = d.shapes[e.shape];
+        if (s.type != NH_SHAPE_MESH || s.has_normals || s.emitter < 0) return out;
+    }
+    for (uint32_t i = 0; i < d.n_shapes; ++i) {
+        const nh_shape &s = d.shapes[i];
+        if (s.emitter < 0) continue;
+        if (s.type != NH_SHAPE_MESH || s.has_normals || (uint64_t)s.f_offset + s.n_faces > d.n_faces) return {};
+        for (uint32_t f = 0; f < s.n_faces; ++f)
+            for (int j = 0; j < 3; ++j) {
+                const uint64_t v = (uint64_t)s.v_offset + d.F[3 * ((size_t)s.f_offset + f) + j];
+                if (v >= d.n_vertices) return {};
+                out.insert(out.end(), d.V + 3 * v, d.V + 3 * v + 3);
+            }
+    }
+    return out;
+}
+
+uint64_t shadow_emitter_mask(const f4 *prims, int n_records, const float *emit_faces, int n_faces) {
+    return analyse(prims, n_records, emit_faces, n_faces).emitter_word;
+}
+
+bool shadow_block_masks(const nh_camera &cam, const f4 *prims, int n_records, const float *emit_faces, int n_faces,
+                        const int32_t *blocks, int n_blocks, std::vector<uint64_t> &masks) {
+    masks.clear();
+    std::vector<uint64_t> pm;
+    std::vector<char> in_front;
+    if (!primary_masks(cam, prims, n_records, blocks, n_blocks, pm) ||
+        !primary_mask_in_front(cam, prims, n_records, in_front))
+        return false;
+    const Analysis A = analyse(prims, n_records, emit_faces, n_faces);
+    masks.assign((size_t)std::max(n_blocks, 0), 0);
+    bool all_in_front = true;
+    for (char c : in_front) all_in_front = all_in_front && c;
+    const int nbx = (cam.width + 31) / 32, nby = (cam.height + 31) / 32;
+    const double pad = primary_mask_pad(cam.width, cam.height);
+    const float *cw = cam.camera_to_world;
+    const V3 org{(double)cw[3] / cw[15], (double)cw[7] / cw[15], (double)cw[11] / cw[15]};
+    const auto direction = [&](double x, double y, V3 &d) {
+        const float *m = cam.sample_to_camera;
+        const double sx = x / cam.width, sy = y / cam.height;
+        double r[4];
+        for (int i = 0; i < 4; ++i) r[i] = m[4 * i] * sx + m[4 * i + 1] * sy + m[4 * i + 3];
+        const V3 l{r[0] / r[3], r[1] / r[3], r[2] / r[3]};
+        d = V3{cw[0] * l.x + cw[1] * l.y + cw[2] * l.z, cw[4] * l.x + cw[5] * l.y + cw[6] * l.z,
+               cw[8] * l.x + cw[9] * l.y + cw[10] * l.z};
+        const double len = norm(d);
+        if (!(len > 0.0) || !std::isfinite(len)) return false;
+        d = (1.0 / len) * d;
+        return true;
+    };
+    std::vector<V3> poly, tmp;
+    for (int i = 0; i < n_blocks; ++i) {
+        const uint64_t p = pm[(size_t)i];
+        if (!p) continue;
+        masks[(size_t)i] = A.emitter_word;
+        const int bid = blocks[i];
+        if (!A.ok || !all_in_front || bid < 0 || bid >= nbx * nby) continue;
+        const int bx = bid % nbx, by = bid / nbx;
+        const double x0 = 32.0 * bx - pad, x1 = std::min(32.0 * bx + 32.0, (double)cam.width) + pad;
+        const double y0 = 32.0 * by - pad, y1 = std::min(32.0 * by + 32.0, (double)cam.height) + pad;
+        V3 d[4], mid;
+        if (!direction(x0, y0, d[0]) || !direction(x1, y0, d[1]) || !direction(x1, y1, d[2]) ||
+            !direction(x0, y1, d[3]) || !direction(0.5 * (x0 + x1), 0.5 * (y0 + y1), mid))
+            continue;
+        V3 pn[4];
+        bool planes_ok = true;
+        double cone_cos = 1.0;
+        for (int e = 0; e < 4; ++e) {
+            pn[e] = cross(d[e], d[(e + 1) & 3]);
+            const double s = dot(pn[e], mid);
+            if (s < 0) pn[e] = -1.0 * pn[e];
+            planes_ok = planes_ok && s != 0.0;
+            for (int j = 0; j < 4; ++j) cone_cos = std::min(cone_cos, dot(d[e], d[j]));
+        }
+        if (!planes_ok || !(cone_cos > 0.5)) continue;
+        AABB region;
+        double w = 0;
+        bool grazing = false;
+        for (int k = 0; k < n_records && !grazing; ++k) {
+            if (!((p >> k) & 1)) continue;
+            const Record &R = A.rec[(size_t)k];
+            if (R.sphere) {
+                double dist = norm(R.p[0] - org);
+                const double G = sphere_grown(R.r, dist + R.r), reach = std::sqrt(3.0) * G;
+                const double t0 = std::max(dist - reach, 0.0), t1 = (dist + reach) / cone_cos;
+                AABB fr, sb;
+                for (int e = 0; e < 4; ++e) {
+                    fr.add(org + t0 * d[e]);
+                    fr.add(org + t1 * d[e]);
+                }
+                sb.add(V3{R.p[0].x - G, R.p[0].y - G, R.p[0].z - G});
+                sb.add(V3{R.p[0].x + G, R.p[0].y + G, R.p[0].z + G});
+                if (!fr.meets(sb, 0.0)) continue;
+                region.add(V3{std::max(fr.lo.x, sb.lo.x), std::max(fr.lo.y, sb.lo.y), std::max(fr.lo.z, sb.lo.z)});
+                region.add(V3{std::min(fr.hi.x, sb.hi.x), std::min(fr.hi.y, sb.hi.y), std::min(fr.hi.z, sb.hi.z)});
+                continue;
+            }
+            double c_min = INFINITY, reach = 0;
+            int side = 0;
+            for (int e = 0; e < 4; ++e) {
+                const double c = dot(R.n, d[e]);
+                const int sg = c > 0 ? 1 : c < 0 ? -1 : 0;
+                if (sg == 0 || (side && sg != side)) grazing = true;
+                side = sg;
+                c_min = std::min(c_min, std::fabs(c));
+            }
+            for (int j = 0; j < 3; ++j) reach = std::max(reach, norm(R.p[j] - org));
+            if (grazing || !(R.sin_t > 0.0)) {
+                grazing = true;
+                break;
+            }
+            w = std::max(w, 64.0 * kU * (reach + R.len) / (R.sin_t * c_min));
+            poly.assign(R.p, R.p + 3);
+            for (int e = 0; e < 4 && !poly.empty(); ++e) {
+                clip(poly, org, pn[e], tmp);
+                poly.swap(tmp);
+            }
+            for (const V3 &q : poly) region.add(q);
+        }
+        if (grazing || !std::isfinite(w)) continue;
+        AABB target = A.emit;
+        if (!region.empty()) {
+            target.add(region.lo);
+            target.add(region.hi);
+        }
+        uint64_t keep = 0;
+        for (int k = 0; k < n_records; ++k) {
+            const Record &R = A.rec[(size_t)k];
+            if (!std::isfinite(R.rho) || R.box.meets(target, A.m + A.eps_o + w + R.rho)) keep |= (uint64_t)1 << k;
+        }
+        if (n_records < 64) keep |= ~(uint64_t)0 << n_records;
+        masks[(size_t)i] = keep & A.emitter_word;
+    }
+    return true;
+}
+
+}
+
+extern "C" {
+
+int nh_shadow_emitter_faces(const nh_scene_desc *scene, float *faces, int32_t cap_faces, int32_t *n_faces) {
+    if (!scene || !n_faces || cap_faces < 0 || (cap_faces > 0 && !faces)) {
+        nh::set_host_error("nh_shadow_emitter_faces: invalid argument");
+        return NH_ERR_INVALID;
+    }
+    const std::vector<float> f = nh::shadow_emitter_faces(*scene);
+    *n_faces = (int32_t)(f.size() / 9);
+    if (*n_faces > cap_faces) {
+        nh::set_host_error("nh_shadow_emitter_faces: more faces than the caller has room for");
+        return NH_ERR_INVALID;
+    }
+    if (!f.empty()) std::memcpy(faces, f.data(), f.size() * sizeof(float));
+    return NH_OK;
+}
+
+int nh_shadow_masks(const nh_camera *camera, const float *records, int32_t n_records, const float *emit_faces,
+                    int32_t n_emit_faces, const int32_t *blocks, int32_t n_blocks, uint64_t *emitter_mask,
+                    uint64_t *masks, int32_t *built) {
+    if (!camera || !built || !emitter_mask || n_records < 0 || n_blocks < 0 || (n_records > 0 && !records) ||
+        (n_emit_faces > 0 && !emit_faces) || (n_blocks > 0 && (!blocks || !masks))) {
+        nh::set_host_error("nh_shadow_masks: invalid argument");
+        return NH_ERR_INVALID;
+    }
+    const nh::f4 *prims = reinterpret_cast<const nh::f4 *>(records);
+    *emitter_mask = nh::shadow_emitter_mask(prims, n_records, emit_faces, n_emit_faces);
+    std::vector<uint64_t> m;
+    *built = nh::shadow_block_masks(*camera, prims, n_records, emit_faces, n_emit_faces, blocks, n_blocks, m) ? 1 : 0;
+    if (*built && n_blocks > 0) std::memcpy(masks, m.data(), (size_t)n_blocks * sizeof(uint64_t));
+    return NH_OK;
+}
+
+}
diff --git a/optix-renderer_amd/nori_hip.py b/optix-renderer_amd/nori_hip.py
--- a/optix-renderer_amd/nori_hip.py
+++ b/optix-renderer_amd/nori_hip.py
@@ -188,7 +188,7 @@
                                   "tail_coop_bounces", "bounce_cycles_load", "bounce_cycles_body",
                                   "bounce_cycles_shadow", "bounce_cycles_closest", "bounce_cycles_head",
                                   "bounce_cycles_store", "bounce_bounces", "bounce_traits", "primary_masks",
-                                  "pair_kinds", "flat_trace")]
+                                  "pair_kinds", "flat_trace", "shadow_masks")]
 
 
 def _sig(name, res, *args):
@@ -220,6 +220,9 @@
 _sig("nh_primary_masks", _i32, C.POINTER(nh_camera), _fp, _i32, C.POINTER(_i32), _i32, C.POINTER(C.c_uint64),
      C.POINTER(_i32))
 _sig("nh_primary_mask_pad", _i32, _i32, _i32)
+_sig("nh_shadow_emitter_faces", _i32, C.POINTER(nh_scene_desc), _fp, _i32, C.POINTER(_i32))
+_sig("nh_shadow_masks", _i32, C.POINTER(nh_camera), _fp, _i32, _fp, _i32, C.POINTER(_i32), _i32, C.POINTER(C.c_uint64),
+     C.POINTER(C.c_uint64), C.POINTER(_i32))
 _sig("nh_pair_layout", _i32, _fp, _i32, C.POINTER(_i32), _i32, _i32, C.POINTER(_i32), C.POINTER(_i32))
 _sig("nh_flat_image", _i32, _fp, _i32, C.POINTER(_i32), _i32, _fp, _i32, _fp, _i32, C.POINTER(_i32), C.POINTER(_i32))
 _sig("nh_framebuffer_to_rgb", _i32, _fp, _i32, _i32, _i32, _fp)
@@ -843,6 +846,24 @@
     return out if built.value else None
 
 
+def shadow_emitter_faces(desc: nh_scene_desc):
+    out, n = np.zeros((max(int(desc.n_faces), 1), 9), np.float32), _i32(0)
+    _host_check(_lib.nh_shadow_emitter_faces(C.byref(desc), _fptr(out), len(out), C.byref(n)), "shadow_emitter_faces")
+    return out[:n.value].copy()
+
+
+def shadow_masks(camera: nh_camera, records: np.ndarray, emit_faces, blocks):
+    rec = np.ascontiguousarray(records, dtype=np.float32).reshape(-1, 12)
+    blk = np.ascontiguousarray(blocks, dtype=np.int32).ravel()
+    ef = np.zeros((0, 9), np.float32) if emit_faces is None else np.ascontiguousarray(emit_faces, np.float32).reshape(-1, 9)
+    out = np.zeros(len(blk), np.uint64)
+    word, built = C.c_uint64(0), _i32(0)
+    _host_check(_lib.nh_shadow_masks(C.byref(camera), _fptr(rec), len(rec), _fptr(ef), len(ef),
+                                     blk.ctypes.data_as(C.POINTER(_i32)), len(blk), C.byref(word),
+                                     out.ctypes.data_as(C.POINTER(C.c_uint64)), C.byref(built)), "shadow_masks")
+    return int(word.value), (out if built.value else None)
+
+
 def pair_layout(records: np.ndarray, leaves, by_kind: bool = True):
     rec = np.ascontiguousarray(records, dtype=np.float32).reshape(-1, 12)
     lv = np.ascontiguousarray(leaves, dtype=np.int32).reshape(-1, 2)
```
